# neel-dey/anatomix

Hardware: AMD Instinct MI355X
Metric: 128^3 volumes/sec feature-extraction (6M UNet) (higher is better)
Workload: dtype f16; 1 GPU; anatomix 6M UNet (ngf=16,num_downs=4) forward on sw_batch=4 windows of 1x128^3 (the predictor call of sliding_window_inference, BASELINE configs[1] / the metric); fp32 NCDHW in/out, 16-bit (f16) channels-last activations, fp32 accumulate; holds the 1e-3 tolerance against the fp32 reference in rel-L2 ONLY (max-norm 0.86e-3 .. 1.4e-3 by weight seed; the mode that holds both norms is value_strict); batch_per_gpu=4, window=128, parallelism=replicas x1 (no data-path collective)

## Files before the change

anatomix_amd/_lib.py:

```python
from __future__ import annotations

import ctypes as C
import os

_HERE = os.path.dirname(os.path.abspath(__file__))
LIB_PATH = os.environ.get("AMX_LIB_PATH") or os.path.join(_HERE, "csrc", "libanatomix_amd.so")

NORM = {"none": 0, "batch": 1, "instance": 2, "instance_affine": 3}
ACT = {"none": 0, "relu": 1, "lrelu": 2}
POOL = {"Max": 0, "Avg": 1}
INTERP = {"nearest": 0, "trilinear": 1}
WARP = {"bilinear": 0, "nearest": 1}
SEG_LABEL = {"float32": 0, "int64": 1, "uint8": 2}
SW_MAP = {"constant": 0, "gaussian": 1}
SW_OUT = {"features": 0, "logits": 1, "labels": 2}
PRECISION = {"f16": 0, "fp16": 0, "float16": 0, "bf16": 1, "bfloat16": 1, "f16x2": 2, "bf16x2": 3, "strict": 3, "fp32": 3,
             "f16x2mx": 4, "strict_mx": 4}


class UnetCfg(C.Structure):
    _fields_ = [
        ("input_nc", C.c_int32), ("output_nc", C.c_int32), ("num_downs", C.c_int32), ("ngf", C.c_int32),
        ("norm", C.c_int32), ("norm_eps", C.c_float), ("activation", C.c_int32), ("act_slope", C.c_float),
        ("final_act", C.c_int32), ("pooling", C.c_int32), ("interp", C.c_int32), ("doubleconv", C.c_int32),
        ("use_skip", C.c_int32), ("precision", C.c_int32),
    ]


class VitCfg(C.Structure):
    _fields_ = [
        ("input_channels", C.c_int32), ("num_classes", C.c_int32), ("embed_dim", C.c_int32), ("depth", C.c_int32),
        ("heads", C.c_int32), ("num_register_tokens", C.c_int32), ("grid_d", C.c_int32), ("grid_h", C.c_int32),
        ("grid_w", C.c_int32), ("hidden", C.c_int32), ("dec1", C.c_int32), ("dec2", C.c_int32), ("qk_norm", C.c_int32),
        ("scale_attn_inner", C.c_int32), ("layer_scale", C.c_int32), ("in_eps", C.c_float), ("out_norm", C.c_int32),
        ("decoder_split", C.c_int32), ("stem_split", C.c_int32),
    ]


_P = C.c_void_p
_I = C.c_int


class PackReq(C.Structure):
    _fields_ = [("d_weight", C.c_void_p), ("d_wpk", C.c_void_p), ("weight_mode", C.c_int32), ("cin_real", C.c_int32),
                ("cin_pad", C.c_int32), ("cout_real", C.c_int32), ("cout", C.c_int32), ("w", C.c_int32)]


WEIGHTS_PREPACKED = 16


class LaunchRecord(C.Structure):
    _fields_ = [("kernel", C.c_char * 64), ("module_idx", C.c_int32), ("cin", C.c_int32), ("cout", C.c_int32),
                ("n", C.c_int32), ("d", C.c_int32), ("h", C.c_int32), ("w", C.c_int32), ("ms", C.c_float),
                ("flops", C.c_double), ("bytes", C.c_double)]


SYMBOLS = {
    "amx_version": (_I, []),
    "amx_debug_fill_lds": (_I, [C.c_uint, _P]),
    "amx_last_error": (C.c_char_p, []),
    "amx_unet_create": (_I, [C.POINTER(_P), C.POINTER(UnetCfg)]),
    "amx_unet_destroy": (None, [_P]),
    "amx_unet_num_modules": (_I, [_P]),
    "amx_unet_num_convs": (_I, [_P]),
    "amx_unet_conv_info": (_I, [_P, _I, C.POINTER(_I), C.POINTER(_I), C.POINTER(_I), C.POINTER(_I)]),
    "amx_unet_load_conv": (_I, [_P, _I, _P, _P, _P, _P, _P, _P, _P]),
    "amx_unet_workspace_bytes": (C.c_size_t, [_P, _I, _I, _I, _I]),
    "amx_unet_forward": (_I, [_P, _P, _P, _I, _I, _I, _I, _P, C.c_size_t, _P]),
    "amx_unet_forward_profiled": (_I, [_P, _P, _P, _I, _I, _I, _I, _P, C.c_size_t, _P, C.POINTER(LaunchRecord), _I,
                                        C.POINTER(_I)]),
    "amx_unet_module_info": (_I, [_P, _I, C.POINTER(_I), C.POINTER(_I)]),
    "amx_unet_numerics_status": (_I, [_P, _I, _P]),
    "amx_unet_forward_taps": (_I, [_P, _P, _P, _I, _I, _I, _I, _P, C.c_size_t, C.POINTER(_I), _I, C.POINTER(_P), _I, _P]),
    "amx_unet_forward_window": (_I, [_P, _P, _I, _I, _I, _I, _I, _I, _I, _I, _I, _P, _P, _P, C.c_size_t, _P]),
    "amx_unet_forward_windows": (_I, [_P, _P, _I, _I, _I, _I, C.POINTER(C.c_int), _I, _I, _I, _P, _P, _P, C.c_size_t, _P]),
    "amx_unet_forward_windows_pipelined": (_I, [_P, _P, _I, _I, _I, _I, C.POINTER(C.c_int), _I, _I, _I, _P, _P, _P, C.c_size_t, _I, _P]),
    "amx_sw_normalize": (_I, [_P, _P, _I, C.c_longlong, _P]),
    "amx_sw_count": (_I, [_P, _I, _I, _I, _I, _I, _I, _I, _I, _I, _P, _P]),
    "amx_sw_plan": (_I, [_I, _I, _I, _I, _I, _I, C.c_double, C.POINTER(C.c_int), _I]),
    "amx_sw_importance_map": (_I, [_P, _I, _I, _I, _I, C.c_double, _P]),
    "amx_sw_count_all": (_I, [_P, _I, _I, _I, _I, _I, _I, C.c_double, _P, _P]),
    "amx_sw_finish": (_I, [_I, _P, _P, _I, C.c_longlong, _P, _P, _I, _P, _P]),
    "amx_sliding_window_workspace_bytes": (C.c_size_t, [_P, _I, _I, _I, _I]),
    "amx_sliding_window": (_I, [_P, _P, _I, _I, _I, _I, _I, _I, C.c_double, _I, C.c_double, _I, _I, _P, _P, _I, _P, _P, _P, _P,
                                C.c_size_t, _P]),
    "amx_conv3d_packed_bytes": (C.c_size_t, [_I, _I]),
    "amx_conv3d_k3_reflect": (_I, [_P, _I, _P, _I, _P, _P, _P, _I, _I, _I, _I, _I, _I, C.c_float, _I, _P, _P, _P, _P]),
    "amx_conv3d_dgrad_interior_supported": (_I, [_I, _I, _I, _I, _I, _I]),
    "amx_conv3d_dgrad_interior": (_I, [_P, _I, _P, _I, _I, _I, _I, _I, _I, _I, _I, _I, _P, _P, _P]),
    "amx_conv3d_dgrad_shell_scratch_bytes": (C.c_size_t, []),
    "amx_conv3d_dgrad_fold_shell": (_I, [_P, _I, _P, _I, _I, _P, _I, _I, _I, _I, _I, _I, _P, _P]),
    "amx_conv3d_pack_batch": (_I, [C.POINTER(PackReq), _I, _I, _P]),
    "amx_conv3d_scratch_bytes": (C.c_size_t, [_I, _I, _I, _I, _I, _I, _I, _I]),
    "amx_conv3d_k3_reflect_ws": (_I, [_P, _I, _P, _I, _P, _P, _P, _I, _I, _I, _I, _I, _I, C.c_float, _I, _P, _P, _P, _P, C.c_size_t, _P]),
    "amx_conv3d_upcat_merged_packed_bytes": (C.c_size_t, [_I, _I, _I]),
    "amx_conv3d_upcat_merged": (_I, [_P, _I, _P, _I, _P, _P, _P, _I, _I, _I, _I, _I, _I, C.c_float, _I, _P, _P, _P, _P]),
    "amx_conv3d_k3_reflect_ex": (_I, [_P, _I, _P, _I, _P, _I, _I, _I, _P, _P, _I, _I, _I, _I, _I, _I, C.c_float, _I, _P, _P, _P, _P]),
    "amx_pool2": (_I, [_P, _P, _I, _I, _I, _I, _I, _I, _I, _P]),
    "amx_instance_norm_scratch_bytes": (C.c_size_t, [_I, _I]),
    "amx_instance_norm": (_I, [_P, _P, _P, C.c_float, _I, C.c_longlong, _I, _I, C.c_float, _P, _I, _P]),
    "amx_upsample2_trilinear": (_I, [_P, _P, _I, _I, _I, _I, _I, _I, _P]),
    "amx_upsample2_trilinear_backward": (_I, [_P, _P, _I, _I, _I, _I, _I, _I, _P]),
    "amx_upcat_split_backward": (_I, [_P, _P, _P, _I, _I, _I, _I, _I, _I, _I, _I, _P]),
    "amx_upcat_split_backward_framed": (_I, [_P, _P, _P, _I, _I, _I, _I, _I, _I, _I, _I, _P]),
    "amx_export_ncdhw": (_I, [_P, _I, _I, _I, _I, _I, _P, _I, _P]),
    "amx_import_ncdhw": (_I, [_P, _P, _I, _I, _I, _I, _I, C.c_longlong, C.c_longlong, C.c_longlong, C.c_longlong, _I, _I, _P]),
    "amx_train_scratch_bytes": (C.c_size_t, [_I]),
    "amx_bn_train_forward": (_I, [_P, _P, _P, _P, C.c_float, _I, C.c_longlong, _I, _I, C.c_float, _P, _P, _P, _P, _P,
                                  C.c_float, _I, _P]),
    "amx_bn_act_backward": (_I, [_P, _P, _P, _P, _P, _P, _P, _P, _P, _I, _I, _I, _I, _I, _I, C.c_float, _P, _I, _P]),
    "amx_bn_act_backward_recompute": (_I, [_P, _P, _P, _P, _P, _P, _P, _P, _P, _I, _I, _I, _I, _I, _I, C.c_float, _P, _I, _P]),
    "amx_pad_fold": (_I, [_P, _P, _I, _I, _I, _I, _I, _I, _I, _P]),
    "amx_adamw_step": (_I, [_P, _I, C.c_double, C.c_double, C.c_double, C.c_double, C.c_double, _I, _P]),
    "amx_adamw_step_dev": (_I, [_P, _I, _P, _I, _P]),
    "amx_adamw_step_clip_dev": (_I, [_P, _I, _P, _I, _P, C.c_double, _P]),
    "amx_grad_norms_scratch_bytes": (C.c_size_t, [_P, _I, _I]),
    "amx_grad_norms": (_I, [_P, _I, _I, _P, _P, C.c_size_t, _P]),
    "amx_pool2_max_backward": (_I, [_P, _P, _P, _I, _I, _I, _I, _I, _I, _I, _P]),
    "amx_conv3d_wgrad_scratch_bytes": (C.c_size_t, [_I, _I, _I, _I, _I, _I]),
    "amx_conv3d_wgrad": (_I, [_P, C.c_longlong, C.c_longlong, C.c_longlong, C.c_longlong, _P, _I, _P, _I, _I, _I, _I, _I, _I,
                              _I, _P, _I, _P, C.c_size_t, _I, _P]),
    "amx_attention_scratch_bytes": (C.c_size_t, [_I, _I, _I, _I]),
    "amx_attention_qknorm_rope": (_I, [_P, _P, _P, _P, _P, _P, _P, C.c_float, _P, _I, _I, _I, _I, _I, _P, _P, C.c_size_t, _P]),
    "amx_attention_prepared": (_I, [_P, C.c_size_t, _I, _I, _I, _I, _P, _P]),
    "amx_vit_create": (_I, [C.POINTER(_P), C.POINTER(VitCfg)]),
    "amx_vit_destroy": (None, [_P]),
    "amx_vit_num_params": (_I, [_P]),
    "amx_vit_param_name": (C.c_char_p, [_P, _I]),
    "amx_vit_load": (_I, [_P, C.POINTER(_P), _I, _P, _P]),
    "amx_vit_workspace_bytes": (C.c_size_t, [_P, _I]),
    "amx_vit_forward": (_I, [_P, _P, _P, _I, _P, C.c_size_t, _I, _P]),
    "amx_vit_debug_read": (_I, [_P, C.c_char_p, _P, C.c_size_t, C.POINTER(C.c_size_t), _P]),
    "amx_linear": (_I, [_P, _P, _P, _I, _I, _I, _I, _P, _P]),
    "amx_supcon_scratch_bytes": (C.c_size_t, [_I, _I]),
    "amx_supcon_loss": (_I, [_P, _P, _I, _I, C.c_float, _I, _I, _I, _P, _P, _P, C.c_size_t, _P]),
    "amx_mlp_head_forward": (_I, [_P, _I, _I, _I, _I, _P, _P, _P, _P, _P, C.c_float, C.c_float, _I, C.c_float, _P, _P, _P, _P, _P]),
    "amx_mlp_head_scratch_bytes": (C.c_size_t, [_I, _I, _I]),
    "amx_mlp_head_backward": (_I, [_P, _P, _I, _I, _I, _I, _P, _P, _I, C.c_float, _P, _P, _P, _P, _P, _P, _P, _P, _P, C.c_size_t, _P]),
    "amx_mlp_heads_forward": (_I, [_I, _P, _I, _P, _I, _I, _P, _P, _P, _P, _P, C.c_float, C.c_float, _I, C.c_float, _P, _P, _P, _P, _P]),
    "amx_mlp_heads_backward": (_I, [_I, _P, _P, _I, _P, _I, _I, _P, _P, _I, C.c_float, _P, _P, _P, _P, _P, _P, _P, _P, _P, C.c_size_t, _P]),
    "amx_supcon_loss_batch": (_I, [_I, _P, _P, _I, _I, C.c_float, _I, _I, _I, _P, _P, _P, C.c_size_t, _P]),
    "amx_gather_labels_batch": (_I, [_P, _I, _I, _I, _I, _P, _I, _P, _I, _P, _P]),
    "amx_conv3d_backward_sampled_scratch_bytes": (C.c_size_t, [_I]),
    "amx_conv3d_backward_sampled": (_I, [_P, _P, _P, _I, _P, _I, _I, _I, _I, _I, _I, _I, _P, _P, _I, _P, C.c_size_t, _I, _P]),
    "amx_gather_rows": (_I, [_P, _I, C.c_longlong, C.c_longlong, C.c_longlong, C.c_longlong, C.c_longlong, _P, _I, _I, _I, _P, _P]),
    "amx_scatter_rows": (_I, [_P, _P, _P, _I, C.c_longlong, C.c_longlong, C.c_longlong, C.c_longlong, _I, _I, _I, _I, _P]),
    "amx_sample_coords": (_I, [_P, _I, _I, _I, _I, _I, _P, _P]),
    "amx_sample_perm": (_I, [_P, _I, _I, _I, _I, _P, _P]),
    "amx_import_input": (_I, [_P, _P, _I, _I, _I, _I, _I, _I, _P]),
    "amx_gather_labels": (_I, [_P, _I, _I, _I, _P, _I, _I, _I, _I, _I, _P, _P]),
    "amx_mindssc_scratch_bytes": (C.c_size_t, [_I, _I, _I]),
    "amx_mindssc": (_I, [_P, _I, _I, _I, _I, _I, _P, _P, C.c_size_t, _P]),
    "amx_avg_pool3d_cat": (_I, [_P, _I, C.c_float, _P, _I, C.c_float, _I, _I, _I, _I, _P, _P]),
    "amx_box_filter3d": (_I, [_P, _P, _I, _I, _I, _I, _I, _P]),
    "amx_correlate_scratch_bytes": (C.c_size_t, [_I, _I, _I, _I]),
    "amx_correlate_ssd": (_I, [_P, _P, _I, _I, _I, _I, _I, _P, _P, _P, C.c_size_t, _P]),
    "amx_coupled_convex_scratch_bytes": (C.c_size_t, [_I, _I, _I]),
    "amx_coupled_convex": (_I, [_P, _P, _I, _I, _I, _I, _P, _P, C.c_size_t, _P]),
    "amx_coupled_convex_step_scratch_bytes": (C.c_size_t, [_I, _I, _I]),
    "amx_coupled_convex_step": (_I, [_P, _P, _I, _I, _I, _I, _I, _P, _P, _P, C.c_size_t, _P]),
    "amx_inverse_consistency_scratch_bytes": (C.c_size_t, [_I, _I, _I]),
    "amx_inverse_consistency": (_I, [_P, _P, _I, _I, _I, _I, _P, _P, _P, C.c_size_t, _P]),
    "amx_resize_trilinear3d": (_I, [_P, _I, _I, _I, _I, _P, _I, _I, _I, C.POINTER(C.c_float), _I, _P]),
    "amx_stage1_registration_scratch_bytes": (C.c_size_t, [_I, _I, _I, _I, _I]),
    "amx_stage1_registration": (_I, [_P, _P, _I, _I, _I, _I, _I, _I, _I, _I, _I, _I, _P, _P, C.c_size_t, _P]),
    "amx_instance_opt_smooth3": (_I, [_P, _P, _I, _I, _I, _P]),
    "amx_instance_opt_scratch_bytes": (C.c_size_t, [_I, _I, _I, _I]),
    "amx_instance_opt_grad": (_I, [_P, _P, _P, _I, _I, _I, _I, C.c_float, _P, _P, _P, _P, C.c_size_t, _P]),
    "amx_instance_opt_adam_step": (_I, [_P, _P, _P, _P, C.c_longlong, C.c_double, _I, _P]),
    "amx_instance_opt": (_I, [_P, _P, _P, _I, _I, _I, _I, C.c_float, C.c_double, _I, _P, _P, C.c_size_t, _P]),
    "amx_run_instance_opt_scratch_bytes": (C.c_size_t, [_I, _I, _I, _I, _I, _I]),
    "amx_run_instance_opt": (_I, [_P, _P, _P, _I, _I, _I, _I, _I, C.c_float, _I, _I, C.c_double, _P, _P, C.c_size_t, _P]),
    "amx_warp3d": (_I, [_P, _I, _P, _I, _I, _I, _I, _P, _P]),
    "amx_seg_loss_scratch_bytes": (C.c_size_t, [_I, C.c_longlong, _I, _I]),
    "amx_seg_loss_forward": (_I, [_P, _I, _P, _P, _P, _I, _I, _I, C.c_longlong, _I, C.c_float, C.c_float, C.c_float, C.c_float, _P, _P,
                                  _P, _P, C.c_size_t, _P]),
    "amx_seg_loss_backward": (_I, [_P, _I, _P, _P, _P, _I, _I, _I, C.c_longlong, _I, C.c_float, C.c_float, C.c_float, C.c_float, _P, _P,
                                   _P, _P, _P, _P, C.c_size_t, _P]),
    "amx_seg_argmax": (_I, [_P, _I, _P, _P, _I, _I, C.c_longlong, _P, _P]),
    "amx_segaug_sample_bytes": (C.c_size_t, []),
    "amx_segaug_scratch_bytes": (C.c_size_t, [_I, C.c_longlong]),
    "amx_segaug_minmax": (_I, [_P, _I, C.c_longlong, _P, _P, C.c_size_t, _P]),
    "amx_segaug_minmax_finalize": (_I, [_P, C.c_size_t, _I, C.c_longlong, _P, _P]),
    "amx_segaug_pointwise": (_I, [_P, _P, _I, C.c_longlong, _P, _I, _P, _P, _P]),
    "amx_segaug_crop": (_I, [_I, _I, _I, _I, _P, _I, _P, _P, _P, _P, _P]),
    "amx_segaug_gaussian": (_I, [_P, _P, _P, _I, _I, _I, _I, _I, _P, _P, _P]),
    "amx_segaug_affine": (_I, [_P, _P, _I, _I, _I, _I, _P, _P, _I, _I, _I, _P, _P, _P, C.c_size_t, _P]),
    "amx_preaug_view_bytes": (C.c_size_t, []),
    "amx_preaug_spatial": (_I, [_P, _P, _I, _I, _I, _I, _P, _P, _P, _P, _P, _P]),
    "amx_preaug_blur": (_I, [_P, _P, _P, _I, _I, _I, _I, _P, _P, _P]),
    "amx_preaug_intensity": (_I, [_P, _P, _P, _I, _I, _I, _I, _P, _P, _P]),
    "amx_synth_view_bytes": (C.c_size_t, []),
    "amx_synth_scratch_bytes": (C.c_size_t, [_I, C.c_longlong]),
    "amx_synth_gmm_minmax": (_I, [_P, _P, _I, C.c_longlong, _P, _P, _P, C.c_size_t, _P]),
    "amx_synth_appearance": (_I, [_P, _P, C.POINTER(_P), C.POINTER(_I), _I, _P, _P, _I, _I, _I, _I, _P, _P, _P, C.c_size_t, _P]),
    "amx_synth_logk_mean": (_I, [_P, _I, C.c_longlong, _P, _P, C.c_size_t, _P]),
    "amx_synth_spike": (_I, [_P, _P, _I, _P, _I, _I, _I, _I, _P, _P, _P]),
    "amx_synth_lowres": (_I, [_P, _P, _I, _I, _I, _I, _P, _P, _P]),
    "amx_synth_clip_minmax": (_I, [_P, _I, C.c_longlong, _P, C.c_size_t, _P]),
    "amx_synth_finish": (_I, [_P, _P, _I, C.c_longlong, _P, _I, _P]),
    "amx_labels_template_bytes": (C.c_size_t, []),
    "amx_labels_ensemble_bytes": (C.c_size_t, []),
    "amx_labels_scratch_bytes": (C.c_size_t, [_I, C.c_longlong]),
    "amx_labels_compose": (_I, [_P, C.c_size_t, _P, _P, _I, _P, _P, _P, _I, _I, _I, _I, _P]),
    "amx_labels_median3": (_I, [_P, _P, _I, _I, _I, _I, _I, _P, _P, _P]),
    "amx_labels_sphere_mask": (_I, [C.POINTER(_P), _P, _I, _I, _P, _P, _P]),
    "amx_labels_apply_mask": (_I, [_P, _P, _P, _I, C.c_longlong, _P, _P, _P, C.c_size_t, _P]),
    "amx_labels_envelope": (_I, [_P, _P, _P, _I, _I, _I, _I, _P, _P, _P]),
    "amx_labels_merge_masks": (_I, [_P, _I, C.c_longlong, C.c_longlong, C.POINTER(_I), _P, _P, _P, _I, _P]),
    "amx_label_overlap": (_I, [_P, _I, _P, _I, C.c_longlong, _I, _P, _P, _P]),
    "amx_jacobian_det_scratch_bytes": (C.c_size_t, [_I, _I, _I]),
    "amx_jacobian_det": (_I, [_P, _I, _I, _I, _I, _P, _P, _P, C.c_size_t, _P]),
}

_lib = None


AMX_ERR_INVALID, AMX_ERR_SHAPE, AMX_ERR_NOT_LOADED, AMX_ERR_WORKSPACE, AMX_ERR_HIP, AMX_ERR_OVERFLOW = -1, -2, -3, -4, -5, -6


class AmxError(RuntimeError):

    def __init__(self, *args):
        self.code = args[0] if args and isinstance(args[0], int) else None
        super().__init__(*(args[1:] if self.code is not None else args))


class AmxEnvelopeError(AmxError):
    """The configuration lies outside what an engine entry covers (AMX_ERR_INVALID / AMX_ERR_SHAPE at create time)."""


class AmxOverflowError(AmxError, FloatingPointError):
    """AMX_ERR_OVERFLOW: f16 / f16x2 storage met a value outside the f16 range (include/anatomix_amd.h)."""


def load():
    global _lib
    if _lib is not None:
        return _lib
    if not os.path.exists(LIB_PATH):
        raise AmxError(
            f"{LIB_PATH} not found: build the HIP extension first (python -c 'import __graft_entry__ as g; "
            "g.build()' or make -C anatomix_amd/csrc).  There is no CPU fallback for the HIP path.")
    lib = C.CDLL(LIB_PATH)
    for name, (res, args) in SYMBOLS.items():
        fn = getattr(lib, name)
        fn.restype = res
        fn.argtypes = args
    _lib = lib
    return lib


def check(status: int):
    if status != 0:
        cls = AmxOverflowError if status == AMX_ERR_OVERFLOW else AmxError
        raise cls(int(status), f"anatomix_amd error {status}: {load().amx_last_error().decode()}")


def check_envelope(status: int):
    if status in (AMX_ERR_INVALID, AMX_ERR_SHAPE):
        raise AmxEnvelopeError(int(status), f"anatomix_amd error {status}: {load().amx_last_error().decode()}")
    check(status)


def ptr(t):
    return None if t is None else C.c_void_p(t.data_ptr())


def stream(dev):
    import torch
    return C.c_void_p(torch.cuda.current_stream(dev).cuda_stream)


def scratch(nbytes: int, dev):
    import torch
    return torch.empty(max(nbytes, 1), dtype=torch.uint8, device=dev)


def f32c(t):
    import torch
    return t if (t.dtype == torch.float32 and t.is_contiguous()) else t.float().contiguous()
```

anatomix_amd/csrc/amx_api.hip:

```cpp
#include <stdarg.h>
#include <stdio.h>
#include <string.h>

#include <string>
#include <vector>

#include "amx_launch.h"

static thread_local std::string g_err;

int amx::fail(int code, const char* fmt, ...) {
  char buf[512];
  va_list ap;
  va_start(ap, fmt);
  vsnprintf(buf, sizeof buf, fmt, ap);
  va_end(ap);
  g_err = buf;
  return code;
}

using namespace amx;

extern "C" {

int amx_version(void) { return AMX_VERSION; }

namespace {
__global__ __launch_bounds__(256) void fill_lds_kernel(unsigned pattern, unsigned* sink) {
  extern __shared__ unsigned lds_words[];
  for (int i = threadIdx.x; i < 160 * 1024 / 4; i += 256) lds_words[i] = pattern;
  __syncthreads();
  if (sink && lds_words[(threadIdx.x * 97) % (160 * 1024 / 4)] != pattern) *sink = 1;
}
}

int amx_debug_fill_lds(unsigned pattern, void* stream) {
  static amx::DeviceOnce attr_once;
  if (!attr_once.done()) {
    AMX_HIP(hipFuncSetAttribute((const void*)fill_lds_kernel, hipFuncAttributeMaxDynamicSharedMemorySize, 160 * 1024));
    attr_once.set();
  }
  hipLaunchKernelGGL(fill_lds_kernel, dim3(512), dim3(256), 160 * 1024, (hipStream_t)stream, pattern, (unsigned*)nullptr);
  AMX_HIP(hipGetLastError());
  return AMX_OK;
}

const char* amx_last_error(void) { return g_err.c_str(); }

int amx_sw_normalize(float* d_acc, const float* d_cnt, int channels, long long voxels, void* stream) {
  if (!d_acc || !d_cnt || channels < 1 || voxels < 1) return fail(AMX_ERR_INVALID, "bad argument");
  AMX_HIP(amx::launch_sw_normalize(d_acc, d_cnt, channels, voxels, (hipStream_t)stream));
  return AMX_OK;
}

int amx_sw_count(float* d_cnt, int vd, int vh, int vw, int oz, int oy, int ox, int rd, int rh, int rw,
                 const float* d_wmap, void* stream) {
  if (!d_cnt || !d_wmap) return fail(AMX_ERR_INVALID, "null argument");
  if (oz < 0 || oy < 0 || ox < 0 || oz + rd > vd || oy + rh > vh || ox + rw > vw)
    return fail(AMX_ERR_SHAPE, "window outside volume");
  AMX_HIP(amx::launch_sw_count(d_cnt, vd, vh, vw, oz, oy, ox, rd, rh, rw, d_wmap, (hipStream_t)stream));
  return AMX_OK;
}

int amx_sw_plan(int vd, int vh, int vw, int rd, int rh, int rw, double overlap, int* offsets_zyx, int capacity) {
  if (capacity < 0 || (capacity > 0 && !offsets_zyx)) return fail(AMX_ERR_INVALID, "bad offsets buffer");
  amx::SwPlan plan;
  if (int rc = amx::sw_make_plan(vd, vh, vw, rd, rh, rw, overlap, &plan)) return rc;
  const int n = plan.windows();
  for (int i = 0; i < n && i < capacity; ++i) plan.corner(i, offsets_zyx + 3 * i);
  return n;
}

int amx_sw_importance_map(float* d_wmap, int rd, int rh, int rw, int mode, double sigma_scale, void* stream) {
  if (!d_wmap) return fail(AMX_ERR_INVALID, "null argument");
  if (rd < 1 || rh < 1 || rw < 1) return fail(AMX_ERR_SHAPE, "non-positive roi");
  if (mode != AMX_SW_MAP_CONSTANT && mode != AMX_SW_MAP_GAUSSIAN) return fail(AMX_ERR_INVALID, "mode: constant (0) or gaussian (1) (got %d)", mode);
  if (mode == AMX_SW_MAP_GAUSSIAN && !(sigma_scale > 0.0)) return fail(AMX_ERR_INVALID, "sigma_scale must be positive (got %g)", sigma_scale);
  AMX_HIP(amx::launch_sw_importance_map(d_wmap, rd, rh, rw, mode, sigma_scale, (hipStream_t)stream));
  return AMX_OK;
}

int amx_sw_count_all(float* d_cnt, int vd, int vh, int vw, int rd, int rh, int rw, double overlap, const float* d_wmap,
                     void* stream) {
  if (!d_cnt || !d_wmap) return fail(AMX_ERR_INVALID, "null argument");
  amx::SwPlan plan;
  if (int rc = amx::sw_make_plan(vd, vh, vw, rd, rh, rw, overlap, &plan)) return rc;
  AMX_HIP(amx::launch_sw_count_all(d_cnt, plan, d_wmap, (hipStream_t)stream));
  return AMX_OK;
}

int amx_sw_finish(int kind, float* d_acc, const float* d_cnt, int feat, long long voxels, const float* d_w, const float* d_b,
                  int classes, void* d_out, void* stream) {
  if (int rc = amx::sw_finish_check(kind, d_acc, d_cnt, feat, voxels, d_w, classes, d_out)) return rc;
  AMX_HIP(amx::launch_sw_finish(kind, d_acc, d_cnt, feat, voxels, d_w, d_b, classes, d_out, (hipStream_t)stream));
  return AMX_OK;
}

size_t amx_conv3d_packed_bytes(int cin, int cout) {
  const int cin_pad = (cin + 15) / 16 * 16;
  size_t bytes = (size_t)cout * cin_pad * 28 * 2;
  if (cin == 48 && cout == 16) bytes = (bytes + 255) / 256 * 256 + amx::conv_upcat16_packed_bytes();
  return 2 * bytes + 256;
}

static int conv3d_single(const void* d_x0, int c0, const void* d_x1, int c1, const float* d_weight, int weight_mode,
                         int cin_real, int cout_real, const float* d_scale, const float* d_shift, int cout, int n, int d,
                         int hh, int w, int act, float slope, int precision, void* d_wpk, void* d_out16, float* d_out32,
                         void* stream, void* d_scratch = nullptr, size_t scratch_bytes = 0) {
  if (!d_x0 || (!d_weight && !(weight_mode & AMX_WEIGHTS_PREPACKED)) || !d_wpk || (!d_out16 == !d_out32)) return fail(AMX_ERR_INVALID, "bad pointer arguments");
  if (c0 % 16 || c1 % 16 || c0 + c1 < 16 || cout % 16 || cout < 16)
    return fail(AMX_ERR_INVALID, "channel counts must be multiples of 16 (c0=%d c1=%d cout=%d)", c0, c1, cout);
  if (c1 && (!d_x1 || (d & 1) || (hh & 1) || (w & 1))) return fail(AMX_ERR_SHAPE, "upsampled segment needs even dims");
  if (d < 2 || hh < 2 || w < 2) return fail(AMX_ERR_SHAPE, "reflect padding needs >= 2 voxels per axis");
  hipStream_t st = (hipStream_t)stream;
  if (precision < AMX_PREC_F16 || precision > AMX_PREC_F16X2_MX) return fail(AMX_ERR_INVALID, "unsupported precision %d", precision);
  const bool prepacked = (weight_mode & AMX_WEIGHTS_PREPACKED) != 0;
  weight_mode &= ~AMX_WEIGHTS_PREPACKED;
  if (prepacked && (is_split(precision) || d_scale)) return fail(AMX_ERR_INVALID, "prepacked weights: plain 16-bit precisions, no scale");
  if (is_mx(precision) && weight_mode != 0) return fail(AMX_ERR_INVALID, "f16x2mx packs forward weights only");
  const int q = amx::conv_pick_q(cout, w, precision);
  if (d_out32 && (q > 2 || w < 32)) return fail(AMX_ERR_INVALID, "fp32 planar output needs cout <= 32 and w >= 32");
  if (cin_real < 1 || cin_real > c0 + c1 || cout_real < 1 || cout_real > cout || (weight_mode != 0 && weight_mode != 1))
    return fail(AMX_ERR_INVALID, "bad weight description (mode %d, cin_real %d, cout_real %d)", weight_mode, cin_real, cout_real);
  amx::ConvParams p;
  memset(&p, 0, sizeof p);
  if (is_mx(precision)) {
    int* mxs = (int*)((char*)d_wpk + align_up((size_t)cout * (c0 + c1) * 28 * 2 * 2, 256));
    AMX_HIP(amx::launch_pack_weights_mx(d_weight, d_scale, d_wpk, mxs, cin_real, c0 + c1, cout, q, st, cout_real));
    p.mxs = mxs;
  } else if (!prepacked) {
    AMX_HIP(amx::launch_pack_weights(d_weight, d_scale, d_wpk, cin_real, c0 + c1, cout, q, precision, st, weight_mode, cout_real));
  }
  p.N = n; p.D = d; p.H = hh; p.W = w; p.Cout = cout;
  amx::set_src0(p, d_x0, c0, d, hh, w, precision);
  if (c1) {
    amx::set_src1(p, d_x1, c1, d / 2, hh / 2, w / 2, precision);
    p.up_shift = 1;
  }
  p.wpk = (const char*)d_wpk;
  p.bias = d_shift;
  p.act = act; p.slope = slope;
  if (d_out16) {
    amx::set_out(p, d_out16, cout, d, hh, w, precision);
  } else {
    p.out32 = d_out32;
    p.py = w; p.pz = (long long)hh * w; p.pc = p.pz * d; p.pn = p.pc * cout;
  }
  if (!is_split(precision) && weight_mode == 0 && cin_real == 48 && c0 == 16 && c1 == 32 && cout == 16 && amx::conv_upcat16_eligible(p)) {
    if (prepacked)
      return fail(AMX_ERR_INVALID, "prepacked weights: the 16 + up32 -> 16 merged-tap layer packs its own format (call without the flag)");
    char* up = (char*)d_wpk + ((size_t)cout * (c0 + c1) * 28 * 2 + 255) / 256 * 256;
    AMX_HIP(amx::launch_pack_upcat16(d_weight, d_scale, up, precision, st));
    p.wpk = up;
    AMX_HIP(amx::launch_conv_upcat16(p, precision, st));
    return AMX_OK;
  }
  if (d_scratch && !c1 && d_out16) {
    const size_t need = amx::conv_ks_part_bytes(c0, cout, n, d, hh, w, precision, q);
    if (need && (scratch_bytes < need || ((uintptr_t)d_scratch & 15)))
      return fail(AMX_ERR_WORKSPACE, "split-K scratch needs %zu bytes, 16-byte aligned (got %zu)", need, scratch_bytes);
    if (need) p.part = (float*)d_scratch;
  }
  AMX_HIP(amx::launch_conv(p, precision, q, st));
  return AMX_OK;
}

static bool dgrad_interior_shape_ok(int c_dy, int cout, int d, int hh, int w, int precision) {
  if (precision != AMX_PREC_F16 && precision != AMX_PREC_BF16) return false;
  amx::ConvParams p;
  memset(&p, 0, sizeof p);
  p.C0 = c_dy; p.Cout = cout; p.D = d; p.H = hh; p.W = w; p.out = (char*)1;
  return amx::conv_zmarch_eligible(p) && amx::conv_pick_q(cout, w, precision) == cout / 16 && (size_t)27 * c_dy * cout * 4 <= 150 * 1024;
}

int amx_conv3d_dgrad_interior_supported(int c_dy, int cout, int d, int hh, int w, int precision) {
  return dgrad_interior_shape_ok(c_dy, cout, d, hh, w, precision) ? 1 : 0;
}

int amx_conv3d_dgrad_interior(const void* d_dy_framed, int c_dy, const float* d_weight, int weight_flags, int cin_real, int cout_real, int cout,
                              int n, int d, int hh, int w, int precision, void* d_wpk, void* d_out16, void* stream) {
  if (!d_dy_framed || !d_wpk || !d_out16 || (!d_weight && !(weight_flags & AMX_WEIGHTS_PREPACKED)))
    return fail(AMX_ERR_INVALID, "dgrad_interior: bad pointer arguments");
  if (!dgrad_interior_shape_ok(c_dy, cout, d, hh, w, precision))
    return fail(AMX_ERR_INVALID, "dgrad_interior: shape outside the z-march kernels (ask amx_conv3d_dgrad_interior_supported)");
  if (cin_real < 1 || cin_real > c_dy || cout_real < 1 || cout_real > cout) return fail(AMX_ERR_INVALID, "dgrad_interior: bad weight description");
  hipStream_t st = (hipStream_t)stream;
  const int q = cout / 16;
  if (!(weight_flags & AMX_WEIGHTS_PREPACKED))
    AMX_HIP(amx::launch_pack_weights(d_weight, nullptr, d_wpk, cin_real, c_dy, cout, q, precision, st, 1, cout_real));
  amx::ConvParams p;
  memset(&p, 0, sizeof p);
  p.N = n; p.D = d; p.H = hh; p.W = w; p.Cout = cout; p.C0 = c_dy;
  p.s0x = (long long)c_dy * 2; p.s0y = p.s0x * (w + 4); p.s0z = p.s0y * (hh + 4); p.s0n = p.s0z * (d + 4);
  p.src0 = (const char*)d_dy_framed + 2 * (p.s0z + p.s0y + p.s0x);
  p.raw_halo = 1;
  p.wpk = (const char*)d_wpk;
  p.act = AMX_ACT_NONE;
  p.out = (char*)d_out16;
  p.ox = (long long)cout * 2; p.oy = p.ox * w; p.oz = p.oy * hh; p.on = p.oz * d;
  AMX_HIP(amx::launch_conv(p, precision, q, st));
  return AMX_OK;
}

size_t amx_conv3d_dgrad_shell_scratch_bytes(void) { return amx::dgrad_shell_scratch_bytes(); }

int amx_conv3d_dgrad_fold_shell(const void* d_dy_framed, int c_dy, const float* d_weight, int co_real, int ci_real, void* d_dx, int c_dx, int n,
                                int d, int hh, int w, int precision, void* d_scratch, void* stream) {
  if (!d_dy_framed || !d_weight || !d_dx || !d_scratch || ((uintptr_t)d_scratch & 15) || co_real < 1 || co_real > c_dy || ci_real < 1 || ci_real > c_dx || d < 2 || hh < 2 || w < 2)
    return fail(AMX_ERR_INVALID, "dgrad_fold_shell: bad arguments");
  const long long fx = (long long)c_dy * 2, fy = fx * (w + 4), fz = fy * (hh + 4), fn = fz * (d + 4);
  AMX_HIP(amx::launch_dgrad_fold_shell((const char*)d_dy_framed + 2 * (fz + fy + fx), fn, fz, fy, fx, c_dy, d_weight, co_real, ci_real, d_dx, c_dx,
                                       n, d, hh, w, precision, d_scratch, (hipStream_t)stream));
  return AMX_OK;
}

int amx_conv3d_pack_batch(const amx_pack_req* reqs, int count, int precision, void* stream) {
  if (!reqs || count < 1 || count > 256 || (precision != AMX_PREC_F16 && precision != AMX_PREC_BF16))
    return fail(AMX_ERR_INVALID, "pack_batch: bad arguments");
  std::vector<const float*> w(count);
  std::vector<void*> wpk(count);
  std::vector<int> cr(count), cp(count), co(count), q(count), md(count), cor(count);
  for (int i = 0; i < count; ++i) {
    const amx_pack_req& r = reqs[i];
    if (!r.d_weight || !r.d_wpk || r.cin_pad % 16 || r.cin_pad < 16 || r.cout % 16 || r.cout < 16 || r.cin_real < 1 || r.cin_real > r.cin_pad ||
        r.cout_real < 1 || r.cout_real > r.cout || (r.weight_mode != 0 && r.weight_mode != 1))
      return fail(AMX_ERR_INVALID, "pack_batch: bad request %d", i);
    w[i] = r.d_weight; wpk[i] = r.d_wpk; cr[i] = r.cin_real; cp[i] = r.cin_pad; co[i] = r.cout; md[i] = r.weight_mode; cor[i] = r.cout_real;
    q[i] = amx::conv_pick_q(r.cout, r.w, precision);
  }
  AMX_HIP(amx::launch_pack_weights_batch(count, w.data(), wpk.data(), cr.data(), cp.data(), co.data(), q.data(), md.data(), cor.data(), precision,
                                         (hipStream_t)stream));
  return AMX_OK;
}

size_t amx_conv3d_scratch_bytes(int c0, int c1, int cout, int n, int d, int hh, int w, int precision) {
  if (c1 || c0 % 16 || cout % 16 || precision < AMX_PREC_F16 || precision > AMX_PREC_F16X2_MX) return 0;
  return amx::conv_ks_part_bytes(c0, cout, n, d, hh, w, precision, amx::conv_pick_q(cout, w, precision));
}

int amx_conv3d_k3_reflect_ws(const void* d_x0, int c0, const void* d_x1, int c1, const float* d_weight,
                             const float* d_scale, const float* d_shift, int cout, int n, int d, int hh, int w,
                             int act, float slope, int precision, void* d_wpk, void* d_out16, float* d_out32,
                             void* d_scratch, size_t scratch_bytes, void* stream) {
  return conv3d_single(d_x0, c0, d_x1, c1, d_weight, 0, c0 + c1, cout, d_scale, d_shift, cout, n, d, hh, w, act, slope,
                       precision, d_wpk, d_out16, d_out32, stream, d_scratch, scratch_bytes);
}

int amx_conv3d_k3_reflect(const void* d_x0, int c0, const void* d_x1, int c1, const float* d_weight,
                          const float* d_scale, const float* d_shift, int cout, int n, int d, int hh, int w,
                          int act, float slope, int precision, void* d_wpk, void* d_out16, float* d_out32,
                          void* stream) {
  return conv3d_single(d_x0, c0, d_x1, c1, d_weight, 0, c0 + c1, cout, d_scale, d_shift, cout, n, d, hh, w, act, slope,
                       precision, d_wpk, d_out16, d_out32, stream);
}

int amx_conv3d_k3_reflect_ex(const void* d_x0, int c0, const void* d_x1, int c1, const float* d_weight, int weight_mode,
                             int cin_real, int cout_real, const float* d_scale, const float* d_shift, int cout, int n,
                             int d, int hh, int w, int act, float slope, int precision, void* d_wpk, void* d_out16,
                             float* d_out32, void* stream) {
  return conv3d_single(d_x0, c0, d_x1, c1, d_weight, weight_mode, cin_real, cout_real, d_scale, d_shift, cout, n, d, hh, w,
                       act, slope, precision, d_wpk, d_out16, d_out32, stream);
}

size_t amx_conv3d_upcat_merged_packed_bytes(int c0, int c1, int cout) {
  return 2 * (align_up((size_t)cout * c0 * 28 * 2, 256) + amx::conv_upmerge_packed_bytes(c1, cout, 0));
}

int amx_conv3d_upcat_merged(const void* d_x0, int c0, const void* d_x1, int c1, const float* d_weight, const float* d_scale,
                            const float* d_shift, int cout, int n, int d, int hh, int w, int act, float slope, int precision,
                            void* d_wpk, void* d_partial, void* d_out16, void* stream) {
  if (!d_x0 || !d_x1 || !d_weight || !d_wpk || !d_partial || !d_out16) return fail(AMX_ERR_INVALID, "null argument");
  if (precision < AMX_PREC_F16 || precision > AMX_PREC_BF16X2) return fail(AMX_ERR_INVALID, "unsupported precision %d", precision);
  const bool split = is_split(precision);
  if (c0 != cout || !amx::conv_upmerge_eligible(c0, c1, cout, d, hh, w, 1, split))
    return fail(AMX_ERR_INVALID, "merged concat conv needs c0 == cout >= 32 (16 in the strict precisions), c1 %% 32 == 0, w >= 16, even dims "
                "(c0=%d c1=%d cout=%d dims %d,%d,%d)", c0, c1, cout, d, hh, w);
  hipStream_t st = (hipStream_t)stream;
  const int q = amx::conv_pick_q(cout, w, precision);
  char* wmerge = (char*)d_wpk + align_up((size_t)cout * c0 * 28 * 2 * (split ? 2 : 1), 256);
  AMX_HIP(amx::launch_pack_weights(d_weight, d_scale, d_wpk, c0, c0, cout, q, precision, st, 0, 0, c0 + c1));
  AMX_HIP(amx::launch_pack_upmerge(d_weight, d_scale, wmerge, c0, c0 + c1, c1, cout, precision, st));
  amx::ConvParams p;
  memset(&p, 0, sizeof p);
  p.N = n; p.D = d; p.H = hh; p.W = w; p.Cout = cout;
  amx::set_src0(p, d_x0, c0, d, hh, w, precision);
  p.wpk = (const char*)d_wpk; p.act = AMX_ACT_NONE;
  amx::set_out(p, d_partial, cout, d, hh, w, precision);
  AMX_HIP(amx::launch_conv(p, precision, q, st));
  amx::UpmergeParams u;
  memset(&u, 0, sizeof u);
  amx::set_src(u, d_x1, c1, d / 2, hh / 2, w / 2, precision);
  u.N = n; u.LD = d / 2; u.LH = hh / 2; u.LW = w / 2; u.Cout = cout;
  u.wpk = wmerge; u.part = (const char*)d_partial; u.out = (char*)d_out16;
  u.bias = d_shift; u.act = act; u.slope = slope;
  AMX_HIP(amx::launch_conv_upmerge(u, precision, st));
  return AMX_OK;
}

int amx_pool2(const void* d_in, void* d_out, int n, int dout, int hout, int wout, int c, int avg, int precision,
              void* stream) {
  if (!d_in || !d_out || c % 8) return fail(AMX_ERR_INVALID, "bad argument");
  AMX_HIP(amx::launch_pool2(d_in, d_out, n, dout, hout, wout, c, avg, precision, (hipStream_t)stream));
  return AMX_OK;
}

size_t amx_train_scratch_bytes(int c) { return amx::train_scratch_bytes(c); }

int amx_bn_train_forward(const void* d_x, void* d_y, const float* d_gamma, const float* d_beta, float eps, int n,
                         long long voxels, int c, int act, float slope, void* d_scratch, float* d_save_mean,
                         float* d_save_rstd, float* d_running_mean, float* d_running_var, float momentum, int precision,
                         void* stream) {
  if (!d_x || !d_y || !d_scratch || n < 1 || voxels < 1 || c % 8 || c > 2048) return fail(AMX_ERR_INVALID, "bad argument");
  AMX_HIP(amx::launch_bn_train_forward(d_x, d_y, d_gamma, d_beta, eps, (long long)n * voxels, c, act, slope, d_scratch, d_save_mean,
                                       d_save_rstd, d_running_mean, d_running_var, momentum, precision, (hipStream_t)stream));
  return AMX_OK;
}

int amx_bn_act_backward(const void* d_dy, const void* d_y, const void* d_x, const float* d_mean, const float* d_rstd,
                        const float* d_gamma, float* d_dgamma, float* d_dbeta, void* d_dx_framed, int n, int d, int hh, int w,
                        int c, int act, float slope, void* d_scratch, int precision, void* stream) {
  if (!d_dy || !d_y || !d_dx_framed || !d_scratch || c % 8 || c > 2048) return fail(AMX_ERR_INVALID, "bad argument");
  if (d_mean && (!d_x || !d_rstd || !d_dgamma || !d_dbeta)) return fail(AMX_ERR_INVALID, "norm backward needs x, rstd, dgamma, dbeta");
  AMX_HIP(amx::launch_bn_act_backward(d_dy, d_y, d_x ? d_x : d_y, d_mean, d_rstd, d_gamma, nullptr, d_dgamma, d_dbeta, d_dx_framed, n,
                                      d, hh, w, c, act, slope, d_scratch, precision, (hipStream_t)stream));
  return AMX_OK;
}

int amx_bn_act_backward_recompute(const void* d_dy, const void* d_x, const float* d_mean, const float* d_rstd, const float* d_gamma,
                                  const float* d_beta, float* d_dgamma, float* d_dbeta, void* d_dx_framed, int n, int d, int hh, int w,
                                  int c, int act, float slope, void* d_scratch, int precision, void* stream) {
  if (!d_dy || !d_x || !d_mean || !d_rstd || !d_dgamma || !d_dbeta || !d_dx_framed || !d_scratch || c % 8 || c > 2048)
    return fail(AMX_ERR_INVALID, "bad argument");
  AMX_HIP(amx::launch_bn_act_backward(d_dy, nullptr, d_x, d_mean, d_rstd, d_gamma, d_beta, d_dgamma, d_dbeta, d_dx_framed, n, d, hh, w,
                                      c, act, slope, d_scratch, precision, (hipStream_t)stream));
  return AMX_OK;
}

int amx_pad_fold(const void* d_g_framed, void* d_din, int n, int d, int hh, int w, int c, int accumulate, int precision,
                 void* stream) {
  if (!d_g_framed || !d_din || c % 8 || d < 2 || hh < 2 || w < 2) return fail(AMX_ERR_INVALID, "bad argument");
  AMX_HIP(amx::launch_pad_fold(d_g_framed, d_din, n, d, hh, w, c, accumulate, precision, (hipStream_t)stream));
  return AMX_OK;
}

int amx_adamw_step(const amx_adamw_tensor* tensors, int count, double lr, double beta1, double beta2, double eps, double weight_decay,
                   int maximize, void* stream) {
  static_assert(sizeof(amx_adamw_tensor) == 48, "six 64-bit fields");
  if (count < 0 || (count && !tensors)) return fail(AMX_ERR_INVALID, "bad argument");
  if (!(lr >= 0.0) || !(eps >= 0.0) || !(beta1 >= 0.0 && beta1 < 1.0) || !(beta2 >= 0.0 && beta2 < 1.0) || !(weight_decay >= 0.0))
    return fail(AMX_ERR_INVALID, "adamw: lr %g, betas (%g, %g), eps %g, weight_decay %g out of range", lr, beta1, beta2, eps, weight_decay);
  for (int t = 0; t < count; ++t) {
    const amx_adamw_tensor& r = tensors[t];
    if (!r.param || !r.grad || !r.exp_avg || !r.exp_avg_sq || !r.step || r.numel < 0)
      return fail(AMX_ERR_INVALID, "adamw: tensor %d has a null pointer or a negative size", t);
  }
  AMX_HIP(amx::launch_adamw((const long long*)tensors, count, lr, beta1, beta2, eps, weight_decay, maximize, (hipStream_t)stream));
  return AMX_OK;
}

int amx_adamw_step_dev(const amx_adamw_tensor* tensors, int count, const double* d_hyper, int maximize, void* stream) {
  if (count < 0 || (count && !tensors) || !d_hyper) return fail(AMX_ERR_INVALID, "bad argument");
  for (int t = 0; t < count; ++t) {
    const amx_adamw_tensor& r = tensors[t];
    if (!r.param || !r.grad || !r.exp_avg || !r.exp_avg_sq || !r.step || r.numel < 0)
      return fail(AMX_ERR_INVALID, "adamw: tensor %d has a null pointer or a negative size", t);
  }
  AMX_HIP(amx::launch_adamw((const long long*)tensors, count, 0.0, 0.0, 0.0, 0.0, 0.0, maximize, (hipStream_t)stream, d_hyper));
  return AMX_OK;
}

int amx_adamw_step_clip_dev(const amx_adamw_tensor* tensors, int count, const double* d_hyper, int maximize, const float* d_total_norm,
                            double max_norm, void* stream) {
  if (count < 0 || (count && !tensors) || !d_hyper || !d_total_norm || !(max_norm >= 0.0))
    return fail(AMX_ERR_INVALID, "adamw: bad argument (max_norm %g)", max_norm);
  for (int t = 0; t < count; ++t) {
    const amx_adamw_tensor& r = tensors[t];
    if (!r.param || !r.grad || !r.exp_avg || !r.exp_avg_sq || !r.step || r.numel < 0)
      return fail(AMX_ERR_INVALID, "adamw: tensor %d has a null pointer or a negative size", t);
  }
  AMX_HIP(amx::launch_adamw((const long long*)tensors, count, 0.0, 0.0, 0.0, 0.0, 0.0, maximize, (hipStream_t)stream, d_hyper, d_total_norm,
                            max_norm));
  return AMX_OK;
}

size_t amx_grad_norms_scratch_bytes(const amx_grad_tensor* tensors, int count, int groups) {
  static_assert(sizeof(amx_grad_tensor) == 24, "three 64-bit fields");
  if (count < 0 || groups < 0 || (count && !tensors)) return 0;
  return amx::grad_norms_scratch_bytes((const long long*)tensors, count, groups);
}

int amx_grad_norms(const amx_grad_tensor* tensors, int count, int groups, float* d_out, void* d_scratch, size_t scratch_bytes,
                   void* stream) {
  if (count < 0 || groups < 0 || (count && !tensors) || (groups && !d_out) || !d_scratch) return fail(AMX_ERR_INVALID, "bad argument");
  for (int t = 0; t < count; ++t)
    if (!tensors[t].grad && tensors[t].numel) return fail(AMX_ERR_INVALID, "grad_norms: tensor %d has a null pointer", t);
  if (amx_grad_norms_scratch_bytes(tensors, count, groups) == 0 || scratch_bytes < amx_grad_norms_scratch_bytes(tensors, count, groups))
    return fail(AMX_ERR_INVALID, "grad_norms: a negative size, a group outside [0, %d), too many blocks, or too little scratch", groups);
  AMX_HIP(amx::launch_grad_norms((const long long*)tensors, count, groups, d_out, d_scratch, scratch_bytes, (hipStream_t)stream));
  return AMX_OK;
}

int amx_pool2_max_backward(const void* d_dp, const void* d_in, void* d_din, int n, int dout, int hout, int wout, int c,
                           int accumulate, int precision, void* stream) {
  if (!d_dp || !d_in || !d_din || c % 8) return fail(AMX_ERR_INVALID, "bad argument");
  AMX_HIP(amx::launch_pool2_max_backward(d_dp, d_in, d_din, n, dout, hout, wout, c, accumulate, precision, (hipStream_t)stream));
  return AMX_OK;
}

size_t amx_conv3d_wgrad_scratch_bytes(int n, int d, int hh, int w, int cout, int cin_pad) {
  return amx::wgrad_scratch_bytes(n, d, hh, w, cout, cin_pad);
}

int amx_conv3d_wgrad(const void* d_dy, long long dy_sn, long long dy_sz, long long dy_sy, long long dy_sx, const void* d_x0,
                     int c0, const void* d_x1, int c1, int cin_real, int cout, int n, int d, int hh, int w, float* d_dw,
                     int accumulate, void* d_scratch, size_t scratch_bytes, int precision, void* stream) {
  if (!d_dy || !d_x0 || !d_dw || !d_scratch) return fail(AMX_ERR_INVALID, "null argument");
  if (c0 % 16 || c1 % 16 || c0 + c1 < 16 || cout % 16 || cout < 16 || cin_real < 1 || cin_real > c0 + c1)
    return fail(AMX_ERR_INVALID, "channel counts must be multiples of 16 (c0=%d c1=%d cout=%d)", c0, c1, cout);
  if (c1 && (!d_x1 || (d & 1) || (hh & 1) || (w & 1))) return fail(AMX_ERR_SHAPE, "upsampled segment needs even dims");
  if (d < 2 || hh < 2 || w < 2 || w > 128) return fail(AMX_ERR_SHAPE, "wgrad supports 2 <= w <= 128 (got %d)", w);
  if (scratch_bytes < amx::wgrad_scratch_bytes(n, d, hh, w, cout, c0 + c1))
    return fail(AMX_ERR_WORKSPACE, "scratch needs %zu bytes", amx::wgrad_scratch_bytes(n, d, hh, w, cout, c0 + c1));
  amx::WgradParams p;
  memset(&p, 0, sizeof p);
  p.dy = (const char*)d_dy; p.yn = dy_sn; p.yz = dy_sz; p.yy = dy_sy; p.yx = dy_sx;
  amx::set_src0(p, d_x0, c0, d, hh, w, AMX_PREC_F16);
  if (c1) {
    amx::set_src1(p, d_x1, c1, d / 2, hh / 2, w / 2, AMX_PREC_F16);
    p.up_shift = 1;
  }
  p.N = n; p.D = d; p.H = hh; p.W = w; p.Cout = cout;
  AMX_HIP(amx::launch_wgrad(p, cin_real, d_dw, accumulate, d_scratch, precision, (hipStream_t)stream));
  return AMX_OK;
}

size_t amx_attention_scratch_bytes(int b, int heads, int n, int head_dim) {
  if (b < 1 || heads < 1 || n < 1 || head_dim < 2 || head_dim > 80) return 0;
  return amx::attention_scratch_bytes(b, heads, n);
}

int amx_attention_qknorm_rope(const float* d_q, const float* d_k, const float* d_v, const float* d_qn_w, const float* d_qn_b,
                              const float* d_kn_w, const float* d_kn_b, float norm_eps, const float* d_rope, int n_prefix, int b,
                              int n, int heads, int head_dim, float* d_out, void* d_scratch, size_t scratch_bytes, void* stream) {
  if (!d_q || !d_k || !d_v || !d_out || !d_scratch) return fail(AMX_ERR_INVALID, "null argument");
  if (b < 1 || n < 1 || heads < 1 || head_dim < 2 || head_dim > 80 || (head_dim & 1))
    return fail(AMX_ERR_INVALID, "attention: head_dim must be even and <= 80 (got %d), b, n, heads >= 1", head_dim);
  if ((!d_qn_w) != (!d_qn_b) || (!d_kn_w) != (!d_kn_b)) return fail(AMX_ERR_INVALID, "attention: norm weight and bias go together");
  if (n_prefix < 0 || n_prefix > n) return fail(AMX_ERR_INVALID, "attention: 0 <= n_prefix <= n");
  if (scratch_bytes < amx::attention_scratch_bytes(b, heads, n) || ((uintptr_t)d_scratch & 15))
    return fail(AMX_ERR_WORKSPACE, "attention scratch needs %zu bytes, 16-byte aligned", amx::attention_scratch_bytes(b, heads, n));
  AMX_HIP(amx::launch_attention(d_q, d_k, d_v, d_qn_w, d_qn_b, d_kn_w, d_kn_b, norm_eps, d_rope, n_prefix, b, n, heads, head_dim, d_out,
                                d_scratch, (hipStream_t)stream));
  return AMX_OK;
}

int amx_attention_prepared(const void* d_scratch, size_t scratch_bytes, int b, int n, int heads, int head_dim, float* d_out, void* stream) {
  if (!d_scratch || !d_out) return fail(AMX_ERR_INVALID, "null argument");
  if (b < 1 || n < 1 || heads < 1 || head_dim < 2 || head_dim > 80 || (head_dim & 1))
    return fail(AMX_ERR_INVALID, "attention: head_dim must be even and <= 80 (got %d), b, n, heads >= 1", head_dim);
  if (scratch_bytes < amx::attention_scratch_bytes(b, heads, n) || ((uintptr_t)d_scratch & 15))
    return fail(AMX_ERR_WORKSPACE, "attention scratch needs %zu bytes, 16-byte aligned", amx::attention_scratch_bytes(b, heads, n));
  void *Qp, *Kp, *Vt;
  amx::attention_operands((void*)d_scratch, b, heads, n, &Qp, &Kp, &Vt, nullptr, nullptr);
  AMX_HIP(amx::launch_attention_fwd(Qp, Kp, Vt, b, n, heads, head_dim, d_out, (hipStream_t)stream));
  return AMX_OK;
}

size_t amx_supcon_scratch_bytes(int n, int c) { return amx::supcon_scratch_bytes(n, c); }

int amx_supcon_loss(const float* d_feat, const int* d_labels, int n, int c, float temperature, int weigh_rarity,
                    int balance_denominator, int sqrt_mode, float* d_loss, float* d_grad, void* d_scratch,
                    size_t scratch_bytes, void* stream) {
  if (!d_feat || !d_labels || !d_loss || !d_scratch) return fail(AMX_ERR_INVALID, "null argument");
  if (n < 2 || n > 16384 || c < 1 || !(temperature > 0.f)) return fail(AMX_ERR_INVALID, "bad sizes (n=%d c=%d T=%g)", n, c, temperature);
  if (int rc = amx::need_scratch(amx::supcon_scratch_bytes(n, c), scratch_bytes)) return rc;
  AMX_HIP(amx::launch_supcon(d_feat, d_labels, n, c, temperature, weigh_rarity, balance_denominator, sqrt_mode, d_loss,
                             d_grad, d_scratch, (hipStream_t)stream));
  return AMX_OK;
}

size_t amx_instance_norm_scratch_bytes(int n, int c) { return amx::instnorm_scratch_bytes(n, c, 0); }

int amx_instance_norm(void* d_x, const float* d_gamma, const float* d_beta, float eps, int n, long long voxels, int c,
                      int act, float slope, void* d_scratch, int precision, void* stream) {
  if (!d_x || !d_scratch || c % 8 || c > 2048 || n < 1 || voxels < 1) return fail(AMX_ERR_INVALID, "bad argument");
  if (!d_gamma != !d_beta) return fail(AMX_ERR_INVALID, "gamma and beta come together");
  if (precision == AMX_PREC_F16X2_MX && voxels > (1 << 24)) return fail(AMX_ERR_INVALID, "f16x2mx: at most 2^24 voxels per sample here");
  AMX_HIP(amx::launch_instnorm(d_x, d_gamma, d_beta, eps, n, voxels, c, act, slope, d_scratch, precision,
                               (hipStream_t)stream, nullptr, 0, nullptr, (int)voxels));
  return AMX_OK;
}

int amx_upsample2_trilinear(const void* d_in, void* d_out, int n, int din, int hin, int win, int c, int precision,
                            void* stream) {
  if (!d_in || !d_out || c % 8 || n < 1 || din < 1 || hin < 1 || win < 1) return fail(AMX_ERR_INVALID, "bad argument");
  AMX_HIP(amx::launch_upsample2_trilinear(d_in, d_out, n, din, hin, win, c, precision, (hipStream_t)stream));
  return AMX_OK;
}

size_t amx_mindssc_scratch_bytes(int H, int W, int D) { return amx::mindssc_scratch_bytes(H, W, D); }

int amx_mindssc(const float* d_img, int H, int W, int D, int radius, int dilation, float* d_out, void* d_scratch,
                size_t scratch_bytes, void* stream) {
  if (!d_img || !d_out || !d_scratch) return fail(AMX_ERR_INVALID, "null argument");
  if (H < 1 || W < 1 || D < 1) return fail(AMX_ERR_SHAPE, "non-positive shape");
  if (radius < 1 || radius > 2 || dilation < 1 || dilation > 4)
    return fail(AMX_ERR_INVALID, "radius in {1, 2}, dilation in [1, 4] (got %d, %d)", radius, dilation);
  if (int rc = amx::need_scratch(amx::mindssc_scratch_bytes(H, W, D), scratch_bytes)) return rc;
  AMX_HIP(amx::launch_mindssc(d_img, H, W, D, radius, dilation, d_out, d_scratch, (hipStream_t)stream));
  return AMX_OK;
}

int amx_avg_pool3d_cat(const float* d_a, int ca, float scale_a, const float* d_b, int cb, float scale_b, int H, int W, int D,
                       int g, float* d_out, void* stream) {
  if (!d_out || (ca > 0 && !d_a) || (cb > 0 && !d_b) || ca < 0 || cb < 0 || ca + cb < 1) return fail(AMX_ERR_INVALID, "bad argument");
  if (g < 1 || H < g || W < g || D < g) return fail(AMX_ERR_SHAPE, "pool size %d does not fit (%d,%d,%d)", g, H, W, D);
  AMX_HIP(amx::launch_pool_cat(d_a, ca, scale_a, d_b, cb, scale_b, H, W, D, g, d_out, (hipStream_t)stream));
  return AMX_OK;
}

int amx_box_filter3d(const float* d_in, float* d_out, int c, int H, int W, int D, int k, void* stream) {
  if (!d_in || !d_out || d_in == d_out || c < 1 || c > 65535) return fail(AMX_ERR_INVALID, "bad argument");
  if (H < 1 || W < 1 || D < 1) return fail(AMX_ERR_SHAPE, "non-positive shape");
  if (k < 3 || k > 9 || !(k & 1)) return fail(AMX_ERR_INVALID, "kernel size must be odd in [3, 9] (got %d)", k);
  AMX_HIP(amx::launch_box_filter(d_in, d_out, c, H, W, D, k, (hipStream_t)stream));
  return AMX_OK;
}

size_t amx_correlate_scratch_bytes(int h, int w, int d, int disp_hw) { return amx::correlate_scratch_bytes(h, w, d, disp_hw); }

int amx_correlate_ssd(const float* d_fix, const float* d_mov, int c, int h, int w, int d, int disp_hw, float* d_ssd,
                      long long* d_argmin, void* d_scratch, size_t scratch_bytes, void* stream) {
  if (!d_fix || !d_mov || !d_ssd || !d_scratch || c < 1) return fail(AMX_ERR_INVALID, "bad argument");
  if (h < 1 || w < 1 || d < 1) return fail(AMX_ERR_SHAPE, "non-positive shape");
  if (disp_hw < 1 || disp_hw > 3) return fail(AMX_ERR_INVALID, "disp_hw in {1, 2, 3} (got %d)", disp_hw);
  if (int rc = amx::need_scratch(amx::correlate_scratch_bytes(h, w, d, disp_hw), scratch_bytes)) return rc;
  AMX_HIP(amx::launch_correlate(d_fix, d_mov, c, h, w, d, disp_hw, d_ssd, d_argmin, d_scratch, (hipStream_t)stream));
  return AMX_OK;
}

static int mlp_check(int n, int cin, int width, int n_layers) {
  if (n < 1 || n > 2048) return fail(AMX_ERR_SHAPE, "mlp head: 1 <= n <= 2048 rows (got %d)", n);
  if (cin < 4 || cin % 4 || width < 8 || width % 8) return fail(AMX_ERR_SHAPE, "mlp head: cin %% 4 == 0 and width %% 8 == 0 (got %d, %d)", cin, width);
  if (cin > 4096 || width > 4096) return fail(AMX_ERR_SHAPE, "mlp head: at most 4096 features per layer (got %d, %d)", cin, width);
  if (n_layers < 1 || n_layers > 8) return fail(AMX_ERR_INVALID, "mlp head: 1 <= n_layers <= 8 (got %d)", n_layers);
  return AMX_OK;
}

// ... 254 lines not shown
```

anatomix_amd/csrc/amx_conv3d_upcat.hip:

```cpp
#include <stdlib.h>

#include "amx_device.h"
#include "amx_launch.h"

namespace amx {

typedef __attribute__((address_space(1))) const void* gptr_t;
typedef __attribute__((address_space(3))) void* lptr_t;

struct UpcatCfg {
  static constexpr int TY = 8, TX = 32, NC = 8, NL = 3;
  static constexpr int R = 10;
  static constexpr int RL = 6;
  static constexpr int HY = TY + 2, HX = TX + 2, HXH = HX / 2;
  static constexpr int HVP = HY * HX;
  static constexpr int PPL = ((HVP * 16 + 255) / 256) * 256;
  static constexpr int PLSZ = 2 * PPL;
  static constexpr int LY = TY / 2 + 2, LX = TX / 2 + 2, LVP = LY * LX;
  static constexpr int LPL = ((LVP * 16 + 255) / 256) * 256;
  static constexpr int LPSZ = 4 * LPL;
  static constexpr int LOFF = R * PLSZ;
  static constexpr int FLAGOFF = LOFF + RL * LPSZ;
  static constexpr int LDS_BYTES = FLAGOFF + 64;
  static constexpr int NDMA = (HVP + 63) / 64;
  static constexpr int NDMAL = 4 * ((LVP + 63) / 64);
  static constexpr int AHEAD = R - 4;
  static constexpr int AHEADL = RL - 3;
  static_assert(LDS_BYTES <= 160 * 1024, "rings must fit the LDS");
  static_assert(R * NDMA <= 60 && RL * NDMAL <= 60, "vmcnt range");
};

template <typename T, int OUTMODE>
__global__ __launch_bounds__((UpcatCfg::NC + UpcatCfg::NL) * 64) void conv3d_upcat16_kernel(const ConvParams p, int zseg,
                                                                                           int nseg) {
  typedef UpcatCfg C;
  typedef typename Ops<T>::vec8 vec8;
  constexpr int HX = C::HX, PPL = C::PPL, PLSZ = C::PLSZ, LX = C::LX, LPL = C::LPL, LPSZ = C::LPSZ, R = C::R, RL = C::RL;
  constexpr int NC = C::NC, TY = C::TY, TX = C::TX;

  extern __shared__ __attribute__((aligned(16))) char smem[];

  const int tid = threadIdx.x, lane = tid & 63;
  const int wave = __builtin_amdgcn_readfirstlane(tid >> 6);

  int b = blockIdx.x;
  const int nb = gridDim.x;
  if ((nb & 7) == 0) b = (b & 7) * (nb >> 3) + (b >> 3);
  const int bx = b % p.nbx;
  b /= p.nbx;
  const int by = b % p.nby;
  b /= p.nby;
  const int sg = b % nseg;
  const int n = b / nseg;
  const int y0 = by * TY, x0 = bx * TX;
  const int zs = sg * zseg;
  const int ze = (zs + zseg < p.D) ? zs + zseg : p.D;
  const int nsteps = (ze - zs) / 2;
  const int nplanes = ze - zs + 2;
  const int nlow = nsteps + 2;

  int* ready = (int*)(smem + C::FLAGOFF);
  int* done = (int*)(smem + C::FLAGOFF + 32);
  if (tid < 16) ((int*)(smem + C::FLAGOFF))[tid] = 0;
  __syncthreads();

  if (wave >= NC + 2) {
    constexpr int NJ = (C::LVP + 63) / 64;
    int off[NJ];
    bool valid[NJ];
    const int LD = p.D >> 1, LH = p.H >> 1, LW = p.W >> 1;
#pragma unroll
    for (int j = 0; j < NJ; ++j) {
      const int hv = j * 64 + lane;
      const int hy = hv / LX, hx = hv - hy * LX;
      valid[j] = hv < C::LVP;
      int gy = (y0 >> 1) - 1 + hy, gxx = (x0 >> 1) - 1 + hx;
      gy = gy < 0 ? 0 : (gy >= LH ? LH - 1 : gy);
      gxx = gxx < 0 ? 0 : (gxx >= LW ? LW - 1 : gxx);
      off[j] = gy * (int)p.s1y + gxx * (int)p.s1x;
    }
    const char* src_n = p.src1 + (long long)n * p.s1n;
    auto issue_plane = [&](int ql) {
      int lz = (zs >> 1) - 1 + ql;
      lz = lz < 0 ? 0 : (lz >= LD ? LD - 1 : lz);
      const char* plane = src_n + (long long)lz * p.s1z;
      char* dstp = smem + C::LOFF + (ql % RL) * LPSZ;
#pragma unroll
      for (int cg = 0; cg < 4; ++cg)
#pragma unroll
        for (int j = 0; j < NJ; ++j)
          if (valid[j])
            __builtin_amdgcn_global_load_lds((gptr_t)(plane + off[j] + cg * 16), (lptr_t)(dstp + cg * LPL + j * 1024), 16, 0, 0);
    };
    int next_issue = 0, next_pub = 0;
    const unsigned a_ready = lds_addr(ready + 2), a_done = lds_addr(done);
    while (next_pub < nlow) {
      if (next_issue < nlow) {
        const int md = __builtin_amdgcn_readfirstlane(flag_min8_asm(a_done));
        int lim = RL + md;
        lim = lim < nlow ? lim : nlow;
        while (next_issue < lim) issue_plane(next_issue++);
      }
      if (next_issue == next_pub) {
        __builtin_amdgcn_s_sleep(2);
        continue;
      }
      WaitVm<C::NDMAL, RL - 1>::run(next_issue - next_pub - 1);
      flag_store_asm(a_ready, ++next_pub);
    }
    return;
  }
  if (wave >= NC) {
    const int cp = wave - NC;
    int off[C::NDMA];
    bool valid[C::NDMA];
#pragma unroll
    for (int j = 0; j < C::NDMA; ++j) {
      const int sl = j * 64 + lane;
      const int hy = sl / HX, pos = sl - hy * HX;
      const int hx = pos < C::HXH ? 2 * pos : 2 * (pos - C::HXH) + 1;
      valid[j] = sl < C::HVP;
      off[j] = reflect_clamp(y0 + hy - 1, p.H) * (int)p.s0y + reflect_clamp(x0 + hx - 1, p.W) * (int)p.s0x + cp * 16;
    }
    const char* src_n = p.src0 + (long long)n * p.s0n;
    auto issue_plane = [&](int q) {
      const char* plane = src_n + (long long)reflect_clamp(zs - 1 + q, p.D) * p.s0z;
      char* dstp = smem + (q % R) * PLSZ + cp * PPL;
#pragma unroll
      for (int j = 0; j < C::NDMA; ++j)
        if (valid[j]) __builtin_amdgcn_global_load_lds((gptr_t)(plane + off[j]), (lptr_t)(dstp + j * 1024), 16, 0, 0);
    };
    int next_issue = 0, next_pub = 0;
    const unsigned a_ready = lds_addr(ready + cp), a_done = lds_addr(done);
    while (next_pub < nplanes) {
      if (next_issue < nplanes) {
        const int md = __builtin_amdgcn_readfirstlane(flag_min8_asm(a_done));
        int lim = R + 2 * md;
        lim = lim < nplanes ? lim : nplanes;
        while (next_issue < lim) issue_plane(next_issue++);
      }
      if (next_issue == next_pub) {
        __builtin_amdgcn_s_sleep(2);
        continue;
      }
      WaitVm<C::NDMA, R - 1>::run(next_issue - next_pub - 1);
      flag_store_asm(a_ready, ++next_pub);
    }
    return;
  }

  const int pz = wave >> 2, py = (wave >> 1) & 1, px = wave & 1;
  const int li = lane & 15, g = lane >> 4, hi = g >> 1;
  vec8 wsk[kSteps], wup[8];
#pragma unroll
  for (int s = 0; s < kSteps; ++s) wsk[s] = *(const vec8*)(p.wpk + s * 1024 + lane * 16);
#pragma unroll
  for (int e = 0; e < 8; ++e) wup[e] = *(const vec8*)(p.wpk + (kSteps + wave * 8 + e) * 1024 + lane * 16);
  f32x4 bias = f32x4{0.f, 0.f, 0.f, 0.f};
  if (p.bias) bias = *(const f32x4*)(p.bias + g * 4);
  asm volatile("s_waitcnt vmcnt(0)" ::: "memory");

  const int slot0 = px * C::HXH + li;
  const int d1 = px ? -(C::HXH - 1) : C::HXH;
  const int lanebase = (g & 1) * PPL + (py * HX + slot0) * 16;
  const int base_d1 = lanebase + hi * d1 * 16;
  const int base_dx = lanebase + hi * HX * 16;
  const int lbase = C::LOFF + g * LPL + ((py * LX) + li + px) * 16;

  const bool full_xy = (y0 + TY <= p.H) & (x0 + TX <= p.W);
  const int yl = y0 + py, xl = x0 + 2 * li + px;
  char* out_l = OUTMODE == 0 ? p.out + (long long)n * p.on + (long long)yl * p.oy + (long long)xl * p.ox + g * 8 : nullptr;
  char* out_w = OUTMODE == 0 ? p.out + (long long)n * p.on + (long long)yl * p.oy + (long long)xl * p.ox + (g >> 1) * 16 : nullptr;
  float* out32_l = OUTMODE == 1 ? p.out32 + (long long)n * p.pn + (long long)(g * 4) * p.pc + (long long)yl * p.py + xl
                                : nullptr;

  bool bad = false;
  for (int s = 0; s < nsteps; ++s) {
    {
      int need = 2 * s + 4, needl = s + 3;
      need = need < nplanes ? need : nplanes;
      needl = needl < nlow ? needl : nlow;
      while (true) {
        static_assert(C::FLAGOFF % 16 == 0, "the ready flags are polled with one 16-byte read");
        const flag4_t r = flag_read4(ready);
        if ((r[0] < r[1] ? r[0] : r[1]) >= need && r[2] >= needl) break;
        __builtin_amdgcn_s_sleep(1);
      }
      asm volatile("" ::: "memory");
    }
    const int zo = zs + 2 * s + pz;
    int slo[3], llo[2];
#pragma unroll
    for (int kz = 0; kz < 3; ++kz) slo[kz] = __builtin_amdgcn_readfirstlane(((2 * s + pz + kz) % R) * PLSZ);
#pragma unroll
    for (int ez = 0; ez < 2; ++ez) llo[ez] = __builtin_amdgcn_readfirstlane(((s + pz + ez) % RL) * LPSZ);
    const int bzv = lanebase + (hi ? slo[1] : slo[0]);

    f32x4 acc[4];
#pragma unroll
    for (int c = 0; c < 4; ++c) acc[c] = bias;

    if (!(p.dbg & 2)) {
      constexpr int NSK = 4 * kSteps, NU = NSK + 4 * 8, NSLOT = 8;
      auto src = [&](int i) -> const vec8* {
        if (i < NSK) {
          const int st = i >> 2, c = i & 3;
          const int kz = st < 9 ? st / 3 : (st < 12 ? st - 9 : (st == 12 ? 0 : 2));
          const int ky = st < 9 ? st % 3 : (st < 12 ? 0 : 2);
          const int kx2 = st < 9 ? 0 : 1;
          const int off = (ky * HX + kx2) * 16 + (2 * c * HX) * 16;
          if (st < 9) return (const vec8*)(smem + base_d1 + (slo[kz] + off));
          if (st < 12) return (const vec8*)(smem + base_dx + (slo[kz] + off));
          if (st == 12) return (const vec8*)(smem + bzv + off);
          return (const vec8*)(smem + lanebase + (slo[2] + off));
        }
        const int e = (i - NSK) >> 2, c = (i - NSK) & 3;
        const int ez = e >> 2, ey = (e >> 1) & 1, ex = e & 1;
        return (const vec8*)(smem + lbase + (llo[ez] + ((c + ey) * LX + ex) * 16));
      };
      vec8 S[NSLOT];
#pragma unroll
      for (int i = 0; i < NSLOT; ++i) S[i] = *src(i);
#pragma unroll
      for (int i = 0; i < NU; ++i) {
        const int c = i < NSK ? (i & 3) : ((i - NSK) & 3);
        acc[c] = Ops<T>::mfma(i < NSK ? wsk[i >> 2] : wup[(i - NSK) >> 2], S[i % NSLOT], acc[c]);
        if (i + NSLOT < NU) S[i % NSLOT] = *src(i + NSLOT);
        __builtin_amdgcn_sched_barrier(0);
      }
    }
    asm volatile("s_waitcnt lgkmcnt(0)" ::: "memory");
    flag_store(done + wave, s + 1);

    act_inplace<4>(&acc[0], p.act, p.slope);
    if (OUTMODE == 0 && zo < ze && !(p.dbg & 4) && !(p.dbg & 32)) {
#pragma unroll
      for (int cp = 0; cp < 2; ++cp) {
        unsigned pk[2][2];
#pragma unroll
        for (int h = 0; h < 2; ++h) {
          float v[4];
#pragma unroll
          for (int j = 0; j < 4; ++j) {
            float f = acc[2 * cp + h][j];
              if (RangeCheck<T>::on) bad |= RangeCheck<T>::bad(f);
            v[j] = f;
          }
          pk[h][0] = (unsigned)to_bits<T>(v[0]) | ((unsigned)to_bits<T>(v[1]) << 16);
          pk[h][1] = (unsigned)to_bits<T>(v[2]) | ((unsigned)to_bits<T>(v[3]) << 16);
        }
        const auto s0 = __builtin_amdgcn_permlane16_swap(pk[0][0], pk[1][0], false, false);
        const auto s1 = __builtin_amdgcn_permlane16_swap(pk[0][1], pk[1][1], false, false);
        const int row = 2 * (2 * cp + (g & 1));
        if (!full_xy && !((yl + row < p.H) & (xl < p.W))) continue;
        *(uint4*)(out_w + (long long)zo * p.oz + row * p.oy) = make_uint4(s0[0], s1[0], s0[1], s1[1]);
      }
    } else if (zo < ze && !(p.dbg & 4)) {
#pragma unroll
      for (int c = 0; c < 4; ++c) {
        if (!full_xy && !((yl + 2 * c < p.H) & (xl < p.W))) continue;
        float v[4];
#pragma unroll
        for (int j = 0; j < 4; ++j) {
          float f = acc[c][j];
          if (OUTMODE == 0 && RangeCheck<T>::on) bad |= RangeCheck<T>::bad(f);
          v[j] = f;
        }
        if (OUTMODE == 0) {
          char* dst = out_l + (long long)zo * p.oz + (2 * c) * p.oy;
          *(uint2*)dst = make_uint2((unsigned)to_bits<T>(v[0]) | ((unsigned)to_bits<T>(v[1]) << 16),
                                    (unsigned)to_bits<T>(v[2]) | ((unsigned)to_bits<T>(v[3]) << 16));
        } else {
          float* dst = out32_l + (long long)zo * p.pz + (2 * c) * p.py;
          if (p.wmap) {
            const float wgt = p.wmap[((long long)zo * p.H + yl + 2 * c) * p.W + xl];
#pragma unroll
            for (int j = 0; j < 4; ++j) dst[(long long)j * p.pc] += wgt * v[j];
          } else {
#pragma unroll
            for (int j = 0; j < 4; ++j) dst[(long long)j * p.pc] = v[j];
          }
        }
      }
    }
  }
  if (OUTMODE == 0 && RangeCheck<T>::on) raise_flag(p.oflow, bad);
}

template <typename T>
__global__ void pack_upcat16_kernel(const float* __restrict__ w, const float* __restrict__ scale, T* __restrict__ wpk) {
  const int idx = blockIdx.x * blockDim.x + threadIdx.x;
  const int total = (kSteps + 64) * 512;
  if (idx >= total) return;
  const int e8 = idx & 7, lane = (idx >> 3) & 63, frag = idx >> 9;
  const int m = lane & 15, g = lane >> 4;
  const float sc = scale ? scale[m] : 1.f;
  float v = 0.f;
  if (frag < kSteps) {
    const int tap = (g >> 1) ? tapB_index(frag) : tapA_index(frag);
    const int cin = (g & 1) * 8 + e8;
    if (tap >= 0) v = w[(m * 48 + cin) * 27 + tap] * sc;
  } else {
    const int f = frag - kSteps;
    const int cls = f >> 3, e = f & 7;
    const int par[3] = {cls >> 2, (cls >> 1) & 1, cls & 1};
    const int ee[3] = {e >> 2, (e >> 1) & 1, e & 1};
    const int cin = 16 + g * 8 + e8;
    int lo[3], hi[3];
    for (int a = 0; a < 3; ++a) {
      if (par[a] == 0) { lo[a] = ee[a] ? 1 : 0; hi[a] = ee[a] ? 2 : 0; }
      else { lo[a] = ee[a] ? 2 : 0; hi[a] = ee[a] ? 2 : 1; }
    }
    float sum = 0.f;
    for (int kz = lo[0]; kz <= hi[0]; ++kz)
      for (int ky = lo[1]; ky <= hi[1]; ++ky)
        for (int kx = lo[2]; kx <= hi[2]; ++kx) sum += w[(m * 48 + cin) * 27 + (kz * 3 + ky) * 3 + kx];
    v = sum * sc;
  }
  wpk[idx] = (T)v;
}

size_t conv_upcat16_packed_bytes() { return (size_t)(kSteps + 64) * 1024; }

bool conv_upcat16_eligible(const ConvParams& p) {
  return !p.src0_f32c1 && p.up_shift == 1 && p.C0 == 16 && p.C1 == 32 && p.Cout == 16 && p.W >= 32 && p.H >= 8 && p.D >= 4 &&
         !(p.D & 1) && !(p.H & 1) && !(p.W & 1);
}

template <typename T, int OUTMODE>
static hipError_t launch_upcat_t(ConvParams p, hipStream_t st, ConvLaunchInfo* info) {
  typedef UpcatCfg C;
  if (info) info->report(0, "conv3d_upcat16<%s,2x8x32,c8+l3,r%d/%d,o%d>", __is_same(T, f16) ? "f16" : "bf16", C::R, C::RL, OUTMODE);
  auto kern = conv3d_upcat16_kernel<T, OUTMODE>;
  static amx::DeviceOnce attr_once;
  if (!attr_once.done()) {
    hipError_t e = hipFuncSetAttribute((const void*)kern, hipFuncAttributeMaxDynamicSharedMemorySize, C::LDS_BYTES);
    if (e != hipSuccess) return e;
    attr_once.set();
  }
  p.nby = (p.H + C::TY - 1) / C::TY;
  p.nbx = (p.W + C::TX - 1) / C::TX;
  const int tiles = p.nby * p.nbx * p.N;
  int nseg, zseg;
  pick_z_segments(tiles, p.D, 2, 256 * (C::LDS_BYTES <= 80 * 1024 ? 2 : 1), &zseg, &nseg);
  hipLaunchKernelGGL(kern, dim3((unsigned)(tiles * nseg)), dim3((C::NC + C::NL) * 64), C::LDS_BYTES, st, p, zseg, nseg);
  return hipGetLastError();
}

hipError_t launch_conv_upcat16(const ConvParams& p, int precision, hipStream_t st, ConvLaunchInfo* info) {
  const bool planar = p.out32 != nullptr;
  if (precision == 0) return planar ? launch_upcat_t<f16, 1>(p, st, info) : launch_upcat_t<f16, 0>(p, st, info);
  return planar ? launch_upcat_t<bf16, 1>(p, st, info) : launch_upcat_t<bf16, 0>(p, st, info);
}

hipError_t launch_pack_upcat16(const float* w, const float* scale, void* wpk, int precision, hipStream_t st) {
  const int total = (kSteps + 64) * 512;
  if (precision == 0)
    hipLaunchKernelGGL(pack_upcat16_kernel<f16>, dim3((total + 255) / 256), dim3(256), 0, st, w, scale, (f16*)wpk);
  else
    hipLaunchKernelGGL(pack_upcat16_kernel<bf16>, dim3((total + 255) / 256), dim3(256), 0, st, w, scale, (bf16*)wpk);
  return hipGetLastError();
}

}
```

anatomix_amd/csrc/amx_conv3d_zmarch.hip:

```cpp
#include <stdlib.h>
#include <string.h>

#include "amx_device.h"
#include "amx_launch.h"

namespace amx {

typedef __attribute__((address_space(1))) const void* gptr_t;
typedef __attribute__((address_space(3))) void* lptr_t;

template <int NCK, int QT, int TY, int TX, int R>
struct ZmCfg {
  static constexpr int NC = 8, TZ = 2;
  static constexpr int NL = 2 * NCK;
  static constexpr int HY = TY + 2, HX = TX + 2, HVP = HY * HX;
  static constexpr int PPL = ((HVP * 16 + 255) / 256) * 256;
  static constexpr int PLSZ = NL * PPL;
  static constexpr int FLAGOFF = R * PLSZ;
  static constexpr int LDS_BYTES = R * PLSZ + 64;
  static constexpr int XT = TX / 16;
  static constexpr int WPQ = NC / QT;
  static constexpr int NDMA = (HVP + 63) / 64;
  static_assert(WPQ == (TY / 2) * XT, "each consumer wave owns a 2 x 2 x 16 voxel block per step");
  static_assert(R - 4 > TZ, "ring must hold more than one step of prefetch");
  static constexpr bool VMCNT_OK = R * NDMA <= 60;
  static_assert(NL <= 8 && LDS_BYTES <= 160 * 1024, "ring must fit the LDS");
};

template <int QT, int TY, int TX, int OUTMODE>
struct ZmStage {
  static constexpr int CB = 32 * QT;
  static constexpr int CS = 2 * TY * TX * 4 + 64;
  static constexpr int BYTES = OUTMODE == 0 ? 2 * TY * TX * CB : 16 * QT * CS;
  static constexpr int NB = OUTMODE == 0 ? 2 : 1;
  static constexpr int TOTAL = NB * BYTES;
};

struct StemIn {
  const char* src;
  long long sn, sz, sy;
  long long offs[16];
  int use_offs;
  const char* wpk;
  const float* bias;
  int act;
  float slope;
};

template <int TY, int TX>
struct ZmStemCfg {
  static constexpr int HY = TY + 2, HX = TX + 2, HVP = HY * HX;
  static constexpr int IY = HY + 2, IX = HX + 2, IVP = IY * IX;
  static constexpr int RS = (TX + 8) * 2;
  static constexpr int CPSZ = IY * RS;
  static constexpr int IPLSZ = ((2 * CPSZ + 8 + 63) / 64) * 64;
  static constexpr int DUMMY = IPLSZ - 8;
  static constexpr int RC = 16;
  static constexpr int SW = 40;
  static constexpr int STGSZ = ((IY * SW * 4 + 255) / 256) * 256;
  static constexpr int RSTG = 8;
  static constexpr int NLD = (IVP + 63) / 64;
  static constexpr int BYTES = RC * IPLSZ + RSTG * STGSZ;
  static constexpr int NSW = 7;
  static constexpr int LEAD = 3;
  static constexpr int NT = 2 * HY + (2 * HY + 15) / 16;
  static constexpr bool OK = TX == 32 && IY == 12 && RSTG * 2 <= 60 && NLD == 7;
};

template <typename T, int NCK, int QT, int TY, int TX, int R, int OUTMODE, int NS, bool POOL, bool SPLIT = false, bool STEM = false>
__global__ __launch_bounds__((8 + (STEM ? ZmStemCfg<8, 32>::NSW + 1 : 2 * (SPLIT ? 2 : NCK)) + NS) * 64) void conv3d_k3_zmarch_kernel(const ConvParams p, int zseg, int nseg, const StemIn si) {
  static_assert(!SPLIT || (NCK == 1 && QT == 1 && NS == 0), "strict z-march: 16 -> 16, direct stores");
  static_assert(!STEM || (NCK == 1 && !SPLIT && NS == 0 && OUTMODE == 0), "stem-fed z-march: 16 input channels, direct 16-bit stores");
  constexpr int NCKP = SPLIT ? 2 : NCK;
  typedef ZmCfg<NCKP, QT, TY, TX, R> C;
  typedef ZmStage<QT, TY, TX, OUTMODE> SG;
  typedef typename Ops<T>::vec8 vec8;
  constexpr int HX = C::HX, PPL = C::PPL, PLSZ = C::PLSZ, XT = C::XT, NDMA = C::NDMA, NL = C::NL, NC = C::NC, TZ = C::TZ;
  constexpr int STAGEOFF = C::FLAGOFF + 128;
  static_assert(NS == 0 || NS == 2, "one storer wave per output plane of a step");
  static_assert(NS == 0 || STAGEOFF + SG::TOTAL <= 160 * 1024, "ring + staging tile must fit the LDS");

  extern __shared__ __attribute__((aligned(16))) char smem[];

  const int tid = threadIdx.x, lane = tid & 63;
  const int wave = __builtin_amdgcn_readfirstlane(tid >> 6);

  int b = blockIdx.x;
  const int nb = gridDim.x;
  if ((nb & 7) == 0) b = (b & 7) * (nb >> 3) + (b >> 3);
  const int bx = b % p.nbx;
  b /= p.nbx;
  const int by = b % p.nby;
  b /= p.nby;
  const int sg = b % nseg;
  const int n = b / nseg;
  const int y0 = by * TY, x0 = bx * TX;
  const int zs = sg * zseg;
  const int ze = (zs + zseg < p.D) ? zs + zseg : p.D;
  const int nplanes = ze - zs + 2;
  const int nsteps = (ze - zs + TZ - 1) / TZ;

  int* ready = (int*)(smem + C::FLAGOFF);
  int* done = (int*)(smem + C::FLAGOFF + 32);
  int* staged = (int*)(smem + C::FLAGOFF + 64);
  int* stored = (int*)(smem + C::FLAGOFF + 96);
  if (tid < ((NS || STEM) ? 32 : 16))
    ((int*)(smem + C::FLAGOFF))[tid] = (STEM && (tid < 8 || tid >= 24)) ? ((tid & 7) == 7 ? 0x7fffffff : (tid & 7)) : 0;
  if constexpr (STEM) {
    typedef ZmStemCfg<TY, TX> SC;
    static_assert(SC::OK && STAGEOFF + SC::BYTES <= 160 * 1024, "stem-fed geometry; ring + input rings must fit the LDS");
    for (int i = tid; i < SC::RC * SC::IPLSZ / 4; i += (NC + SC::NSW + 1) * 64) ((int*)(smem + STAGEOFF))[i] = 0;
  }
  __syncthreads();

  if (NS && wave >= NC + NL) {
    const int w = wave - NC - NL;
    const unsigned a_staged = lds_addr(staged), a_stored = lds_addr(stored + w);
    if constexpr (OUTMODE == 0) {
      constexpr int NR = TY * QT;
      const char* sbase = smem + STAGEOFF + w * TY * TX * SG::CB + lane * 16;
      char* gbase = p.out + (long long)n * p.on + (long long)y0 * p.oy + (long long)x0 * p.ox + lane * 16;
      for (int s = 0; s < nsteps; ++s) {
        while (__builtin_amdgcn_readfirstlane(flag_min8_asm(a_staged)) < s + 1) __builtin_amdgcn_s_sleep(1);
        uint4 v[NR];
#pragma unroll
        for (int r = 0; r < NR; ++r) v[r] = *(const uint4*)(sbase + (s % SG::NB) * SG::BYTES + r * 1024);
        asm volatile("s_waitcnt lgkmcnt(0)" ::: "memory");
        flag_store_asm(a_stored, s + 1);
        const int zo = zs + s * TZ + w;
        if (zo >= ze || (p.dbg & 4)) continue;
        char* dst = gbase + (long long)zo * p.oz;
#pragma unroll
        for (int r = 0; r < NR; ++r) *(uint4*)(dst + (long long)(r / QT) * p.oy + (r % QT) * 1024) = v[r];
      }
    } else {
      constexpr int NCH = 16 * QT;
      const int y = lane >> 3, xq = lane & 7;
      const char* sbase = smem + STAGEOFF + (w * TY + y) * (TX * 4) + xq * 16;
      float* gbase = p.out32 + (long long)n * p.pn + (long long)(y0 + y) * p.py + x0 + xq * 4;
      for (int s = 0; s < nsteps; ++s) {
        while (__builtin_amdgcn_readfirstlane(flag_min8_asm(a_staged)) < s + 1) __builtin_amdgcn_s_sleep(1);
        float4 v[NCH];
#pragma unroll
        for (int c = 0; c < NCH; ++c) v[c] = *(const float4*)(sbase + c * SG::CS);
        asm volatile("s_waitcnt lgkmcnt(0)" ::: "memory");
        flag_store_asm(a_stored, s + 1);
        const int zo = zs + s * TZ + w;
        if (zo >= ze || (p.dbg & 4)) continue;
        float* dst = gbase + (long long)zo * p.pz;
        if (p.wmap) {
          const float4 wg = *(const float4*)(p.wmap + ((long long)zo * p.H + y0 + y) * p.W + x0 + xq * 4);
#pragma unroll
          for (int c = 0; c < NCH; ++c) {
            const float4 old = *(const float4*)(dst + (long long)c * p.pc);
            v[c] = make_float4(old.x + wg.x * v[c].x, old.y + wg.y * v[c].y, old.z + wg.z * v[c].z, old.w + wg.w * v[c].w);
          }
        }
#pragma unroll
        for (int c = 0; c < NCH; ++c) *(float4*)(dst + (long long)c * p.pc) = v[c];
      }
    }
    return;
  }

  if constexpr (STEM) {
    if (wave >= NC) {
      typedef ZmStemCfg<TY, TX> SC;
      constexpr int RS = SC::RS, CPSZ = SC::CPSZ, IPLSZ = SC::IPLSZ, RC = SC::RC, RSTG = SC::RSTG, NLD = SC::NLD, IX = SC::IX, SW = SC::SW;
      constexpr int INOFF = STAGEOFF, STGOFF = STAGEOFF + RC * IPLSZ;
      int* landed = staged;
      int* inconv = stored;
      const int zlo = zs >= 2 ? zs - 2 : 0;
      const int zhi = ze + 1 <= p.D - 1 ? ze + 1 : p.D - 1;
      const int nin = zhi - zlo + 1;
      const char* src_n = si.src + (si.use_offs ? si.offs[n & 15] : (long long)n * si.sn);
      if (wave == NC + SC::NSW) {
        const int pr = lane / 10, pc = lane - pr * 10;
        const bool pvalid = lane < 60;
        int goff[2];
#pragma unroll
        for (int j = 0; j < 2; ++j) {
          int yy = y0 - 2 + pr + 6 * j, xx = x0 - 4 + 4 * pc;
          yy = yy < 0 ? 0 : (yy > p.H - 1 ? p.H - 1 : yy);
          xx = xx < 0 ? 0 : (xx > p.W - 4 ? p.W - 4 : xx);
          goff[j] = pvalid ? yy * (int)si.sy + xx * 4 : 0;
        }
        auto issue_plane = [&](int k) {
          const char* plane = src_n + (long long)(zlo + k) * si.sz;
          char* dstp = smem + STGOFF + (k % RSTG) * SC::STGSZ;
          if (pvalid) {
            __builtin_amdgcn_global_load_lds((gptr_t)(plane + goff[0]), (lptr_t)dstp, 16, 0, 0);
            __builtin_amdgcn_global_load_lds((gptr_t)(plane + goff[1]), (lptr_t)(dstp + 960), 16, 0, 0);
          }
        };
        int next_issue = 0, next_pub = 0, seen_conv = 0;
        const unsigned a_landed = lds_addr(landed);
        while (next_pub < nin) {
          while (next_issue < nin) {
            const int need = next_issue - RSTG + 1;
            if (seen_conv < need) seen_conv = __builtin_amdgcn_readfirstlane(flag_min8_asm(lds_addr(inconv)));
            if (seen_conv < need) break;
            issue_plane(next_issue++);
          }
          if (next_issue == next_pub) {
            __builtin_amdgcn_s_sleep(2);
            continue;
          }
          WaitVm<2, RSTG - 1>::run(next_issue - next_pub - 1);
          flag_store_asm(a_landed, ++next_pub);
        }
        return;
      }
      constexpr int NSW = SC::NSW;
      const int w = wave - NC;
      const int li = lane & 15, g = lane >> 4;
      const vec8 w0 = *(const vec8*)(si.wpk + 4096 + lane * 16);
      typedef __attribute__((ext_vector_type(2))) unsigned u32x2;
      typedef __attribute__((ext_vector_type(4))) unsigned u32x4;
      u32x2 w1 = *(const u32x2*)(si.wpk + 4096 + 1024 + lane * 16);
      if (g) w1 = u32x2{0u, 0u};
      const f32x4 sbias = si.bias ? *(const f32x4*)(si.bias + g * 4) : f32x4{0.f, 0.f, 0.f, 0.f};
      asm volatile("s_waitcnt vmcnt(0)" ::: "memory");
      const float lo_clip = si.act == ACT_RELU ? 0.f : -__builtin_inff();
      const int r0 = 2 * g, r1 = 2 * g + 1;
      const int kz0 = r0 / 3, kz1 = r1 / 3;
      auto xpart = [&](int hx) -> int {
        const int v0 = reflect_clamp(x0 + hx - 1, p.W) - (x0 - 2) - 1;
        return (v0 & 1) * CPSZ + (v0 & ~1) * 2;
      };
      auto ytop = [&](int hy) -> int { return reflect_clamp(y0 + hy - 1, p.H) - (y0 - 2) - 1; };
      const int xA = xpart(li), xB = xpart(16 + li);
      const int d0 = __builtin_amdgcn_readfirstlane((ytop(0) - 0) * RS), d9 = __builtin_amdgcn_readfirstlane((ytop(9) - 9) * RS);
      const int wlane = (g >> 1) * PPL + (g & 1) * 8 + li * 16;
      int croff[2], cwoff[2];
#pragma unroll
      for (int c = 0; c < 2; ++c) {
        const int crow = 8 * c + (li >> 1);
        const bool cvalid = crow < C::HY;
        const int crc = cvalid ? crow : 0;
        croff[c] = ytop(crc) * RS + xpart(32 + (li & 1));
        cwoff[c] = cvalid ? (g >> 1) * PPL + (g & 1) * 8 + (crow * HX + 32 + (li & 1)) * 16 : (g >> 1) * PPL + C::HVP * 16 + (g & 1) * 8;
      }
      constexpr int NB = 4;
      float vmax = 0.f;
      int seen_in = 0, seen_done = 0;
      int myk = w, seen_landed = 0, seen_ready = 0;
      bool ibad = false;
      auto convert_plane = [&](int k) {
        while (seen_landed < k + 1) {
          seen_landed = flag_load(landed);
          if (seen_landed < k + 1) __builtin_amdgcn_s_sleep(1);
        }
        const int need_done = zlo + k - RC + 3 - zs;
        while (seen_ready < need_done) {
          seen_ready = __builtin_amdgcn_readfirstlane(flag_min8_asm(lds_addr(ready)));
          if (seen_ready < need_done) __builtin_amdgcn_s_sleep(1);
        }
        asm volatile("" ::: "memory");
        const int so = (k % RSTG) * SC::STGSZ, dof = ((zlo + k) % RC) * IPLSZ;
        int lane_o = lane;
        asm volatile("" : "+v"(lane_o));
#pragma unroll
        for (int j = 0; j < NLD; ++j) {
          const int hv = j * 64 + lane_o;
          const bool valid = hv < SC::IVP;
          const int hvc = valid ? hv : SC::IVP - 1;
          const int iy = hvc / IX, ix = hvc - iy * IX;
          const int ry = reflect_clamp(y0 + iy - 2, p.H) - (y0 - 2), rx = reflect_clamp(x0 + ix - 2, p.W) - (x0 - 4);
          const float f = *(const float*)(smem + STGOFF + so + (ry * SW + rx) * 4);
          if (RangeCheck<T>::on) ibad |= RangeCheck<T>::bad(f);
          const unsigned short hb = to_bits<T>(f);
          const int la = valid ? iy * RS + ix * 2 : SC::DUMMY;
          const int lb = (valid && ix > 0) ? CPSZ + iy * RS + (ix - 1) * 2 : SC::DUMMY;
          *(unsigned short*)(smem + INOFF + dof + la) = hb;
          *(unsigned short*)(smem + INOFF + dof + lb) = hb;
        }
        asm volatile("" ::: "memory");
        flag_store(inconv + w, k + NSW);
      };
      for (int q = w; q < nplanes; q += NSW) {
        const int z1 = reflect_clamp(zs - 1 + q, p.D);
        int zi[3];
#pragma unroll
        for (int kz = 0; kz < 3; ++kz) zi[kz] = reflect_clamp(z1 - 1 + kz, p.D);
        int zmax = zi[0] > zi[1] ? zi[0] : zi[1];
        zmax = zmax > zi[2] ? zmax : zi[2];
        {
          int kmax = zs + q - zlo + SC::LEAD;
          kmax = kmax < nin - 1 ? kmax : nin - 1;
          for (; myk <= kmax; myk += NSW) convert_plane(myk);
        }
        while (seen_in < zmax - zlo + 1) {
          seen_in = __builtin_amdgcn_readfirstlane(flag_min8_asm(lds_addr(inconv)));
          if (seen_in < zmax - zlo + 1) __builtin_amdgcn_s_sleep(1);
        }
        while (q >= R + TZ * seen_done) {
          seen_done = __builtin_amdgcn_readfirstlane(flag_min8_asm(lds_addr(done)));
          if (q >= R + TZ * seen_done) __builtin_amdgcn_s_sleep(1);
        }
        asm volatile("" ::: "memory");
        int ib[3];
#pragma unroll
        for (int kz = 0; kz < 3; ++kz) ib[kz] = INOFF + (zi[kz] % RC) * IPLSZ;
        const int b0 = (kz0 == 0 ? ib[0] : (kz0 == 1 ? ib[1] : ib[2])) + (r0 % 3) * RS;
        const int b1 = (kz1 == 0 ? ib[0] : (kz1 == 1 ? ib[1] : ib[2])) + (r1 % 3) * RS;
        const int b8 = ib[2] + 2 * RS;
        int a0 = b0 + xA, a1 = b1 + xA, a8 = b8 + xA, c0 = b0 + xB, c1 = b1 + xB, c8 = b8 + xB;
        int wr = (q % R) * PLSZ + wlane;
        asm volatile("" : "+v"(a0), "+v"(a1), "+v"(a8), "+v"(c0), "+v"(c1), "+v"(c8), "+v"(wr));
        auto rd = [&](int addr) -> u32x2 {
          const unsigned* qq = (const unsigned*)(smem + addr);
          return u32x2{qq[0], qq[1]};
        };
        auto raddr = [&](int TI, int& r_0, int& r_1, int& r_8) {
          if (TI < 2 * C::HY) {
            const int row = TI >> 1, xt = TI & 1;
            const int d = (row == 0 ? d0 : (row == C::HY - 1 ? d9 : 0)) + row * RS;
            r_0 = (xt ? c0 : a0) + d; r_1 = (xt ? c1 : a1) + d; r_8 = (xt ? c8 : a8) + d;
          } else {
            const int c = TI - 2 * C::HY;
            r_0 = b0 + croff[c]; r_1 = b1 + croff[c]; r_8 = b8 + croff[c];
          }
        };
        auto waddr = [&](int TI) -> int {
          if (TI < 2 * C::HY) return wr + ((TI >> 1) * HX + 16 * (TI & 1)) * 16;
          return (q % R) * PLSZ + cwoff[TI - 2 * C::HY];
        };
        constexpr int NBT = (SC::NT + NB - 1) / NB;
        u32x4 fa[2][NB];
        u32x2 fe[2][NB];
        f32x4 sacc[2][NB];
        auto stage_a = [&](int bt) {
#pragma unroll
          for (int t = 0; t < NB; ++t) {
            if (bt * NB + t >= SC::NT) continue;
            int r_0, r_1, r_8;
            raddr(bt * NB + t, r_0, r_1, r_8);
            const u32x2 a = rd(r_0), bq = rd(r_1);
            fa[bt & 1][t] = u32x4{a[0], a[1], bq[0], bq[1]};
            fe[bt & 1][t] = rd(r_8);
          }
        };
        auto stage_b = [&](int bt) {
#pragma unroll
          for (int t = 0; t < NB; ++t)
            if (bt * NB + t < SC::NT) sacc[bt & 1][t] = Ops<T>::mfma(w0, __builtin_bit_cast(vec8, fa[bt & 1][t]), sbias);
#pragma unroll
          for (int t = 0; t < NB; ++t)
            if (bt * NB + t < SC::NT) sacc[bt & 1][t] = Ops<T>::mfma16(w1, fe[bt & 1][t], sacc[bt & 1][t]);
        };
        auto stage_c = [&](int bt) {
#pragma unroll
          for (int t = 0; t < NB; ++t) {
            if (bt * NB + t >= SC::NT) continue;
            float v[4];
#pragma unroll
            for (int j = 0; j < 4; ++j) v[j] = __builtin_amdgcn_fmed3f(sacc[bt & 1][t][j], lo_clip, __builtin_inff());
            if (RangeCheck<T>::on) {
              asm("v_max3_f32 %0, %1, |%2|, |%3|" : "=v"(vmax) : "v"(vmax), "v"(v[0]), "v"(v[1]));
              asm("v_max3_f32 %0, %1, |%2|, |%3|" : "=v"(vmax) : "v"(vmax), "v"(v[2]), "v"(v[3]));
            }
            *(uint2*)(smem + waddr(bt * NB + t)) = make_uint2(Ops<T>::pack2(v[0], v[1]), Ops<T>::pack2(v[2], v[3]));
          }
        };
        stage_a(0);
        if (NBT > 1) stage_a(1);
        __builtin_amdgcn_sched_barrier(0);
        stage_b(0);
        __builtin_amdgcn_sched_barrier(0);
#pragma unroll
        for (int bt = 0; bt < NBT; ++bt) {
          if (bt + 2 < NBT) stage_a(bt + 2);
          __builtin_amdgcn_sched_barrier(0);
          if (bt + 1 < NBT) stage_b(bt + 1);
          __builtin_amdgcn_sched_barrier(0);
          stage_c(bt);
          __builtin_amdgcn_sched_barrier(0);
        }
        asm volatile("" ::: "memory");
        flag_store(ready + w, q + NSW);
      }
      for (; myk < nin; myk += NSW) convert_plane(myk);
      if (RangeCheck<T>::on) raise_flag(p.oflow, ibad | !(vmax <= 65504.f));
      return;
    }
  }

  if (!STEM && wave >= NC) {
    static_assert(STEM || C::VMCNT_OK, "loader wave must not exceed the 6-bit vmcnt range");
    const int cp = wave - NC;
    int off[NDMA];
    bool valid[NDMA];
#pragma unroll
    for (int j = 0; j < NDMA; ++j) {
      const int hv = j * 64 + lane;
      const int hy = hv / HX, hx = hv - hy * HX;
      valid[j] = hv < C::HVP;
      off[j] = halo_coord(y0 + hy - 1, p.H, p.raw_halo) * (int)p.s0y + halo_coord(x0 + hx - 1, p.W, p.raw_halo) * (int)p.s0x + cp * 16;
    }
    const char* src_n = p.src0 + (long long)n * p.s0n;
    auto issue_plane = [&](int q) {
      const char* plane = src_n + (long long)halo_coord(zs - 1 + q, p.D, p.raw_halo) * p.s0z;
      char* dstp = smem + (q % R) * PLSZ + cp * PPL;
#pragma unroll
      for (int j = 0; j < NDMA; ++j)
        if (valid[j]) __builtin_amdgcn_global_load_lds((gptr_t)(plane + off[j]), (lptr_t)(dstp + j * 1024), 16, 0, 0);
    };
    int next_issue = 0, next_pub = 0;
    const unsigned a_ready = lds_addr(ready + cp), a_done = lds_addr(done);
    while (next_pub < nplanes) {
      if (next_issue < nplanes) {
        const int md = __builtin_amdgcn_readfirstlane(flag_min8_asm(a_done));
        int lim = R + TZ * md;
        lim = lim < nplanes ? lim : nplanes;
        while (next_issue < lim) issue_plane(next_issue++);
      }
      if (next_issue == next_pub) {
        __builtin_amdgcn_s_sleep(2);
        continue;
      }
      WaitVm<NDMA, R - 1>::run(next_issue - next_pub - 1);
      flag_store_asm(a_ready, ++next_pub);
    }
    return;
  }

  const int li = lane & 15, g = lane >> 4, hi = g >> 1;
  const int wq = wave / C::WPQ;
  const int wr = wave % C::WPQ;
  const int wrow = (wr / XT) * 2;
  const int wcx = wr % XT;
  vec8 wreg[NCKP][kSteps];
#pragma unroll
  for (int k = 0; k < NCKP; ++k)
#pragma unroll
    for (int s = 0; s < kSteps; ++s) wreg[k][s] = *(const vec8*)(p.wpk + ((k * kSteps + s) * QT + wq) * 1024 + lane * 16);
  const int cb = g * 4 * QT + wq * 4;
  f32x4 bias = f32x4{0.f, 0.f, 0.f, 0.f};
  if (p.bias) bias = *(const f32x4*)(p.bias + cb);
  asm volatile("s_waitcnt vmcnt(0)" ::: "memory");

  const int lanebase = (g & 1) * PPL + ((wrow * HX) + wcx * 16 + li) * 16;
  const int base_d1 = lanebase + hi * 16;
  const int base_dx = lanebase + hi * 16 * HX;
  const bool full_xy = (y0 + TY <= p.H) & (x0 + TX <= p.W);

  const int yl = y0 + wrow, xl = x0 + wcx * 16 + li;
  char* out_l = OUTMODE == 0 ? p.out + (long long)n * p.on + (long long)yl * p.oy + (long long)xl * p.ox + cb * 2 : nullptr;
  float* out32_l = OUTMODE == 1 ? p.out32 + (long long)n * p.pn + (long long)cb * p.pc + (long long)yl * p.py + xl : nullptr;
  constexpr bool WIDE = OUTMODE == 0 && NS == 0 && QT == 1;
  char* out_w = WIDE ? p.out + (long long)n * p.on + (long long)(yl + (g & 1)) * p.oy + (long long)xl * p.ox + (g >> 1) * 16 : nullptr;
  const bool vec_planar = OUTMODE == 1 && !(p.W & 3) && !(p.py & 3) && !(p.pz & 3) && !(p.pc & 3) && !(p.pn & 3) &&
                          !((size_t)p.out32 & 15) && !((size_t)p.wmap & 15);
  float* out32_q = OUTMODE == 1 ? p.out32 + (long long)n * p.pn + (long long)(cb + (li & 3)) * p.pc + (long long)yl * p.py +
                                      x0 + wcx * 16 + (li & ~3)
                                : nullptr;
  char* out2_l = (OUTMODE == 0 && POOL) ? p.out2 + (long long)n * p.qn + (long long)(yl >> 1) * p.qy +
                                               (long long)(xl >> 1) * p.qx + cb * 2
                                          : nullptr;

  bool bad = false;
  unsigned long long* trace = (p.dbg & 8) && (wave == 0 || wave == 4) && lane == 0 && blockIdx.x < 500
                                  ? (unsigned long long*)p.stats + ((long long)blockIdx.x * 2 + (wave >> 2)) * 128 : nullptr;
  int tcount = 0;
#define AMX_ZSTAMP()                                                             \
  do {                                                                           \
    if (trace && tcount < 128) trace[tcount] = __builtin_readcyclecounter();     \
    ++tcount;                                                                    \
  } while (0)
  AMX_ZSTAMP();
  for (int s = 0; s < nsteps; ++s) {
    {
      int need = TZ * s + TZ + 2;
      need = need < nplanes ? need : nplanes;
      static_assert(NL <= 4 && C::FLAGOFF % 16 == 0, "the ready flags are polled with one 16-byte read");
      if constexpr (STEM) {
        while (__builtin_amdgcn_readfirstlane(flag_min8_asm(lds_addr(ready))) < need) __builtin_amdgcn_s_sleep(1);
      } else {
        while (flag_min4<NL>(ready) < need) __builtin_amdgcn_s_sleep(1);
      }
      asm volatile("" ::: "memory");
    }

    AMX_ZSTAMP();
    int b1[4], bx3[4];
#pragma unroll
    for (int pl = 0; pl < 4; ++pl) {
      const int sl = ((s * TZ + pl) % R) * PLSZ;
      b1[pl] = base_d1 + sl;
      bx3[pl] = base_dx + sl;
    }
    f32x4 acc[2][2];
#pragma unroll
    for (int tz = 0; tz < 2; ++tz)
#pragma unroll
      for (int cy = 0; cy < 2; ++cy) acc[tz][cy] = bias;

    for (int rep = (p.dbg >> 10) & 7; rep >= 0; --rep)
    if (!(p.dbg & 2)) {
      if constexpr ((NCKP > 1 && !SPLIT) || STEM) {
        constexpr int PER = 4 * 6 + 8, NU = NCKP * PER, NSLOT = 4;
        int slo[4];
#pragma unroll
        for (int pl = 0; pl < 4; ++pl) slo[pl] = __builtin_amdgcn_readfirstlane(((s * TZ + pl) % R) * PLSZ);
        const int tail_lo = lanebase + (2 * HX + 2) * 16;
        auto src = [&](int i) -> const vec8* {
          const int ps = i / PER, j = i % PER, koff = ps * 2 * PPL;
          if (j < 24) {
            const int pl = j / 6, f = j % 6;
            return f < 4 ? (const vec8*)(smem + base_d1 + (slo[pl] + koff + (f * HX) * 16))
                         : (const vec8*)(smem + base_dx + (slo[pl] + koff + ((f - 4) * HX + 2) * 16));
          }
          const int t = j - 24, tz = t >> 2, cy = (t >> 1) & 1, which = t & 1;
          if (which) return (const vec8*)(smem + tail_lo + (slo[tz + 2] + koff + (cy * HX) * 16));
          return (const vec8*)(smem + tail_lo + ((hi ? slo[tz + 1] : slo[tz]) + koff + (cy * HX) * 16));
        };
        auto use = [&](int i, const vec8& frag) {
          const int ps = i / PER, j = i % PER;
          const int k = SPLIT ? 0 : ps;
          const bool both = SPLIT && ps == 0;
          auto mm = [&](const int widx, f32x4 a) {
            a = Ops<T>::mfma(wreg[k][widx], frag, a);
            if (both) a = Ops<T>::mfma(wreg[NCKP - 1][widx], frag, a);
            return a;
          };
          if (j < 24) {
            const int pl = j / 6, f = j % 6;
#pragma unroll
            for (int tz = 0; tz < 2; ++tz) {
              const int kz = pl - tz;
              if (kz < 0 || kz > 2) continue;
              if (f < 4) {
#pragma unroll
                for (int cy = 0; cy < 2; ++cy) {
                  const int ky = f - cy;
                  if (ky >= 0 && ky < 3) acc[tz][cy] = mm(kz * 3 + ky, acc[tz][cy]);
                }
              } else {
                acc[tz][f - 4] = mm(9 + kz, acc[tz][f - 4]);
              }
            }
          } else {
            const int t = j - 24, tz = t >> 2, cy = (t >> 1) & 1, which = t & 1;
            acc[tz][cy] = mm(12 + which, acc[tz][cy]);
          }
        };
        vec8 S[NSLOT];
#pragma unroll
        for (int i = 0; i < NSLOT; ++i) S[i] = *src(i);
#pragma clang loop unroll(full)
        for (int i = 0; i < NU; ++i) {
          use(i, S[i % NSLOT]);
          if (i + NSLOT < NU) S[i % NSLOT] = *src(i + NSLOT);
          __builtin_amdgcn_sched_barrier(0);
        }
      } else {
#pragma unroll
        for (int ps = 0; ps < NCKP; ++ps) {
          const int k = SPLIT ? 0 : ps;
          const bool both = SPLIT && ps == 0;
          const int koff = ps * 2 * PPL;
          auto mm = [&](const int widx, const vec8& frag, f32x4 a) {
            a = Ops<T>::mfma(wreg[k][widx], frag, a);
            if (both) a = Ops<T>::mfma(wreg[NCKP - 1][widx], frag, a);
            return a;
          };
          constexpr bool DB = NCKP == 1;
          vec8 F[DB ? 2 : 1][4], H[DB ? 2 : 1][2];
          auto load_plane = [&](int buf, int pl) {
  #pragma unroll
            for (int r = 0; r < 4; ++r) F[buf][r] = *(const vec8*)(smem + b1[pl] + koff + (r * HX) * 16);
  #pragma unroll
            for (int cy = 0; cy < 2; ++cy) H[buf][cy] = *(const vec8*)(smem + bx3[pl] + koff + (cy * HX + 2) * 16);
          };
          auto mma_plane = [&](int buf, int pl) {
  #pragma unroll
            for (int tz = 0; tz < 2; ++tz) {
              const int kz = pl - tz;
              if (kz < 0 || kz > 2) continue;
  #pragma unroll
              for (int ky = 0; ky < 3; ++ky)
  #pragma unroll
                for (int cy = 0; cy < 2; ++cy) acc[tz][cy] = mm(kz * 3 + ky, F[buf][cy + ky], acc[tz][cy]);
  #pragma unroll
              for (int cy = 0; cy < 2; ++cy) acc[tz][cy] = mm(9 + kz, H[buf][cy], acc[tz][cy]);
            }
          };
          if (DB) {
            load_plane(0, 0);
  #pragma unroll
            for (int pl = 0; pl < 4; ++pl) {
              if (pl + 1 < 4) load_plane((pl + 1) & 1, pl + 1);
              __builtin_amdgcn_sched_barrier(0);
              mma_plane(pl & 1, pl);
            }
          } else {
  #pragma unroll
            for (int pl = 0; pl < 4; ++pl) {
              load_plane(0, pl);
              mma_plane(0, pl);
            }
          }
  #pragma unroll
          for (int tz = 0; tz < 2; ++tz) {
            const int sl0 = ((s * TZ + tz) % R) * PLSZ, sl1 = ((s * TZ + tz + 1) % R) * PLSZ, sl2 = ((s * TZ + tz + 2) % R) * PLSZ;
            const int bz = lanebase + (hi ? sl1 : sl0) + koff + (2 * HX + 2) * 16;
            const int b0 = lanebase + sl2 + koff + (2 * HX + 2) * 16;
  #pragma unroll
            for (int cy = 0; cy < 2; ++cy) {
              const vec8 s0 = *(const vec8*)(smem + bz + (cy * HX) * 16);
              const vec8 s1 = *(const vec8*)(smem + b0 + (cy * HX) * 16);
              acc[tz][cy] = mm(12, s0, acc[tz][cy]);
              acc[tz][cy] = mm(13, s1, acc[tz][cy]);
            }
          }
        }
      }
      }
    asm volatile("s_waitcnt lgkmcnt(0)" ::: "memory");
    flag_store(done + wave, s + 1);
    AMX_ZSTAMP();

    if (p.dbg & 4) {
      if (NS) flag_store(staged + wave, s + 1);
      continue;
    }
    if constexpr (NS > 0) {
      if (s >= SG::NB)
        while (flag_min2(stored) < s + 1 - SG::NB) __builtin_amdgcn_s_sleep(1);
      asm volatile("" ::: "memory");
    }
    act_inplace<4>(&acc[0][0], p.act, p.slope);
    float pooled[4] = {-3.0e38f, -3.0e38f, -3.0e38f, -3.0e38f};
#pragma unroll
    for (int tz = 0; tz < 2; ++tz) {
      const int zo = zs + s * TZ + tz;
      if (WIDE && (SPLIT || !(p.dbg & 32))) {
        unsigned pk[2][2], pl[SPLIT ? 2 : 1][2];
#pragma unroll
        for (int cy = 0; cy < 2; ++cy) {
          float v[4];
#pragma unroll
          for (int j = 0; j < 4; ++j) {
            float f = acc[tz][cy][j];
              if (RangeCheck<T>::on) bad |= RangeCheck<T>::bad(f);
            v[j] = f;
            pooled[j] = f > pooled[j] ? f : pooled[j];
          }
          pk[cy][0] = (unsigned)to_bits<T>(v[0]) | ((unsigned)to_bits<T>(v[1]) << 16);
          pk[cy][1] = (unsigned)to_bits<T>(v[2]) | ((unsigned)to_bits<T>(v[3]) << 16);
          if constexpr (SPLIT) {
            float r[4];
#pragma unroll
            for (int j = 0; j < 4; ++j) r[j] = v[j] - (float)(T)v[j];
            pl[cy][0] = (unsigned)to_bits<T>(r[0]) | ((unsigned)to_bits<T>(r[1]) << 16);
            pl[cy][1] = (unsigned)to_bits<T>(r[2]) | ((unsigned)to_bits<T>(r[3]) << 16);
          }
        }
        const auto s0 = __builtin_amdgcn_permlane16_swap(pk[0][0], pk[1][0], false, false);
        const auto s1 = __builtin_amdgcn_permlane16_swap(pk[0][1], pk[1][1], false, false);
        unsigned l0a = 0, l0b = 0, l1a = 0, l1b = 0;
        if constexpr (SPLIT) {
          const auto t0 = __builtin_amdgcn_permlane16_swap(pl[0][0], pl[1][0], false, false);
          const auto t1 = __builtin_amdgcn_permlane16_swap(pl[0][1], pl[1][1], false, false);
          l0a = t0[0]; l0b = t0[1]; l1a = t1[0]; l1b = t1[1];
        }
        if (zo >= ze) continue;
        if (!full_xy && !((yl + (g & 1) < p.H) & (xl < p.W))) continue;
        *(uint4*)(out_w + (long long)zo * p.oz) = make_uint4(s0[0], s1[0], s0[1], s1[1]);
        if constexpr (SPLIT) *(uint4*)(out_w + (long long)zo * p.oz + p.Cout * 2) = make_uint4(l0a, l1a, l0b, l1b);
        continue;
      }
#pragma unroll
      for (int cy = 0; cy < 2; ++cy) {
        float v[4];
#pragma unroll
        for (int j = 0; j < 4; ++j) {
          float f = acc[tz][cy][j];
          if (OUTMODE == 0 && RangeCheck<T>::on) bad |= RangeCheck<T>::bad(f);
          v[j] = f;
          pooled[j] = f > pooled[j] ? f : pooled[j];
        }
        if constexpr (NS > 0) {
          if (OUTMODE == 0) {
            char* dst = smem + STAGEOFF + (s % SG::NB) * SG::BYTES + (((tz * TY + wrow + cy) * TX) + wcx * 16 + li) * SG::CB + cb * 2;
            *(uint2*)dst = make_uint2((unsigned)to_bits<T>(v[0]) | ((unsigned)to_bits<T>(v[1]) << 16),
                                      (unsigned)to_bits<T>(v[2]) | ((unsigned)to_bits<T>(v[3]) << 16));
          } else {
            quad_transpose4(v, li);
            char* dst = smem + STAGEOFF + (cb + (li & 3)) * SG::CS + ((tz * TY + wrow + cy) * TX + wcx * 16 + (li & ~3)) * 4;
            *(float4*)dst = make_float4(v[0], v[1], v[2], v[3]);
          }
          continue;
        }
        if (zo >= ze) continue;
        if (!full_xy && !((yl + cy < p.H) & (xl < p.W))) continue;
        if (OUTMODE == 0) {
          char* dst = out_l + (long long)zo * p.oz + cy * p.oy;
          *(uint2*)dst = make_uint2((unsigned)to_bits<T>(v[0]) | ((unsigned)to_bits<T>(v[1]) << 16),
                                    (unsigned)to_bits<T>(v[2]) | ((unsigned)to_bits<T>(v[3]) << 16));
        } else if (vec_planar) {
          quad_transpose4(v, li);
          float* dst = out32_q + (long long)zo * p.pz + cy * p.py;
          float4 o = make_float4(v[0], v[1], v[2], v[3]);
          if (p.wmap) {
            const float4 wg = *(const float4*)(p.wmap + ((long long)zo * p.H + yl + cy) * p.W + x0 + wcx * 16 + (li & ~3));
            const float4 old = *(const float4*)dst;
            o = make_float4(old.x + wg.x * o.x, old.y + wg.y * o.y, old.z + wg.z * o.z, old.w + wg.w * o.w);
          }
          *(float4*)dst = o;
        } else {
          float* dst = out32_l + (long long)zo * p.pz + cy * p.py;
          if (p.wmap) {
            const float wgt = p.wmap[((long long)zo * p.H + yl + cy) * p.W + xl];
#pragma unroll
            for (int j = 0; j < 4; ++j) dst[(long long)j * p.pc] += wgt * v[j];
          } else {
#pragma unroll
            for (int j = 0; j < 4; ++j) dst[(long long)j * p.pc] = v[j];
          }
        }
      }
    }
    if constexpr (NS > 0) {
      asm volatile("" ::: "memory");
      flag_store(staged + wave, s + 1);
    }
    if constexpr (OUTMODE == 0 && POOL) {
      float pm[4];
#pragma unroll
      for (int j = 0; j < 4; ++j) {
        const float o = dpp_quad<0xB1>(pooled[j]);
        pm[j] = pooled[j] > o ? pooled[j] : o;
      }
      const int zp = (zs + s * TZ) >> 1;
      if (!(li & 1) && zs + s * TZ + 1 < ze && (full_xy || ((yl + 1 < p.H) & (xl + 1 < p.W)))) {
        char* dst = out2_l + (long long)zp * p.qz;
        *(uint2*)dst = make_uint2((unsigned)to_bits<T>(pm[0]) | ((unsigned)to_bits<T>(pm[1]) << 16),
                                  (unsigned)to_bits<T>(pm[2]) | ((unsigned)to_bits<T>(pm[3]) << 16));
        if constexpr (SPLIT) {
          float r[4];
#pragma unroll
          for (int j = 0; j < 4; ++j) r[j] = pm[j] - (float)(T)pm[j];
          *(uint2*)(dst + p.Cout * 2) = make_uint2((unsigned)to_bits<T>(r[0]) | ((unsigned)to_bits<T>(r[1]) << 16),
                                                   (unsigned)to_bits<T>(r[2]) | ((unsigned)to_bits<T>(r[3]) << 16));
        }
      }
    }
    AMX_ZSTAMP();
  }
  if (OUTMODE == 0 && RangeCheck<T>::on) raise_flag(p.oflow, bad);
}

template <typename T, int NCK, int QT, int TY, int R, int OUTMODE, int NS, bool POOL = false, bool SPLIT = false, int TX = 32, bool STEM = false>
static hipError_t launch_zm_ns(ConvParams p, hipStream_t st, ConvLaunchInfo* info, const StemIn& si = StemIn{}) {
  if constexpr (OUTMODE == 0 && NS == 0 && !POOL && !STEM)
    if (p.out2) return launch_zm_ns<T, NCK, QT, TY, R, OUTMODE, NS, true, SPLIT, TX, STEM>(p, st, info, si);
  constexpr int TZ = 2;
  typedef ZmCfg<SPLIT ? 2 : NCK, QT, TY, TX, R> C;
  constexpr int LDS = STEM ? C::FLAGOFF + 128 + ZmStemCfg<TY, TX>::BYTES : NS ? C::FLAGOFF + 128 + ZmStage<QT, TY, TX, OUTMODE>::TOTAL : C::LDS_BYTES;
  if (info && STEM)
    info->report(0, "conv3d_k3_zmarch<%s,stem1->16->16,%dx%dx%d,c8+st%d+ld1,r%d/%d%s>", __is_same(T, f16) ? "f16" : "bf16", TZ, TY, TX,
                 ZmStemCfg<TY, TX>::NSW, R, ZmStemCfg<TY, TX>::RC, p.out2 ? ",pool" : "");
  else if (info)
    info->report(0, "conv3d_k3_zmarch<%s%s,%d->%d,%dx%dx%d,c8+l%d+s%d,r%d,o%d%s>", __is_same(T, f16) ? "f16" : "bf16", SPLIT ? "x2" : "",
                 16 * NCK, 16 * QT, TZ, TY, TX, C::NL, NS, R, OUTMODE, p.out2 ? ",pool" : "");
  auto kern = conv3d_k3_zmarch_kernel<T, NCK, QT, TY, TX, R, OUTMODE, NS, POOL, SPLIT, STEM>;
  static amx::DeviceOnce attr_once;
  if (!attr_once.done()) {
    hipError_t e = hipFuncSetAttribute((const void*)kern, hipFuncAttributeMaxDynamicSharedMemorySize, LDS);
    if (e != hipSuccess) return e;
    attr_once.set();
  }
  p.nby = (p.H + TY - 1) / TY;
  p.nbx = (p.W + TX - 1) / TX;
  const int tiles = p.nby * p.nbx * p.N;
  int nseg, zseg;
  pick_z_segments(tiles, p.D, TZ, 256 * (LDS <= 80 * 1024 ? 2 : 1), &zseg, &nseg);
  hipLaunchKernelGGL(kern, dim3((unsigned)(tiles * nseg)), dim3((8 + (STEM ? ZmStemCfg<TY, TX>::NSW + 1 : C::NL) + NS) * 64), LDS, st, p, zseg, nseg, si);
  return hipGetLastError();
}

template <int TY>
static bool zm_can_stage(const ConvParams& p) {
  if (p.H % TY || p.W % 32) return false;
  return !((size_t)p.out32 & 3) && !((size_t)p.wmap & 3);
}

template <typename T, int NCK, int QT, int TY, int R, int OUTMODE>
static hipError_t launch_zm(const ConvParams& p, hipStream_t st, ConvLaunchInfo* info) {
  if constexpr (NCK == 1 && OUTMODE == 1)
    if (zm_can_stage<TY>(p)) return launch_zm_ns<T, NCK, QT, TY, R, OUTMODE, 2>(p, st, info);
  return launch_zm_ns<T, NCK, QT, TY, R, OUTMODE, 0>(p, st, info);
}

bool conv_zmarch_eligible(const ConvParams& p) {
  if (p.src0_f32c1 || p.C1 != 0 || p.W < 32 || p.H < 8 || p.D < 8) return false;
  if (p.C0 == 16 && p.Cout == 16) return true;
  if (p.out32) return false;
  return (p.C0 == 16 || p.C0 == 32) && p.Cout == 32;
}

bool conv_zmarch_can_pool(const ConvParams& p) {
  return conv_zmarch_eligible(p) && !p.out32 && !(p.D & 1) && !(p.H & 1) && !(p.W & 1);
}

bool conv_zmarch_eligible_split(const ConvParams& p) {
  return conv_zmarch_eligible(p) && p.C0 == 16 && p.Cout == 16;
}
bool conv_zmarch_can_pool_split(const ConvParams& p) { return conv_zmarch_can_pool(p) && conv_zmarch_eligible_split(p); }

bool conv_zmarch_stem_eligible(const ConvParams& p, int precision) {
  return precision < 2 && p.C0 == 16 && p.C1 == 0 && p.Cout == 16 && !p.out32 && !p.raw_halo && p.W >= 32 && !(p.W % 32) && !(p.H % 8) &&
         !(p.D & 1) && p.D >= 8 && p.ox == 32 && (p.ocs == 0 || p.ocs == 32);
}
hipError_t launch_conv_zmarch_stem(const ConvParams& p, const float* x, long long xs_n, long long xs_z, long long xs_y, const long long* x_offs,
                                   const void* stem_wpk, const float* stem_bias, int stem_act, float stem_slope, int precision, hipStream_t st,
                                   ConvLaunchInfo* info) {
  if (stem_act != ACT_NONE && stem_act != ACT_RELU) return hipErrorInvalidValue;
  if ((precision != 0 && precision != 1) || (x_offs && p.N > 16)) return hipErrorInvalidValue;
  StemIn si;
  memset(&si, 0, sizeof si);
  si.src = (const char*)x; si.sn = xs_n; si.sz = xs_z; si.sy = xs_y;
  if (x_offs) {
    si.use_offs = 1;
    for (int i = 0; i < p.N; ++i) si.offs[i] = x_offs[i] * 4;
  }
  si.wpk = (const char*)stem_wpk; si.bias = stem_bias; si.act = stem_act; si.slope = stem_slope;
  if (precision == 0) return launch_zm_ns<f16, 1, 1, 8, 10, 0, 0, false, false, 32, true>(p, st, info, si);
  return launch_zm_ns<bf16, 1, 1, 8, 10, 0, 0, false, false, 32, true>(p, st, info, si);
}

hipError_t launch_conv_zmarch(const ConvParams& p, int precision, hipStream_t st, ConvLaunchInfo* info) {
  const bool planar = p.out32 != nullptr;
  if (precision >= 2) {
    if (p.C0 != 16 || p.Cout != 16) return hipErrorInvalidValue;
    if (precision == 2) return planar ? launch_zm_ns<f16, 1, 1, 8, 7, 1, 0, false, true>(p, st, info) : launch_zm_ns<f16, 1, 1, 8, 7, 0, 0, false, true>(p, st, info);
    return planar ? launch_zm_ns<bf16, 1, 1, 8, 7, 1, 0, false, true>(p, st, info) : launch_zm_ns<bf16, 1, 1, 8, 7, 0, 0, false, true>(p, st, info);
  }
  if (p.Cout == 16) {
    if (precision == 0) return planar ? launch_zm<f16, 1, 1, 8, 10, 1>(p, st, info) : launch_zm<f16, 1, 1, 8, 10, 0>(p, st, info);
    return planar ? launch_zm<bf16, 1, 1, 8, 10, 1>(p, st, info) : launch_zm<bf16, 1, 1, 8, 10, 0>(p, st, info);
  }
  if (p.C0 == 16) return precision == 0 ? launch_zm<f16, 1, 2, 4, 10, 0>(p, st, info) : launch_zm<bf16, 1, 2, 4, 10, 0>(p, st, info);
  return precision == 0 ? launch_zm<f16, 2, 2, 4, 10, 0>(p, st, info) : launch_zm<bf16, 2, 2, 4, 10, 0>(p, st, info);
}

}
```

anatomix_amd/csrc/amx_device.h:

```cpp
#pragma once
#include "amx_common.h"

namespace amx {

template <typename T> struct Ops;
typedef __attribute__((ext_vector_type(2))) unsigned amx_u32x2;
template <> struct Ops<f16> {
  typedef f16x8 vec8;
  static __device__ __forceinline__ f32x4 mfma(vec8 a, vec8 b, f32x4 c) {
    return __builtin_amdgcn_mfma_f32_16x16x32_f16(a, b, c, 0, 0, 0);
  }
  static __device__ __forceinline__ f32x4 mfma16(amx_u32x2 a, amx_u32x2 b, f32x4 c) {
    typedef __attribute__((ext_vector_type(4))) _Float16 h4;
    return __builtin_amdgcn_mfma_f32_16x16x16f16(__builtin_bit_cast(h4, a), __builtin_bit_cast(h4, b), c, 0, 0, 0);
  }
  static __device__ __forceinline__ unsigned pack2(float a, float b) {
    typedef __attribute__((ext_vector_type(2))) float f2;
    typedef __attribute__((ext_vector_type(2))) _Float16 h2;
    return __builtin_bit_cast(unsigned, __builtin_convertvector(f2{a, b}, h2));
  }
};
template <> struct Ops<bf16> {
  typedef bf16x8 vec8;
  static __device__ __forceinline__ f32x4 mfma(vec8 a, vec8 b, f32x4 c) {
    return __builtin_amdgcn_mfma_f32_16x16x32_bf16(a, b, c, 0, 0, 0);
  }
  static __device__ __forceinline__ f32x4 mfma16(amx_u32x2 a, amx_u32x2 b, f32x4 c) {
    typedef __attribute__((ext_vector_type(4))) short s4;
    return __builtin_amdgcn_mfma_f32_16x16x16bf16_1k(__builtin_bit_cast(s4, a), __builtin_bit_cast(s4, b), c, 0, 0, 0);
  }
  static __device__ __forceinline__ unsigned pack2(float a, float b) {
    typedef __attribute__((ext_vector_type(2))) float f2;
    typedef __attribute__((ext_vector_type(2))) __bf16 b2;
    return __builtin_bit_cast(unsigned, __builtin_convertvector(f2{a, b}, b2));
  }
};

template <typename T> struct RangeCheck {
  static constexpr bool on = false;
  static __device__ __forceinline__ bool bad(float) { return false; }
};
template <> struct RangeCheck<f16> {
  static constexpr bool on = true;
  static __device__ __forceinline__ bool bad(float v) { return !(__builtin_fabsf(v) <= 65504.f); }
};
__device__ __forceinline__ void raise_flag(int* flag, bool bad) {
  if (bad && flag) __atomic_store_n(flag, 1, __ATOMIC_RELAXED);
}

__device__ __forceinline__ int reflect_clamp(int g, int n) {
  g = g < 0 ? -g : g;
  g = g >= n ? 2 * n - 2 - g : g;
  g = g < 0 ? 0 : g;
  return g >= n ? n - 1 : g;
}

__device__ __forceinline__ int halo_coord(int g, int n, int raw) {
  if (raw) return g < -1 ? -1 : (g > n ? n : g);
  return reflect_clamp(g, n);
}

typedef __attribute__((ext_vector_type(8))) int i32x8;
constexpr float kMxLoScale = 2048.f;
__device__ __forceinline__ unsigned e4m3_pk4(float a, float b, float c, float d) {
  a = __builtin_amdgcn_fmed3f(a, -448.f, 448.f);
  b = __builtin_amdgcn_fmed3f(b, -448.f, 448.f);
  c = __builtin_amdgcn_fmed3f(c, -448.f, 448.f);
  d = __builtin_amdgcn_fmed3f(d, -448.f, 448.f);
  int v = __builtin_amdgcn_cvt_pk_fp8_f32(a, b, 0, false);
  v = __builtin_amdgcn_cvt_pk_fp8_f32(c, d, v, true);
  return (unsigned)v;
}
__device__ __forceinline__ void mx_split8(const float (&f)[8], uint2& xl8, uint2& xh8) {
  float h[8], l[8];
#pragma unroll
  for (int e = 0; e < 8; ++e) {
    h[e] = (float)(_Float16)f[e];
    l[e] = (float)(_Float16)(f[e] - h[e]) * kMxLoScale;
  }
  xl8 = make_uint2(e4m3_pk4(l[0], l[1], l[2], l[3]), e4m3_pk4(l[4], l[5], l[6], l[7]));
  xh8 = make_uint2(e4m3_pk4(h[0], h[1], h[2], h[3]), e4m3_pk4(h[4], h[5], h[6], h[7]));
}

__device__ __forceinline__ void mx_split8_direct(const float (&f)[8], uint2& xl8, uint2& xh8) {
  float h[8], l[8];
#pragma unroll
  for (int e = 0; e < 8; ++e) {
    h[e] = (float)(_Float16)f[e];
    l[e] = (f[e] - h[e]) * kMxLoScale;
  }
  xl8 = make_uint2(e4m3_pk4(l[0], l[1], l[2], l[3]), e4m3_pk4(l[4], l[5], l[6], l[7]));
  xh8 = make_uint2(e4m3_pk4(h[0], h[1], h[2], h[3]), e4m3_pk4(h[4], h[5], h[6], h[7]));
}

__device__ __forceinline__ unsigned dpp_xor1(unsigned v) {
  return (unsigned)__builtin_amdgcn_update_dpp(0, (int)v, 0xB1, 0xF, 0xF, true);
}
__device__ __forceinline__ void mx_store_copies(char* chunk, int odd, const float (&f)[8]) {
  uint2 xl8, xh8;
  mx_split8(f, xl8, xh8);
  const uint2 send = odd ? xl8 : xh8;
  const unsigned r0 = dpp_xor1(send.x), r1 = dpp_xor1(send.y);
  *(uint4*)(chunk + odd * 16) = odd ? make_uint4(r0, r1, xh8.x, xh8.y) : make_uint4(xl8.x, xl8.y, r0, r1);
}

template <typename T>
__device__ __forceinline__ unsigned short to_bits(float v) {
  T t = (T)v;
  return __builtin_bit_cast(unsigned short, t);
}

template <int CTRL>
__device__ __forceinline__ float dpp_quad(float x) {
  return __builtin_bit_cast(float, __builtin_amdgcn_update_dpp(0, __builtin_bit_cast(int, x), CTRL, 0xF, 0xF, true));
}
__device__ __forceinline__ void quad_transpose4(float (&v)[4], int lane_in_quad_bits) {
  const bool b0 = lane_in_quad_bits & 1, b1 = lane_in_quad_bits & 2;
  const float r01 = dpp_quad<0xB1>(b0 ? v[0] : v[1]);
  const float r23 = dpp_quad<0xB1>(b0 ? v[2] : v[3]);
  if (b0) { v[0] = r01; v[2] = r23; } else { v[1] = r01; v[3] = r23; }
  const float r02 = dpp_quad<0x4E>(b1 ? v[0] : v[2]);
  const float r13 = dpp_quad<0x4E>(b1 ? v[1] : v[3]);
  if (b1) { v[0] = r02; v[1] = r13; } else { v[2] = r02; v[3] = r13; }
}

__device__ __forceinline__ int flag_load(const int* p) {
  return __atomic_load_n(p, __ATOMIC_RELAXED);
}
__device__ __forceinline__ void flag_store(int* p, int v) {
  __atomic_store_n(p, v, __ATOMIC_RELAXED);
}

__device__ __forceinline__ unsigned lds_addr(const void* p) {
  return (unsigned)(size_t)(__attribute__((address_space(3))) const void*)p;
}
template <int N>
__device__ __forceinline__ void act_inplace(f32x4* a, int act, float slope) {
  if (act == ACT_RELU) {
#pragma unroll
    for (int i = 0; i < N; ++i)
#pragma unroll
      for (int j = 0; j < 4; ++j) a[i][j] = a[i][j] > 0.f ? a[i][j] : 0.f;
  } else if (act == ACT_LRELU) {
#pragma unroll
    for (int i = 0; i < N; ++i)
#pragma unroll
      for (int j = 0; j < 4; ++j) a[i][j] = a[i][j] > 0.f ? a[i][j] : a[i][j] * slope;
  }
}

__device__ __forceinline__ float act_k(int act, float slope) { return act == ACT_RELU ? 0.f : (act == ACT_LRELU ? slope : 1.f); }
__device__ __forceinline__ float act_fwd(float v, float k) { return (v > 0.f ? v : v * k) + 0.f; }
__device__ __forceinline__ float act_bwd(float dz, float y, float k) {
  const float m = y > 0.f ? 1.f : k;
  return m == 0.f ? 0.f : dz * m;
}

#pragma clang diagnostic push
#pragma clang diagnostic ignored "-Winline-asm"
__device__ __forceinline__ void dma16_asm(const void* g, unsigned lds_base) {
  asm volatile("s_mov_b32 m0, %1\n\ts_nop 0\n\tglobal_load_lds_dwordx4 %0, off" ::"v"(g), "s"(lds_base) : "memory", "m0");
}
#pragma clang diagnostic pop
__device__ __forceinline__ void flag_store_asm(unsigned addr, int v) {
  asm volatile("ds_write_b32 %0, %1" ::"v"(addr), "v"(v) : "memory");
}
__device__ __forceinline__ int flag_load_asm(unsigned addr) {
  int r;
  asm volatile("ds_read_b32 %0, %1\n\ts_waitcnt lgkmcnt(0)" : "=v"(r) : "v"(addr) : "memory");
  return r;
}

typedef __attribute__((ext_vector_type(4))) int flag4_t;
__device__ __forceinline__ flag4_t flag_read4(const int* p) {
  flag4_t a;
  asm volatile("ds_read_b128 %0, %1\n\ts_waitcnt lgkmcnt(0)" : "=v"(a) : "v"(lds_addr(p)) : "memory");
  return a;
}
__device__ __forceinline__ int flag_min2(const int* p) {
  typedef __attribute__((ext_vector_type(2))) int i32x2;
  i32x2 a;
  asm volatile("ds_read_b64 %0, %1\n\ts_waitcnt lgkmcnt(0)" : "=v"(a) : "v"(lds_addr(p)) : "memory");
  return __builtin_amdgcn_readfirstlane(a[0] < a[1] ? a[0] : a[1]);
}
template <int N>
__device__ __forceinline__ int flag_min4(const int* p) {
  typedef __attribute__((ext_vector_type(4))) int i32x4;
  i32x4 a;
  asm volatile("ds_read_b128 %0, %1\n\ts_waitcnt lgkmcnt(0)" : "=v"(a) : "v"(lds_addr(p)) : "memory");
  int m = a[0];
#pragma unroll
  for (int i = 1; i < N; ++i) m = a[i] < m ? a[i] : m;
  return __builtin_amdgcn_readfirstlane(m);
}

__device__ __forceinline__ int flag_min8_asm(unsigned addr) {
  typedef __attribute__((ext_vector_type(4))) int i32x4;
  i32x4 a, b;
  asm volatile("ds_read_b128 %0, %2\n\tds_read_b128 %1, %2 offset:16\n\ts_waitcnt lgkmcnt(0)"
               : "=&v"(a), "=&v"(b)
               : "v"(addr)
               : "memory");
  int m0 = a[0] < a[1] ? a[0] : a[1], m1 = a[2] < a[3] ? a[2] : a[3];
  int m2 = b[0] < b[1] ? b[0] : b[1], m3 = b[2] < b[3] ? b[2] : b[3];
  m0 = m0 < m1 ? m0 : m1;
  m2 = m2 < m3 ? m2 : m3;
  return m0 < m2 ? m0 : m2;
}

template <int PER, int I>
struct WaitVm {
  static __device__ __forceinline__ void run(int k) {
    if (k == I) {
      asm volatile("s_waitcnt vmcnt(%0)" ::"n"(I * PER) : "memory");
    } else {
      WaitVm<PER, I - 1>::run(k);
    }
  }
};
template <int PER>
struct WaitVm<PER, -1> {
  static __device__ __forceinline__ void run(int) {}
};

template <int I>
struct WaitVmDyn {
  static __device__ __forceinline__ void run(int n) {
    if (n >= I) {
      asm volatile("s_waitcnt vmcnt(%0)" ::"n"(I) : "memory");
    } else {
      WaitVmDyn<I - 1>::run(n);
    }
  }
};
template <>
struct WaitVmDyn<0> {
  static __device__ __forceinline__ void run(int) { asm volatile("s_waitcnt vmcnt(0)" ::: "memory"); }
};
__device__ __forceinline__ void wait_vmcnt_dyn(int n) { WaitVmDyn<63>::run(n); }


__device__ __forceinline__ float identity_coord(int i, int n) {
  if (n <= 1) return 0.f;
  const float step = 2.f / (float)(n - 1);
  const float lin = i < n / 2 ? __fmaf_rn(step, (float)i, -1.f) : __fmaf_rn(-step, (float)(n - 1 - i), 1.f);
  return __fdiv_rn(lin * (float)(n - 1), (float)n);
}

}
```

include/anatomix_amd.h:

```cpp
#ifndef ANATOMIX_AMD_H
#define ANATOMIX_AMD_H

#include <stddef.h>
#include <stdint.h>

#ifdef __cplusplus
extern "C" {
#endif

#define AMX_VERSION 100

typedef enum amx_status {
  AMX_OK = 0,
  AMX_ERR_INVALID = -1,
  AMX_ERR_SHAPE = -2,
  AMX_ERR_NOT_LOADED = -3,
  AMX_ERR_WORKSPACE = -4,
  AMX_ERR_HIP = -5,
  AMX_ERR_OVERFLOW = -6
} amx_status;

enum { AMX_NORM_NONE = 0, AMX_NORM_BATCH_EVAL = 1, AMX_NORM_INSTANCE = 2, AMX_NORM_INSTANCE_AFFINE = 3 };
enum { AMX_ACT_NONE = 0, AMX_ACT_RELU = 1, AMX_ACT_LRELU = 2 };
enum { AMX_POOL_MAX = 0, AMX_POOL_AVG = 1 };
enum { AMX_INTERP_NEAREST = 0, AMX_INTERP_TRILINEAR = 1 };
enum { AMX_PREC_F16 = 0, AMX_PREC_BF16 = 1, AMX_PREC_F16X2 = 2, AMX_PREC_BF16X2 = 3, AMX_PREC_F16X2_MX = 4 };

typedef struct amx_unet_cfg {
  int32_t input_nc;
  int32_t output_nc;
  int32_t num_downs;
  int32_t ngf;
  int32_t norm;
  float norm_eps;
  int32_t activation;
  float act_slope;
  int32_t final_act;
  int32_t pooling;
  int32_t interp;
  int32_t doubleconv;
  int32_t use_skip;
  int32_t precision;
} amx_unet_cfg;

typedef struct amx_unet amx_unet_t;

int amx_version(void);

int amx_debug_fill_lds(unsigned pattern, void* stream);
const char* amx_last_error(void);

int amx_unet_create(amx_unet_t** out, const amx_unet_cfg* cfg);
void amx_unet_destroy(amx_unet_t* h);

int amx_unet_num_modules(const amx_unet_t* h);
int amx_unet_num_convs(const amx_unet_t* h);
int amx_unet_conv_info(const amx_unet_t* h, int conv, int* module_idx, int* cin, int* cout, int* norm_module_idx);

int amx_unet_load_conv(amx_unet_t* h, int module_idx, const float* d_weight, const float* d_bias,
                       const float* d_gamma, const float* d_beta, const float* d_mean,
                       const float* d_var, void* stream);

typedef struct amx_launch_record {
  char kernel[64];
  int32_t module_idx;
  int32_t cin, cout;
  int32_t n, d, h, w;
  float ms;
  double flops;
  double bytes;
} amx_launch_record;

size_t amx_unet_workspace_bytes(const amx_unet_t* h, int n, int d, int w_h, int w_w);

int amx_unet_forward(amx_unet_t* h, const float* d_x, float* d_y, int n, int d, int hh, int w,
                     void* d_workspace, size_t workspace_bytes, void* stream);

int amx_unet_numerics_status(amx_unet_t* h, int synchronize, void* stream);

int amx_unet_module_info(const amx_unet_t* h, int module_idx, int* channels, int* level);

int amx_unet_forward_taps(amx_unet_t* h, const float* d_x, float* d_y, int n, int d, int hh, int w,
                          void* d_workspace, size_t workspace_bytes, const int* tap_modules, int n_taps,
                          float* const* d_tap_out, int stop_module, void* stream);

int amx_unet_forward_profiled(amx_unet_t* h, const float* d_x, float* d_y, int n, int d, int hh, int w,
                              void* d_workspace, size_t workspace_bytes, void* stream,
                              amx_launch_record* records, int max_records, int* n_records);

int amx_unet_forward_window(amx_unet_t* h, const float* d_vol, int vd, int vh, int vw, int oz, int oy,
                            int ox, int rd, int rh, int rw, const float* d_wmap, float* d_acc,
                            void* d_workspace, size_t workspace_bytes, void* stream);

int amx_unet_forward_windows(amx_unet_t* h, const float* d_vol, int vd, int vh, int vw, int n_windows,
                             const int* offsets_zyx, int rd, int rh, int rw, const float* d_wmap, float* d_acc,
                             void* d_workspace, size_t workspace_bytes, void* stream);

int amx_unet_forward_windows_pipelined(amx_unet_t* h, const float* d_vol, int vd, int vh, int vw, int n_windows,
                                       const int* offsets_zyx, int rd, int rh, int rw, const float* d_wmap, float* d_acc,
                                       void* d_workspace, size_t workspace_bytes, int slot, void* stream);

int amx_sw_normalize(float* d_acc, const float* d_cnt, int channels, long long voxels, void* stream);

int amx_sw_count(float* d_cnt, int vd, int vh, int vw, int oz, int oy, int ox, int rd, int rh, int rw,
                 const float* d_wmap, void* stream);

typedef enum amx_sw_map { AMX_SW_MAP_CONSTANT = 0, AMX_SW_MAP_GAUSSIAN = 1 } amx_sw_map;
typedef enum amx_sw_out {
  AMX_SW_FEATURES = 0,
  AMX_SW_LOGITS = 1,
  AMX_SW_LABELS = 2
} amx_sw_out;

int amx_sw_plan(int vd, int vh, int vw, int rd, int rh, int rw, double overlap, int* offsets_zyx, int capacity);

int amx_sw_importance_map(float* d_wmap, int rd, int rh, int rw, int mode, double sigma_scale, void* stream);

int amx_sw_count_all(float* d_cnt, int vd, int vh, int vw, int rd, int rh, int rw, double overlap, const float* d_wmap,
                     void* stream);

int amx_sw_finish(int kind, float* d_acc, const float* d_cnt, int feat, long long voxels, const float* d_w, const float* d_b,
                  int classes, void* d_out, void* stream);

size_t amx_sliding_window_workspace_bytes(const amx_unet_t* h, int n_batch, int rd, int rh, int rw);

int amx_sliding_window(amx_unet_t* h, const float* d_vol, int vd, int vh, int vw, int rd, int rh, int rw, double overlap,
                       int mode, double sigma_scale, int n_batch, int out_kind, const float* d_w, const float* d_b,
                       int classes, float* d_acc, float* d_cnt, void* d_out, void* d_workspace, size_t workspace_bytes,
                       void* stream);

size_t amx_conv3d_packed_bytes(int cin, int cout);
int amx_conv3d_k3_reflect(const void* d_x0, int c0, const void* d_x1, int c1, const float* d_weight,
                          const float* d_scale, const float* d_shift, int cout, int n, int d, int hh,
                          int w, int act, float slope, int precision, void* d_wpk, void* d_out16,
                          float* d_out32, void* stream);

size_t amx_conv3d_scratch_bytes(int c0, int c1, int cout, int n, int d, int hh, int w, int precision);
int amx_conv3d_k3_reflect_ws(const void* d_x0, int c0, const void* d_x1, int c1, const float* d_weight,
                             const float* d_scale, const float* d_shift, int cout, int n, int d, int hh,
                             int w, int act, float slope, int precision, void* d_wpk, void* d_out16,
                             float* d_out32, void* d_scratch, size_t scratch_bytes, void* stream);

int amx_conv3d_k3_reflect_ex(const void* d_x0, int c0, const void* d_x1, int c1, const float* d_weight, int weight_mode,
                             int cin_real, int cout_real, const float* d_scale, const float* d_shift, int cout, int n,
                             int d, int hh, int w, int act, float slope, int precision, void* d_wpk, void* d_out16,
                             float* d_out32, void* stream);

#define AMX_WEIGHTS_PREPACKED 16
typedef struct amx_pack_req {
  const float* d_weight;
  void* d_wpk;
  int weight_mode, cin_real, cin_pad, cout_real, cout, w;
} amx_pack_req;
int amx_conv3d_pack_batch(const amx_pack_req* reqs, int count, int precision, void* stream);

int amx_conv3d_dgrad_interior_supported(int c_dy, int cout, int d, int hh, int w, int precision);
int amx_conv3d_dgrad_interior(const void* d_dy_framed, int c_dy, const float* d_weight, int weight_flags, int cin_real, int cout_real, int cout,
                              int n, int d, int hh, int w, int precision, void* d_wpk, void* d_out16, void* stream);
size_t amx_conv3d_dgrad_shell_scratch_bytes(void);
int amx_conv3d_dgrad_fold_shell(const void* d_dy_framed, int c_dy, const float* d_weight, int co_real, int ci_real, void* d_dx, int c_dx, int n,
                                int d, int hh, int w, int precision, void* d_scratch, void* stream);

int amx_pool2(const void* d_in, void* d_out, int n, int d_out_, int h_out, int w_out, int c, int avg,
              int precision, void* stream);

size_t amx_instance_norm_scratch_bytes(int n, int c);
int amx_instance_norm(void* d_x, const float* d_gamma, const float* d_beta, float eps, int n, long long voxels,
                      int c, int act, float slope, void* d_scratch, int precision, void* stream);

int amx_upsample2_trilinear(const void* d_in, void* d_out, int n, int din, int hin, int win, int c,
                            int precision, void* stream);

int amx_upcat_split_backward(const void* d_dcat, void* d_dskip, void* d_dlow, int n, int dlow, int hlow, int wlow, int c0, int c1,
                             int accumulate_skip, int precision, void* stream);
int amx_upcat_split_backward_framed(const void* d_g_framed, void* d_dskip, void* d_dlow, int n, int dlow, int hlow, int wlow, int c0,
                                    int c1, int accumulate_skip, int precision, void* stream);

int amx_import_input(const float* d_src, void* d_dst, int n, int cin, int d, int hh, int w, int precision, void* stream);
int amx_export_ncdhw(const void* d_src, int c, int n, int d, int hh, int w, float* d_out, int precision, void* stream);
int amx_import_ncdhw(const float* d_src, void* d_dst, int n, int c, int d, int hh, int w, long long dst_sn, long long dst_sz,
                     long long dst_sy, long long dst_sx, int accumulate, int precision, void* stream);

int amx_upsample2_trilinear_backward(const void* d_gout, void* d_gin, int n, int din, int hin, int win, int c, int precision,
                                     void* stream);

size_t amx_conv3d_upcat_merged_packed_bytes(int c0, int c1, int cout);
int amx_conv3d_upcat_merged(const void* d_x0, int c0, const void* d_x1, int c1, const float* d_weight, const float* d_scale,
                            const float* d_shift, int cout, int n, int d, int hh, int w, int act, float slope, int precision,
                            void* d_wpk, void* d_partial, void* d_out16, void* stream);

size_t amx_train_scratch_bytes(int c);

int amx_bn_train_forward(const void* d_x, void* d_y, const float* d_gamma, const float* d_beta, float eps, int n,
                         long long voxels, int c, int act, float slope, void* d_scratch, float* d_save_mean,
                         float* d_save_rstd, float* d_running_mean, float* d_running_var, float momentum, int precision,
                         void* stream);

int amx_bn_act_backward(const void* d_dy, const void* d_y, const void* d_x, const float* d_mean, const float* d_rstd,
                        const float* d_gamma, float* d_dgamma, float* d_dbeta, void* d_dx_framed, int n, int d, int hh, int w,
                        int c, int act, float slope, void* d_scratch, int precision, void* stream);
int amx_bn_act_backward_recompute(const void* d_dy, const void* d_x, const float* d_mean, const float* d_rstd, const float* d_gamma,
                                  const float* d_beta, float* d_dgamma, float* d_dbeta, void* d_dx_framed, int n, int d, int hh, int w,
                                  int c, int act, float slope, void* d_scratch, int precision, void* stream);

int amx_pad_fold(const void* d_g_framed, void* d_din, int n, int d, int hh, int w, int c, int accumulate, int precision,
                 void* stream);

int amx_pool2_max_backward(const void* d_dp, const void* d_in, void* d_din, int n, int dout, int hout, int wout, int c,
                           int accumulate, int precision, void* stream);

size_t amx_conv3d_wgrad_scratch_bytes(int n, int d, int hh, int w, int cout, int cin_pad);
int amx_conv3d_wgrad(const void* d_dy, long long dy_sn, long long dy_sz, long long dy_sy, long long dy_sx, const void* d_x0,
                     int c0, const void* d_x1, int c1, int cin_real, int cout, int n, int d, int hh, int w, float* d_dw,
                     int accumulate, void* d_scratch, size_t scratch_bytes, int precision, void* stream);

size_t amx_attention_scratch_bytes(int b, int heads, int n, int head_dim);
int amx_attention_qknorm_rope(const float* d_q, const float* d_k, const float* d_v, const float* d_qn_w, const float* d_qn_b,
                              const float* d_kn_w, const float* d_kn_b, float norm_eps, const float* d_rope, int n_prefix, int b,
                              int n, int heads, int head_dim, float* d_out, void* d_scratch, size_t scratch_bytes, void* stream);

int amx_attention_prepared(const void* d_scratch, size_t scratch_bytes, int b, int n, int heads, int head_dim, float* d_out, void* stream);

typedef struct amx_vit_cfg {
  int32_t input_channels;
  int32_t num_classes;
  int32_t embed_dim;
  int32_t depth;
  int32_t heads;
  int32_t num_register_tokens;
  int32_t grid_d, grid_h, grid_w;
  int32_t hidden;
  int32_t dec1, dec2;
  int32_t qk_norm;
  int32_t scale_attn_inner;
  int32_t layer_scale;
  float in_eps;
  int32_t out_norm;
  int32_t decoder_split;
  int32_t stem_split;
} amx_vit_cfg;
typedef struct amx_vit amx_vit_t;

int amx_vit_create(amx_vit_t** out, const amx_vit_cfg* cfg);
void amx_vit_destroy(amx_vit_t* h);
int amx_vit_num_params(const amx_vit_t* h);
const char* amx_vit_param_name(const amx_vit_t* h, int idx);
int amx_vit_load(amx_vit_t* h, const float* const* d_params, int count, const float* d_rope, void* stream);
size_t amx_vit_workspace_bytes(const amx_vit_t* h, int n);
int amx_vit_forward(amx_vit_t* h, const float* d_x, float* d_y, int n, void* d_ws, size_t ws_bytes, int n_blocks, void* stream);
int amx_vit_debug_read(amx_vit_t* h, const char* name, void* d_dst, size_t max_bytes, size_t* bytes, void* stream);
int amx_linear(const float* d_x, const float* d_w, const float* d_b, int m, int k, int n, int split, float* d_y, void* stream);

size_t amx_supcon_scratch_bytes(int n, int c);
int amx_supcon_loss(const float* d_feat, const int* d_labels, int n, int c, float temperature, int weigh_rarity,
                    int balance_denominator, int sqrt_mode, float* d_loss, float* d_grad, void* d_scratch,
                    size_t scratch_bytes, void* stream);

int amx_mlp_head_forward(const float* d_x, int n, int cin, int width, int n_layers, const float* const* w,
                         const float* const* gamma, const float* const* beta, float* const* running_mean,
                         float* const* running_var, float eps, float momentum, int act, float slope, float* d_z, float* d_y,
                         float* d_mean, float* d_rstd, void* stream);

size_t amx_mlp_head_scratch_bytes(int n, int cin, int width);
int amx_mlp_head_backward(const float* d_dy, const float* d_x, int n, int cin, int width, int n_layers,
                          const float* const* w, const float* const* gamma, int act, float slope, const float* d_z,
                          const float* d_y, const float* d_mean, const float* d_rstd, float* const* dw, float* const* dgamma,
                          float* const* dbeta, float* d_dx, void* d_scratch, size_t scratch_bytes, void* stream);

size_t amx_conv3d_backward_sampled_scratch_bytes(int p);
int amx_conv3d_backward_sampled(const float* d_grows, const long long* d_coords, const void* d_x, int x_channels, const float* d_w, int n,
                                int p, int d, int hh, int w, int cout, int cin, float* d_dw, void* d_din, int din_channels, void* d_scratch,
                                size_t scratch_bytes, int precision, void* stream);

int amx_mlp_heads_forward(int n_heads, const float* const* d_x, int n, const int* cin, int width, int n_layers, const float* const* w,
                          const float* const* gamma, const float* const* beta, float* const* running_mean, float* const* running_var,
                          float eps, float momentum, int act, float slope, float* const* d_z, float* const* d_y, float* const* d_mean,
                          float* const* d_rstd, void* stream);
int amx_mlp_heads_backward(int n_heads, const float* const* d_dy, const float* const* d_x, int n, const int* cin, int width, int n_layers,
                           const float* const* w, const float* const* gamma, int act, float slope, const float* const* d_z,
                           const float* const* d_y, const float* const* d_mean, const float* const* d_rstd, float* const* dw,
                           float* const* dgamma, float* const* dbeta, float* const* d_dx, void* const* d_scratch, size_t scratch_bytes,
                           void* stream);
int amx_supcon_loss_batch(int n_losses, const float* const* d_feat, const int* const* d_labels, int n, int c, float temperature,
                          int weigh_rarity, int balance_denominator, int sqrt_mode, float* const* d_loss, float* const* d_grad,
                          void* d_scratch, size_t scratch_bytes, void* stream);
int amx_gather_labels_batch(const float* d_seg, int sd, int sh, int sw, int n_maps, const long long* const* d_coords, int p, const int* dims,
                            int views, int* const* d_labels, void* stream);

int amx_gather_rows(const void* d_src, int dtype, long long src_sn, long long src_sz, long long src_sy, long long src_sx, long long src_sc,
                    const long long* d_coords, int n, int p, int c, float* d_rows, void* stream);
int amx_scatter_rows(const float* d_rows, const long long* d_coords, void* d_dst, int precision, long long dst_sn, long long dst_sz,
                     long long dst_sy, long long dst_sx, int n, int p, int c, int accumulate, void* stream);

int amx_sample_coords(const long long* d_draws, int n_draws, int num, int d0, int d1, int d2, long long* d_coords, void* stream);
int amx_sample_perm(const long long* d_keys, int d0, int d1, int d2, int num, long long* d_coords, void* stream);
int amx_gather_labels(const float* d_seg, int sd, int sh, int sw, const long long* d_coords, int p, int d, int hh, int w, int views,
                      int* d_labels, void* stream);

typedef struct {
  void* param;
  const void* grad;
  void* exp_avg;
  void* exp_avg_sq;
  const void* step;
  long long numel;
} amx_adamw_tensor;
int amx_adamw_step(const amx_adamw_tensor* tensors, int count, double lr, double beta1, double beta2, double eps,
                   double weight_decay, int maximize, void* stream);
int amx_adamw_step_dev(const amx_adamw_tensor* tensors, int count, const double* d_hyper, int maximize, void* stream);
int amx_adamw_step_clip_dev(const amx_adamw_tensor* tensors, int count, const double* d_hyper, int maximize, const float* d_total_norm,
                            double max_norm, void* stream);
typedef struct {
  const void* grad;
  long long numel;
  long long group;
} amx_grad_tensor;
size_t amx_grad_norms_scratch_bytes(const amx_grad_tensor* tensors, int count, int groups);
int amx_grad_norms(const amx_grad_tensor* tensors, int count, int groups, float* d_out, void* d_scratch, size_t scratch_bytes,
                   void* stream);


size_t amx_mindssc_scratch_bytes(int H, int W, int D);
int amx_mindssc(const float* d_img, int H, int W, int D, int radius, int dilation, float* d_out, void* d_scratch,
                size_t scratch_bytes, void* stream);

int amx_avg_pool3d_cat(const float* d_a, int ca, float scale_a, const float* d_b, int cb, float scale_b, int H, int W, int D,
                       int g, float* d_out, void* stream);

int amx_box_filter3d(const float* d_in, float* d_out, int c, int H, int W, int D, int k, void* stream);

size_t amx_correlate_scratch_bytes(int h, int w, int d, int disp_hw);
int amx_correlate_ssd(const float* d_fix, const float* d_mov, int c, int h, int w, int d, int disp_hw, float* d_ssd,
                      long long* d_argmin, void* d_scratch, size_t scratch_bytes, void* stream);


size_t amx_coupled_convex_scratch_bytes(int h, int w, int d);
int amx_coupled_convex(const float* d_ssd, const long long* d_argmin, int h, int w, int d, int disp_hw, float* d_disp_soft,
                       void* d_scratch, size_t scratch_bytes, void* stream);

size_t amx_coupled_convex_step_scratch_bytes(int h, int w, int d);
int amx_coupled_convex_step(const float* d_ssd, const float* d_soft_hist, int j, int h, int w, int d, int disp_hw,
                            float* d_soft_out, long long* d_label, void* d_scratch, size_t scratch_bytes, void* stream);

size_t amx_inverse_consistency_scratch_bytes(int h, int w, int d);
int amx_inverse_consistency(const float* d_field1, const float* d_field2, int h, int w, int d, int iterations, float* d_out1,
                            float* d_out2, void* d_scratch, size_t scratch_bytes, void* stream);

int amx_resize_trilinear3d(const float* d_in, int c, int h, int w, int d, float* d_out, int H, int W, int D, const float* scale,
                           int flip_channels, void* stream);

size_t amx_stage1_registration_scratch_bytes(int h, int w, int d, int disp_hw, int ic);
int amx_stage1_registration(const float* d_feat_fix, const float* d_feat_mov, int n_ch, int h, int w, int d, int disp_hw,
                            int grid_sp, int ic, int H, int W, int D, float* d_disp_out, void* d_scratch, size_t scratch_bytes,
                            void* stream);


int amx_instance_opt_smooth3(const float* d_in, float* d_out, int h, int w, int d, void* stream);

size_t amx_instance_opt_scratch_bytes(int c, int h, int w, int d);
int amx_instance_opt_grad(const float* d_weight, const float* d_fix, const float* d_mov, int c, int h, int w, int d, float lambda,
                          float* d_grad_weight, float* d_disp_sample, float* d_loss2, void* d_scratch, size_t scratch_bytes,
                          void* stream);

int amx_instance_opt_adam_step(float* d_weight, const float* d_grad, float* d_exp_avg, float* d_exp_avg_sq, long long n, double lr,
                               int t, void* stream);

int amx_instance_opt(float* d_weight_io, const float* d_fix, const float* d_mov, int c, int h, int w, int d, float lambda, double lr,
                     int niter, float* d_fitted, void* d_scratch, size_t scratch_bytes, void* stream);

size_t amx_run_instance_opt_scratch_bytes(int c, int H, int W, int D, int grid_sp_adam, int selected_smooth);
int amx_run_instance_opt(const float* d_disp_hr, const float* d_feat_fix, const float* d_feat_mov, int c, int H, int W, int D,
                         int grid_sp_adam, float lambda, int niter, int selected_smooth, double lr, float* d_out, void* d_scratch,
                         size_t scratch_bytes, void* stream);

enum { AMX_WARP_BILINEAR = 0, AMX_WARP_NEAREST = 1 };
int amx_warp3d(const float* d_vol, int c, const float* d_disp, int H, int W, int D, int mode, float* d_out, void* stream);

enum { AMX_SEG_LABEL_F32 = 0, AMX_SEG_LABEL_I64 = 1, AMX_SEG_LABEL_U8 = 2 };

size_t amx_seg_loss_scratch_bytes(int n, long long voxels, int classes, int feat);

int amx_seg_loss_forward(const float* d_in, int feat, const float* d_w, const float* d_b, const void* d_labels, int label_dtype, int n,
                         int classes, long long voxels, int include_background, float smooth_nr, float smooth_dr, float lambda_dice,
                         float lambda_ce, float* d_loss, float* d_stats, long long* d_bad_labels, void* d_scratch,
                         size_t scratch_bytes, void* stream);

int amx_seg_loss_backward(const float* d_in, int feat, const float* d_w, const float* d_b, const void* d_labels, int label_dtype, int n,
                          int classes, long long voxels, int include_background, float smooth_nr, float smooth_dr, float lambda_dice,
                          float lambda_ce, const float* d_stats, const float* d_gout, float* d_dx, float* d_dw, float* d_db,
                          void* d_scratch, size_t scratch_bytes, void* stream);

int amx_seg_argmax(const float* d_in, int feat, const float* d_w, const float* d_b, int n, int classes, long long voxels,
                   unsigned char* d_out, void* stream);


int amx_label_overlap(const void* d_a, int dtype_a, const void* d_b, int dtype_b, long long voxels, int bins, long long* d_counts,
                      long long* d_bad, void* stream);

size_t amx_jacobian_det_scratch_bytes(int H, int W, int D);
int amx_jacobian_det(const float* d_disp, int H, int W, int D, int add_identity, float* d_jdet, float* d_stats, void* d_scratch,
                     size_t scratch_bytes, void* stream);

enum {
  AMX_SEGAUG_NOISE = 1,
  AMX_SEGAUG_BIAS = 2,
  AMX_SEGAUG_GIBBS = 4,
  AMX_SEGAUG_CONTRAST = 8,
  AMX_SEGAUG_SMOOTH = 16,
  AMX_SEGAUG_SHARPEN = 32,
  AMX_SEGAUG_AFFINE = 64,
  AMX_SEGAUG_RESCALE = 128
};
enum { AMX_SEGAUG_OP_SCALE = 0, AMX_SEGAUG_OP_CONTRAST = 1 };
enum { AMX_SEGAUG_GAUSS_SMOOTH = 0, AMX_SEGAUG_GAUSS_SHARPEN = 1 };

typedef struct amx_segaug_sample {
  const float* vol;
  const void* lab;
  int32_t flags;
  int32_t vol_dim[3];
  int32_t corner[3];
  float noise_std;
  float bias[20];
  float gibbs_r;
  float gamma;
  int32_t radius[3][3];
  float taps[3][3][9];
  float sharpen_alpha;
  float affine[9];
} amx_segaug_sample;

size_t amx_segaug_sample_bytes(void);
size_t amx_segaug_scratch_bytes(int n, long long voxels);

int amx_segaug_minmax(const float* d_x, int n, long long voxels, float* d_minmax, void* d_scratch, size_t scratch_bytes, void* stream);
int amx_segaug_minmax_finalize(const void* d_scratch, size_t scratch_bytes, int n, long long voxels, float* d_minmax, void* stream);

int amx_segaug_pointwise(const float* d_in, float* d_out, int n, long long voxels, const float* d_minmax, int op,
// ... 138 lines not shown
```

Baseline: 2988 volumes/s.

## Specialize conv epilogues on activation, add fast full-tile store path

Turns the activation into a template parameter for the z-march and upcat conv kernels, so activation runs as compile-time code (fmed3 for ReLU) instead of a runtime branch. The epilogue is split into a fast path for full tiles without bounds checks and a checked path. Stores use 32-bit offsets from a marching z base pointer, and the per-element f16 overflow check becomes a bitwise running max. Debug flag branches are removed. It also adds a probe API entry and int32 offset guards, at the cost of more template instantiations and code size.

```diff
diff --git a/anatomix_amd/_lib.py b/anatomix_amd/_lib.py
--- a/anatomix_amd/_lib.py
+++ b/anatomix_amd/_lib.py
@@ -86,6 +86,7 @@
                                 C.c_size_t, _P]),
     "amx_conv3d_packed_bytes": (C.c_size_t, [_I, _I]),
     "amx_conv3d_k3_reflect": (_I, [_P, _I, _P, _I, _P, _P, _P, _I, _I, _I, _I, _I, _I, C.c_float, _I, _P, _P, _P, _P]),
+    "amx_conv3d_k3_reflect_probe": (_I, [_P, _I, _P, _I, _P, _P, _P, _I, _I, _I, _I, _I, _I, C.c_float, _I, _P, _P, _P, _P, _P, _P, _P, _P]),
     "amx_conv3d_dgrad_interior_supported": (_I, [_I, _I, _I, _I, _I, _I]),
     "amx_conv3d_dgrad_interior": (_I, [_P, _I, _P, _I, _I, _I, _I, _I, _I, _I, _I, _I, _P, _P, _P]),
     "amx_conv3d_dgrad_shell_scratch_bytes": (C.c_size_t, []),
diff --git a/anatomix_amd/csrc/amx_api.hip b/anatomix_amd/csrc/amx_api.hip
--- a/anatomix_amd/csrc/amx_api.hip
+++ b/anatomix_amd/csrc/amx_api.hip
@@ -103,10 +103,17 @@
   return 2 * bytes + 256;
 }
 
+struct ConvProbe {
+  void* pool16;
+  const float* wmap;
+  int* oflow;
+  char* kernel;
+};
+
 static int conv3d_single(const void* d_x0, int c0, const void* d_x1, int c1, const float* d_weight, int weight_mode,
                          int cin_real, int cout_real, const float* d_scale, const float* d_shift, int cout, int n, int d,
                          int hh, int w, int act, float slope, int precision, void* d_wpk, void* d_out16, float* d_out32,
-                         void* stream, void* d_scratch = nullptr, size_t scratch_bytes = 0) {
+                         void* stream, void* d_scratch = nullptr, size_t scratch_bytes = 0, const ConvProbe* probe = nullptr) {
   if (!d_x0 || (!d_weight && !(weight_mode & AMX_WEIGHTS_PREPACKED)) || !d_wpk || (!d_out16 == !d_out32)) return fail(AMX_ERR_INVALID, "bad pointer arguments");
   if (c0 % 16 || c1 % 16 || c0 + c1 < 16 || cout % 16 || cout < 16)
     return fail(AMX_ERR_INVALID, "channel counts must be multiples of 16 (c0=%d c1=%d cout=%d)", c0, c1, cout);
@@ -146,13 +153,25 @@
     p.out32 = d_out32;
     p.py = w; p.pz = (long long)hh * w; p.pc = p.pz * d; p.pn = p.pc * cout;
   }
+  amx::ConvLaunchInfo info{};
+  amx::ConvLaunchInfo* const want = probe ? &info : nullptr;
+  if (probe) {
+    p.wmap = probe->wmap;
+    p.oflow = probe->oflow;
+    if (probe->wmap && !d_out32) return fail(AMX_ERR_INVALID, "the importance map belongs to the fp32 planar output");
+    if (probe->pool16) {
+      if (!d_out16 || !amx::conv_zmarch_can_pool(p)) return fail(AMX_ERR_SHAPE, "the fused max-pool needs a z-march layer with even extents");
+      amx::set_out2(p, probe->pool16, cout, d / 2, hh / 2, w / 2, precision);
+    }
+  }
   if (!is_split(precision) && weight_mode == 0 && cin_real == 48 && c0 == 16 && c1 == 32 && cout == 16 && amx::conv_upcat16_eligible(p)) {
     if (prepacked)
       return fail(AMX_ERR_INVALID, "prepacked weights: the 16 + up32 -> 16 merged-tap layer packs its own format (call without the flag)");
     char* up = (char*)d_wpk + ((size_t)cout * (c0 + c1) * 28 * 2 + 255) / 256 * 256;
     AMX_HIP(amx::launch_pack_upcat16(d_weight, d_scale, up, precision, st));
     p.wpk = up;
-    AMX_HIP(amx::launch_conv_upcat16(p, precision, st));
+    AMX_HIP(amx::launch_conv_upcat16(p, precision, st, want));
+    if (probe && probe->kernel) memcpy(probe->kernel, info.name, sizeof info.name);
     return AMX_OK;
   }
   if (d_scratch && !c1 && d_out16) {
@@ -161,7 +180,8 @@
       return fail(AMX_ERR_WORKSPACE, "split-K scratch needs %zu bytes, 16-byte aligned (got %zu)", need, scratch_bytes);
     if (need) p.part = (float*)d_scratch;
   }
-  AMX_HIP(amx::launch_conv(p, precision, q, st));
+  AMX_HIP(amx::launch_conv(p, precision, q, st, want));
+  if (probe && probe->kernel) memcpy(probe->kernel, info.name, sizeof info.name);
   return AMX_OK;
 }
 
@@ -244,6 +264,15 @@
                              void* d_scratch, size_t scratch_bytes, void* stream) {
   return conv3d_single(d_x0, c0, d_x1, c1, d_weight, 0, c0 + c1, cout, d_scale, d_shift, cout, n, d, hh, w, act, slope,
                        precision, d_wpk, d_out16, d_out32, stream, d_scratch, scratch_bytes);
+}
+
+int amx_conv3d_k3_reflect_probe(const void* d_x0, int c0, const void* d_x1, int c1, const float* d_weight, const float* d_scale,
+                                const float* d_shift, int cout, int n, int d, int hh, int w, int act, float slope, int precision,
+                                void* d_wpk, void* d_out16, float* d_out32, void* d_pool16, const float* d_wmap, int* d_oflow,
+                                char* kernel_name, void* stream) {
+  const ConvProbe probe{d_pool16, d_wmap, d_oflow, kernel_name};
+  return conv3d_single(d_x0, c0, d_x1, c1, d_weight, 0, c0 + c1, cout, d_scale, d_shift, cout, n, d, hh, w, act, slope,
+                       precision, d_wpk, d_out16, d_out32, stream, nullptr, 0, &probe);
 }
 
 int amx_conv3d_k3_reflect(const void* d_x0, int c0, const void* d_x1, int c1, const float* d_weight,
diff --git a/anatomix_amd/csrc/amx_conv3d_upcat.hip b/anatomix_amd/csrc/amx_conv3d_upcat.hip
--- a/anatomix_amd/csrc/amx_conv3d_upcat.hip
+++ b/anatomix_amd/csrc/amx_conv3d_upcat.hip
@@ -30,7 +30,7 @@
   static_assert(R * NDMA <= 60 && RL * NDMAL <= 60, "vmcnt range");
 };
 
-template <typename T, int OUTMODE>
+template <typename T, int OUTMODE, int ACT>
 __global__ __launch_bounds__((UpcatCfg::NC + UpcatCfg::NL) * 64) void conv3d_upcat16_kernel(const ConvParams p, int zseg,
                                                                                            int nseg) {
   typedef UpcatCfg C;
@@ -169,12 +169,55 @@
 
   const bool full_xy = (y0 + TY <= p.H) & (x0 + TX <= p.W);
   const int yl = y0 + py, xl = x0 + 2 * li + px;
-  char* out_l = OUTMODE == 0 ? p.out + (long long)n * p.on + (long long)yl * p.oy + (long long)xl * p.ox + g * 8 : nullptr;
-  char* out_w = OUTMODE == 0 ? p.out + (long long)n * p.on + (long long)yl * p.oy + (long long)xl * p.ox + (g >> 1) * 16 : nullptr;
+  const unsigned lo_w = OUTMODE == 0 ? (unsigned)((yl + 2 * (g & 1)) * (int)p.oy + xl * (int)p.ox + (g >> 1) * 16) : 0u;
+  char* zb = OUTMODE == 0 ? p.out + (long long)n * p.on + (long long)(zs + pz) * p.oz : nullptr;
+  const bool ok_w0 = full_xy || ((yl + 2 * (g & 1) < p.H) & (xl < p.W)), ok_w1 = full_xy || ((yl + 2 * (2 + (g & 1)) < p.H) & (xl < p.W));
   float* out32_l = OUTMODE == 1 ? p.out32 + (long long)n * p.pn + (long long)(g * 4) * p.pc + (long long)yl * p.py + xl
                                 : nullptr;
-
-  bool bad = false;
+  const bool fast = OUTMODE == 0 && full_xy;
+  unsigned amax = 0;
+
+  auto epilogue = [&](auto fast_c, const int s, f32x4 (&acc)[4]) {
+    constexpr bool FAST = decltype(fast_c)::value != 0;
+    const int zo = zs + 2 * s + pz;
+    act_values<ACT, 4>(&acc[0], p.slope);
+    if constexpr (OUTMODE == 0) {
+      unsigned ow = lo_w;
+      asm volatile("" : "+v"(ow));
+#pragma unroll
+      for (int cp = 0; cp < 2; ++cp) {
+        unsigned pk[2][2];
+#pragma unroll
+        for (int h = 0; h < 2; ++h) {
+          const f32x4 v = acc[2 * cp + h];
+          if (RangeCheck<T>::on) {
+            amax = RangeCheck<T>::template track<ACT == ACT_RELU>(amax, v[0], v[1]);
+            amax = RangeCheck<T>::template track<ACT == ACT_RELU>(amax, v[2], v[3]);
+          }
+          pk[h][0] = Ops<T>::pack2(v[0], v[1]);
+          pk[h][1] = Ops<T>::pack2(v[2], v[3]);
+        }
+        const auto s0 = __builtin_amdgcn_permlane16_swap(pk[0][0], pk[1][0], false, false);
+        const auto s1 = __builtin_amdgcn_permlane16_swap(pk[0][1], pk[1][1], false, false);
+        if (FAST || (zo < ze && (cp ? ok_w1 : ok_w0))) *(uint4*)(zb + (cp ? 4 * p.oy : 0) + ow) = make_uint4(s0[0], s1[0], s0[1], s1[1]);
+      }
+    } else if (zo < ze) {
+#pragma unroll
+      for (int c = 0; c < 4; ++c) {
+        if (!full_xy && !((yl + 2 * c < p.H) & (xl < p.W))) continue;
+        float* dst = out32_l + (long long)zo * p.pz + (2 * c) * p.py;
+        if (p.wmap) {
+          const float wgt = p.wmap[((long long)zo * p.H + yl + 2 * c) * p.W + xl];
+#pragma unroll
+          for (int j = 0; j < 4; ++j) dst[(long long)j * p.pc] += wgt * acc[c][j];
+        } else {
+#pragma unroll
+          for (int j = 0; j < 4; ++j) dst[(long long)j * p.pc] = acc[c][j];
+        }
+      }
+    }
+  };
+
   for (int s = 0; s < nsteps; ++s) {
     {
       int need = 2 * s + 4, needl = s + 3;
@@ -188,7 +231,6 @@
       }
       asm volatile("" ::: "memory");
     }
-    const int zo = zs + 2 * s + pz;
     int slo[3], llo[2];
 #pragma unroll
     for (int kz = 0; kz < 3; ++kz) slo[kz] = __builtin_amdgcn_readfirstlane(((2 * s + pz + kz) % R) * PLSZ);
@@ -200,7 +242,7 @@
 #pragma unroll
     for (int c = 0; c < 4; ++c) acc[c] = bias;
 
-    if (!(p.dbg & 2)) {
+    {
       constexpr int NSK = 4 * kSteps, NU = NSK + 4 * 8, NSLOT = 8;
       auto src = [&](int i) -> const vec8* {
         if (i < NSK) {
@@ -232,59 +274,11 @@
     asm volatile("s_waitcnt lgkmcnt(0)" ::: "memory");
     flag_store(done + wave, s + 1);
 
-    act_inplace<4>(&acc[0], p.act, p.slope);
-    if (OUTMODE == 0 && zo < ze && !(p.dbg & 4) && !(p.dbg & 32)) {
-#pragma unroll
-      for (int cp = 0; cp < 2; ++cp) {
-        unsigned pk[2][2];
-#pragma unroll
-        for (int h = 0; h < 2; ++h) {
-          float v[4];
-#pragma unroll
-          for (int j = 0; j < 4; ++j) {
-            float f = acc[2 * cp + h][j];
-              if (RangeCheck<T>::on) bad |= RangeCheck<T>::bad(f);
-            v[j] = f;
-          }
-          pk[h][0] = (unsigned)to_bits<T>(v[0]) | ((unsigned)to_bits<T>(v[1]) << 16);
-          pk[h][1] = (unsigned)to_bits<T>(v[2]) | ((unsigned)to_bits<T>(v[3]) << 16);
-        }
-        const auto s0 = __builtin_amdgcn_permlane16_swap(pk[0][0], pk[1][0], false, false);
-        const auto s1 = __builtin_amdgcn_permlane16_swap(pk[0][1], pk[1][1], false, false);
-        const int row = 2 * (2 * cp + (g & 1));
-        if (!full_xy && !((yl + row < p.H) & (xl < p.W))) continue;
-        *(uint4*)(out_w + (long long)zo * p.oz + row * p.oy) = make_uint4(s0[0], s1[0], s0[1], s1[1]);
-      }
-    } else if (zo < ze && !(p.dbg & 4)) {
-#pragma unroll
-      for (int c = 0; c < 4; ++c) {
-        if (!full_xy && !((yl + 2 * c < p.H) & (xl < p.W))) continue;
-        float v[4];
-#pragma unroll
-        for (int j = 0; j < 4; ++j) {
-          float f = acc[c][j];
-          if (OUTMODE == 0 && RangeCheck<T>::on) bad |= RangeCheck<T>::bad(f);
-          v[j] = f;
-        }
-        if (OUTMODE == 0) {
-          char* dst = out_l + (long long)zo * p.oz + (2 * c) * p.oy;
-          *(uint2*)dst = make_uint2((unsigned)to_bits<T>(v[0]) | ((unsigned)to_bits<T>(v[1]) << 16),
-                                    (unsigned)to_bits<T>(v[2]) | ((unsigned)to_bits<T>(v[3]) << 16));
-        } else {
-          float* dst = out32_l + (long long)zo * p.pz + (2 * c) * p.py;
-          if (p.wmap) {
-            const float wgt = p.wmap[((long long)zo * p.H + yl + 2 * c) * p.W + xl];
-#pragma unroll
-            for (int j = 0; j < 4; ++j) dst[(long long)j * p.pc] += wgt * v[j];
-          } else {
-#pragma unroll
-            for (int j = 0; j < 4; ++j) dst[(long long)j * p.pc] = v[j];
-          }
-        }
-      }
-    }
-  }
-  if (OUTMODE == 0 && RangeCheck<T>::on) raise_flag(p.oflow, bad);
+    if (OUTMODE == 0 && fast) epilogue(Const<1>{}, s, acc);
+    else epilogue(Const<0>{}, s, acc);
+    if constexpr (OUTMODE == 0) zb += 2 * p.oz;
+  }
+  if (OUTMODE == 0 && RangeCheck<T>::on) raise_flag(p.oflow, RangeCheck<T>::bad_bits(amax));
 }
 
 template <typename T>
@@ -327,17 +321,23 @@
          !(p.D & 1) && !(p.H & 1) && !(p.W & 1);
 }
 
-template <typename T, int OUTMODE>
+template <typename T, int OUTMODE, int ACT = -1>
 static hipError_t launch_upcat_t(ConvParams p, hipStream_t st, ConvLaunchInfo* info) {
   typedef UpcatCfg C;
+  if constexpr (ACT < 0) {
+    if (p.act == ACT_RELU) return launch_upcat_t<T, OUTMODE, ACT_RELU>(p, st, info);
+    if (p.act == ACT_LRELU) return launch_upcat_t<T, OUTMODE, ACT_LRELU>(p, st, info);
+    return launch_upcat_t<T, OUTMODE, ACT_NONE>(p, st, info);
+  } else {
   if (info) info->report(0, "conv3d_upcat16<%s,2x8x32,c8+l3,r%d/%d,o%d>", __is_same(T, f16) ? "f16" : "bf16", C::R, C::RL, OUTMODE);
-  auto kern = conv3d_upcat16_kernel<T, OUTMODE>;
+  auto kern = conv3d_upcat16_kernel<T, OUTMODE, ACT>;
   static amx::DeviceOnce attr_once;
   if (!attr_once.done()) {
     hipError_t e = hipFuncSetAttribute((const void*)kern, hipFuncAttributeMaxDynamicSharedMemorySize, C::LDS_BYTES);
     if (e != hipSuccess) return e;
     attr_once.set();
   }
+  if (p.out && (p.H + C::TY) * p.oy + (p.W + C::TX) * p.ox >= (1LL << 31)) return hipErrorInvalidValue;
   p.nby = (p.H + C::TY - 1) / C::TY;
   p.nbx = (p.W + C::TX - 1) / C::TX;
   const int tiles = p.nby * p.nbx * p.N;
@@ -345,6 +345,7 @@
   pick_z_segments(tiles, p.D, 2, 256 * (C::LDS_BYTES <= 80 * 1024 ? 2 : 1), &zseg, &nseg);
   hipLaunchKernelGGL(kern, dim3((unsigned)(tiles * nseg)), dim3((C::NC + C::NL) * 64), C::LDS_BYTES, st, p, zseg, nseg);
   return hipGetLastError();
+  }
 }
 
 hipError_t launch_conv_upcat16(const ConvParams& p, int precision, hipStream_t st, ConvLaunchInfo* info) {
diff --git a/anatomix_amd/csrc/amx_conv3d_zmarch.hip b/anatomix_amd/csrc/amx_conv3d_zmarch.hip
--- a/anatomix_amd/csrc/amx_conv3d_zmarch.hip
+++ b/anatomix_amd/csrc/amx_conv3d_zmarch.hip
@@ -67,7 +67,7 @@
   static constexpr bool OK = TX == 32 && IY == 12 && RSTG * 2 <= 60 && NLD == 7;
 };
 
-template <typename T, int NCK, int QT, int TY, int TX, int R, int OUTMODE, int NS, bool POOL, bool SPLIT = false, bool STEM = false>
+template <typename T, int NCK, int QT, int TY, int TX, int R, int OUTMODE, int NS, bool POOL, bool SPLIT = false, bool STEM = false, int ACT = ACT_NONE>
 __global__ __launch_bounds__((8 + (STEM ? ZmStemCfg<8, 32>::NSW + 1 : 2 * (SPLIT ? 2 : NCK)) + NS) * 64) void conv3d_k3_zmarch_kernel(const ConvParams p, int zseg, int nseg, const StemIn si) {
   static_assert(!SPLIT || (NCK == 1 && QT == 1 && NS == 0), "strict z-march: 16 -> 16, direct stores");
   static_assert(!STEM || (NCK == 1 && !SPLIT && NS == 0 && OUTMODE == 0), "stem-fed z-march: 16 input channels, direct 16-bit stores");
@@ -128,7 +128,7 @@
         asm volatile("s_waitcnt lgkmcnt(0)" ::: "memory");
         flag_store_asm(a_stored, s + 1);
         const int zo = zs + s * TZ + w;
-        if (zo >= ze || (p.dbg & 4)) continue;
+        if (zo >= ze) continue;
         char* dst = gbase + (long long)zo * p.oz;
 #pragma unroll
         for (int r = 0; r < NR; ++r) *(uint4*)(dst + (long long)(r / QT) * p.oy + (r % QT) * 1024) = v[r];
@@ -146,7 +146,7 @@
         asm volatile("s_waitcnt lgkmcnt(0)" ::: "memory");
         flag_store_asm(a_stored, s + 1);
         const int zo = zs + s * TZ + w;
-        if (zo >= ze || (p.dbg & 4)) continue;
+        if (zo >= ze) continue;
         float* dst = gbase + (long long)zo * p.pz;
         if (p.wmap) {
           const float4 wg = *(const float4*)(p.wmap + ((long long)zo * p.H + y0 + y) * p.W + x0 + xq * 4);
@@ -389,6 +389,7 @@
   if (!STEM && wave >= NC) {
     static_assert(STEM || C::VMCNT_OK, "loader wave must not exceed the 6-bit vmcnt range");
     const int cp = wave - NC;
+    const int lane = lane_id();
     int off[NDMA];
     bool valid[NDMA];
 #pragma unroll
@@ -436,8 +437,14 @@
 #pragma unroll
     for (int s = 0; s < kSteps; ++s) wreg[k][s] = *(const vec8*)(p.wpk + ((k * kSteps + s) * QT + wq) * 1024 + lane * 16);
   const int cb = g * 4 * QT + wq * 4;
+  constexpr bool TIGHT = NCKP > 1 && !SPLIT;
   f32x4 bias = f32x4{0.f, 0.f, 0.f, 0.f};
-  if (p.bias) bias = *(const f32x4*)(p.bias + cb);
+  float bias_q = 0.f;
+  if constexpr (TIGHT) {
+    if (p.bias) bias_q = p.bias[cb + (lane & 3)];
+  } else {
+    if (p.bias) bias = *(const f32x4*)(p.bias + cb);
+  }
   asm volatile("s_waitcnt vmcnt(0)" ::: "memory");
 
   const int lanebase = (g & 1) * PPL + ((wrow * HX) + wcx * 16 + li) * 16;
@@ -446,29 +453,173 @@
   const bool full_xy = (y0 + TY <= p.H) & (x0 + TX <= p.W);
 
   const int yl = y0 + wrow, xl = x0 + wcx * 16 + li;
-  char* out_l = OUTMODE == 0 ? p.out + (long long)n * p.on + (long long)yl * p.oy + (long long)xl * p.ox + cb * 2 : nullptr;
+  constexpr bool WIDE = OUTMODE == 0 && NS == 0 && QT == 1;
+  constexpr bool DIRECT16 = OUTMODE == 0 && NS == 0;
+  const unsigned lo_w = WIDE ? (unsigned)((yl + (g & 1)) * (int)p.oy + xl * (int)p.ox + (g >> 1) * 16) : 0u;
+  const unsigned lo_l = (DIRECT16 && !TIGHT) ? (unsigned)(yl * (int)p.oy + xl * (int)p.ox + cb * 2) : 0u;
+  char* zb = DIRECT16 ? p.out + (long long)n * p.on + (long long)zs * p.oz : nullptr;
+  if constexpr (TIGHT) zb += (long long)yl * p.oy + (long long)(x0 + wcx * 16) * p.ox + wq * 8;
+  const bool ok_w = full_xy || ((yl + (g & 1) < p.H) & (xl < p.W));
+  const bool ok_l0 = full_xy || ((yl < p.H) & (xl < p.W)), ok_l1 = full_xy || ((yl + 1 < p.H) & (xl < p.W));
   float* out32_l = OUTMODE == 1 ? p.out32 + (long long)n * p.pn + (long long)cb * p.pc + (long long)yl * p.py + xl : nullptr;
-  constexpr bool WIDE = OUTMODE == 0 && NS == 0 && QT == 1;
-  char* out_w = WIDE ? p.out + (long long)n * p.on + (long long)(yl + (g & 1)) * p.oy + (long long)xl * p.ox + (g >> 1) * 16 : nullptr;
   const bool vec_planar = OUTMODE == 1 && !(p.W & 3) && !(p.py & 3) && !(p.pz & 3) && !(p.pc & 3) && !(p.pn & 3) &&
                           !((size_t)p.out32 & 15) && !((size_t)p.wmap & 15);
   float* out32_q = OUTMODE == 1 ? p.out32 + (long long)n * p.pn + (long long)(cb + (li & 3)) * p.pc + (long long)yl * p.py +
                                       x0 + wcx * 16 + (li & ~3)
                                 : nullptr;
-  char* out2_l = (OUTMODE == 0 && POOL) ? p.out2 + (long long)n * p.qn + (long long)(yl >> 1) * p.qy +
-                                               (long long)(xl >> 1) * p.qx + cb * 2
-                                          : nullptr;
-
-  bool bad = false;
-  unsigned long long* trace = (p.dbg & 8) && (wave == 0 || wave == 4) && lane == 0 && blockIdx.x < 500
-                                  ? (unsigned long long*)p.stats + ((long long)blockIdx.x * 2 + (wave >> 2)) * 128 : nullptr;
-  int tcount = 0;
-#define AMX_ZSTAMP()                                                             \
-  do {                                                                           \
-    if (trace && tcount < 128) trace[tcount] = __builtin_readcyclecounter();     \
-    ++tcount;                                                                    \
-  } while (0)
-  AMX_ZSTAMP();
+  constexpr bool DOPOOL = OUTMODE == 0 && POOL;
+  const unsigned lo_p = (DOPOOL && !TIGHT) ? (unsigned)((yl >> 1) * (int)p.qy + (xl >> 1) * (int)p.qx + cb * 2) : 0u;
+  char* zb2 = DOPOOL ? p.out2 + (long long)n * p.qn + (long long)(zs >> 1) * p.qz : nullptr;
+  if constexpr (TIGHT && DOPOOL) zb2 += (long long)(yl >> 1) * p.qy + (long long)((x0 + wcx * 16) >> 1) * p.qx + wq * 8;
+  const bool ok_p = !(li & 1) && (full_xy || ((yl + 1 < p.H) & (xl + 1 < p.W)));
+
+  const int nfast = (DIRECT16 && full_xy) ? (ze - zs) / TZ : 0;
+  const unsigned a_done_w = lds_addr(done + wave);
+  unsigned amax_march = 0;
+  unsigned long long bad = 0;
+
+  auto epilogue = [&](auto fast_c, const int s, f32x4 (&acc)[2][2]) {
+    constexpr bool FAST = decltype(fast_c)::value != 0;
+    constexpr bool CHECK = OUTMODE == 0 && RangeCheck<T>::on;
+    constexpr bool PKPOOL = DOPOOL && ACT == ACT_RELU && !SPLIT;
+    act_values<ACT, 4>(&acc[0][0], p.slope);
+    unsigned ow = WIDE ? lo_w : lo_l, op = lo_p, amax = amax_march;
+    int li_e = li;
+    if constexpr (TIGHT) {
+      const int l = lane_id();
+      li_e = l & 15;
+      ow = (unsigned)(li_e * (int)p.ox + (l >> 4) * (8 * QT));
+      op = (unsigned)((li_e >> 1) * (int)p.qx + (l >> 4) * (8 * QT));
+      amax = 0;
+    } else {
+      if constexpr (DIRECT16) asm volatile("" : "+v"(ow));
+      if constexpr (DOPOOL) asm volatile("" : "+v"(op));
+    }
+    [[maybe_unused]] float pooled[4] = {-3.0e38f, -3.0e38f, -3.0e38f, -3.0e38f};
+    [[maybe_unused]] unsigned ppk[2] = {0u, 0u};
+#pragma unroll
+    for (int tz = 0; tz < 2; ++tz) {
+      const int zo = zs + s * TZ + tz;
+      const bool zok = FAST || zo < ze;
+      unsigned pk[2][2];
+      if constexpr (OUTMODE == 0) {
+#pragma unroll
+        for (int cy = 0; cy < 2; ++cy) {
+          const f32x4 v = acc[tz][cy];
+          if (CHECK && zok) {
+            amax = RangeCheck<T>::template track<ACT == ACT_RELU>(amax, v[0], v[1]);
+            amax = RangeCheck<T>::template track<ACT == ACT_RELU>(amax, v[2], v[3]);
+          }
+          pk[cy][0] = Ops<T>::pack2(v[0], v[1]);
+          pk[cy][1] = Ops<T>::pack2(v[2], v[3]);
+          if constexpr (PKPOOL) {
+            ppk[0] = pk_umax16(ppk[0], pk[cy][0]);
+            ppk[1] = pk_umax16(ppk[1], pk[cy][1]);
+          } else if constexpr (DOPOOL) {
+#pragma unroll
+            for (int j = 0; j < 4; ++j) pooled[j] = v[j] > pooled[j] ? v[j] : pooled[j];
+          }
+        }
+      }
+      if constexpr (WIDE) {
+        const auto s0 = __builtin_amdgcn_permlane16_swap(pk[0][0], pk[1][0], false, false);
+        const auto s1 = __builtin_amdgcn_permlane16_swap(pk[0][1], pk[1][1], false, false);
+        unsigned l0a = 0, l0b = 0, l1a = 0, l1b = 0;
+        if constexpr (SPLIT) {
+          unsigned pl[2][2];
+#pragma unroll
+          for (int cy = 0; cy < 2; ++cy) {
+            float r[4];
+#pragma unroll
+            for (int j = 0; j < 4; ++j) r[j] = acc[tz][cy][j] - (float)(T)acc[tz][cy][j];
+            pl[cy][0] = Ops<T>::pack2(r[0], r[1]);
+            pl[cy][1] = Ops<T>::pack2(r[2], r[3]);
+          }
+          const auto t0 = __builtin_amdgcn_permlane16_swap(pl[0][0], pl[1][0], false, false);
+          const auto t1 = __builtin_amdgcn_permlane16_swap(pl[0][1], pl[1][1], false, false);
+          l0a = t0[0]; l0b = t0[1]; l1a = t1[0]; l1b = t1[1];
+        }
+        if (FAST || (zok && ok_w)) {
+          char* dst = zb + (tz ? p.oz : 0) + ow;
+          *(uint4*)dst = make_uint4(s0[0], s1[0], s0[1], s1[1]);
+          if constexpr (SPLIT) *(uint4*)(dst + p.Cout * 2) = make_uint4(l0a, l1a, l0b, l1b);
+        }
+      } else {
+#pragma unroll
+        for (int cy = 0; cy < 2; ++cy) {
+          if constexpr (NS > 0) {
+            if (OUTMODE == 0) {
+              char* dst = smem + STAGEOFF + (s % SG::NB) * SG::BYTES + (((tz * TY + wrow + cy) * TX) + wcx * 16 + li) * SG::CB + cb * 2;
+              *(uint2*)dst = make_uint2(pk[cy][0], pk[cy][1]);
+            } else {
+              float v[4] = {acc[tz][cy][0], acc[tz][cy][1], acc[tz][cy][2], acc[tz][cy][3]};
+              quad_transpose4(v, li);
+              char* dst = smem + STAGEOFF + (cb + (li & 3)) * SG::CS + ((tz * TY + wrow + cy) * TX + wcx * 16 + (li & ~3)) * 4;
+              *(float4*)dst = make_float4(v[0], v[1], v[2], v[3]);
+            }
+          } else if constexpr (OUTMODE == 0) {
+            if (FAST || (zok && (cy ? ok_l1 : ok_l0)))
+              *(uint2*)(zb + (tz ? p.oz : 0) + (cy ? p.oy : 0) + ow) = make_uint2(pk[cy][0], pk[cy][1]);
+          } else {
+            if (!zok || !(cy ? ok_l1 : ok_l0)) continue;
+            float v[4] = {acc[tz][cy][0], acc[tz][cy][1], acc[tz][cy][2], acc[tz][cy][3]};
+            if (vec_planar) {
+              quad_transpose4(v, li);
+              float* dst = out32_q + (long long)zo * p.pz + cy * p.py;
+              float4 o = make_float4(v[0], v[1], v[2], v[3]);
+              if (p.wmap) {
+                const float4 wg = *(const float4*)(p.wmap + ((long long)zo * p.H + yl + cy) * p.W + x0 + wcx * 16 + (li & ~3));
+                const float4 old = *(const float4*)dst;
+                o = make_float4(old.x + wg.x * o.x, old.y + wg.y * o.y, old.z + wg.z * o.z, old.w + wg.w * o.w);
+              }
+              *(float4*)dst = o;
+            } else {
+              float* dst = out32_l + (long long)zo * p.pz + cy * p.py;
+              if (p.wmap) {
+                const float wgt = p.wmap[((long long)zo * p.H + yl + cy) * p.W + xl];
+#pragma unroll
+                for (int j = 0; j < 4; ++j) dst[(long long)j * p.pc] += wgt * v[j];
+              } else {
+#pragma unroll
+                for (int j = 0; j < 4; ++j) dst[(long long)j * p.pc] = v[j];
+              }
+            }
+          }
+        }
+      }
+    }
+    if constexpr (NS > 0) {
+      asm volatile("" ::: "memory");
+      flag_store(staged + wave, s + 1);
+    }
+    if constexpr (DOPOOL) {
+      const bool pst = FAST || (zs + s * TZ + 1 < ze && ok_p);
+      if constexpr (PKPOOL) {
+        const unsigned m0 = pk_umax16(ppk[0], dpp_xor1(ppk[0])), m1 = pk_umax16(ppk[1], dpp_xor1(ppk[1]));
+        if (FAST ? !(li_e & 1) : pst) *(uint2*)(zb2 + op) = make_uint2(m0, m1);
+      } else {
+        float pm[4];
+#pragma unroll
+        for (int j = 0; j < 4; ++j) {
+          const float o = dpp_quad<0xB1>(pooled[j]);
+          pm[j] = pooled[j] > o ? pooled[j] : o;
+        }
+        if (FAST ? !(li_e & 1) : pst) {
+          char* dst = zb2 + op;
+          *(uint2*)dst = make_uint2(Ops<T>::pack2(pm[0], pm[1]), Ops<T>::pack2(pm[2], pm[3]));
+          if constexpr (SPLIT) {
+            float r[4];
+#pragma unroll
+            for (int j = 0; j < 4; ++j) r[j] = pm[j] - (float)(T)pm[j];
+            *(uint2*)(dst + p.Cout * 2) = make_uint2(Ops<T>::pack2(r[0], r[1]), Ops<T>::pack2(r[2], r[3]));
+          }
+        }
+      }
+    }
+    if constexpr (TIGHT) bad |= __builtin_amdgcn_ballot_w64(RangeCheck<T>::bad_bits(amax));
+    else amax_march = amax;
+  };
+
   for (int s = 0; s < nsteps; ++s) {
     {
       int need = TZ * s + TZ + 2;
@@ -482,7 +633,6 @@
       asm volatile("" ::: "memory");
     }
 
-    AMX_ZSTAMP();
     int b1[4], bx3[4];
 #pragma unroll
     for (int pl = 0; pl < 4; ++pl) {
@@ -494,10 +644,12 @@
 #pragma unroll
     for (int tz = 0; tz < 2; ++tz)
 #pragma unroll
-      for (int cy = 0; cy < 2; ++cy) acc[tz][cy] = bias;
-
-    for (int rep = (p.dbg >> 10) & 7; rep >= 0; --rep)
-    if (!(p.dbg & 2)) {
+      for (int cy = 0; cy < 2; ++cy) {
+        if constexpr (TIGHT) acc[tz][cy] = f32x4{dpp_quad<0x00>(bias_q), dpp_quad<0x55>(bias_q), dpp_quad<0xAA>(bias_q), dpp_quad<0xFF>(bias_q)};
+        else acc[tz][cy] = bias;
+      }
+
+    {
       if constexpr ((NCKP > 1 && !SPLIT) || STEM) {
         constexpr int PER = 4 * 6 + 8, NU = NCKP * PER, NSLOT = 4;
         int slo[4];
@@ -618,144 +770,36 @@
       }
       }
     asm volatile("s_waitcnt lgkmcnt(0)" ::: "memory");
-    flag_store(done + wave, s + 1);
-    AMX_ZSTAMP();
-
-    if (p.dbg & 4) {
-      if (NS) flag_store(staged + wave, s + 1);
-      continue;
-    }
+    if constexpr (TIGHT) {
+      unsigned da = a_done_w;
+      asm volatile("" : "+s"(da));
+      flag_store((int*)(__attribute__((address_space(3))) int*)(size_t)da, s + 1);
+    } else {
+      flag_store(done + wave, s + 1);
+    }
+
     if constexpr (NS > 0) {
       if (s >= SG::NB)
         while (flag_min2(stored) < s + 1 - SG::NB) __builtin_amdgcn_s_sleep(1);
       asm volatile("" ::: "memory");
     }
-    act_inplace<4>(&acc[0][0], p.act, p.slope);
-    float pooled[4] = {-3.0e38f, -3.0e38f, -3.0e38f, -3.0e38f};
-#pragma unroll
-    for (int tz = 0; tz < 2; ++tz) {
-      const int zo = zs + s * TZ + tz;
-      if (WIDE && (SPLIT || !(p.dbg & 32))) {
-        unsigned pk[2][2], pl[SPLIT ? 2 : 1][2];
-#pragma unroll
-        for (int cy = 0; cy < 2; ++cy) {
-          float v[4];
-#pragma unroll
-          for (int j = 0; j < 4; ++j) {
-            float f = acc[tz][cy][j];
-              if (RangeCheck<T>::on) bad |= RangeCheck<T>::bad(f);
-            v[j] = f;
-            pooled[j] = f > pooled[j] ? f : pooled[j];
-          }
-          pk[cy][0] = (unsigned)to_bits<T>(v[0]) | ((unsigned)to_bits<T>(v[1]) << 16);
-          pk[cy][1] = (unsigned)to_bits<T>(v[2]) | ((unsigned)to_bits<T>(v[3]) << 16);
-          if constexpr (SPLIT) {
-            float r[4];
-#pragma unroll
-            for (int j = 0; j < 4; ++j) r[j] = v[j] - (float)(T)v[j];
-            pl[cy][0] = (unsigned)to_bits<T>(r[0]) | ((unsigned)to_bits<T>(r[1]) << 16);
-            pl[cy][1] = (unsigned)to_bits<T>(r[2]) | ((unsigned)to_bits<T>(r[3]) << 16);
-          }
-        }
-        const auto s0 = __builtin_amdgcn_permlane16_swap(pk[0][0], pk[1][0], false, false);
-        const auto s1 = __builtin_amdgcn_permlane16_swap(pk[0][1], pk[1][1], false, false);
-        unsigned l0a = 0, l0b = 0, l1a = 0, l1b = 0;
-        if constexpr (SPLIT) {
-          const auto t0 = __builtin_amdgcn_permlane16_swap(pl[0][0], pl[1][0], false, false);
-          const auto t1 = __builtin_amdgcn_permlane16_swap(pl[0][1], pl[1][1], false, false);
-          l0a = t0[0]; l0b = t0[1]; l1a = t1[0]; l1b = t1[1];
-        }
-        if (zo >= ze) continue;
-        if (!full_xy && !((yl + (g & 1) < p.H) & (xl < p.W))) continue;
-        *(uint4*)(out_w + (long long)zo * p.oz) = make_uint4(s0[0], s1[0], s0[1], s1[1]);
-        if constexpr (SPLIT) *(uint4*)(out_w + (long long)zo * p.oz + p.Cout * 2) = make_uint4(l0a, l1a, l0b, l1b);
-        continue;
-      }
-#pragma unroll
-      for (int cy = 0; cy < 2; ++cy) {
-        float v[4];
-#pragma unroll
-        for (int j = 0; j < 4; ++j) {
-          float f = acc[tz][cy][j];
-          if (OUTMODE == 0 && RangeCheck<T>::on) bad |= RangeCheck<T>::bad(f);
-          v[j] = f;
-          pooled[j] = f > pooled[j] ? f : pooled[j];
-        }
-        if constexpr (NS > 0) {
-          if (OUTMODE == 0) {
-            char* dst = smem + STAGEOFF + (s % SG::NB) * SG::BYTES + (((tz * TY + wrow + cy) * TX) + wcx * 16 + li) * SG::CB + cb * 2;
-            *(uint2*)dst = make_uint2((unsigned)to_bits<T>(v[0]) | ((unsigned)to_bits<T>(v[1]) << 16),
-                                      (unsigned)to_bits<T>(v[2]) | ((unsigned)to_bits<T>(v[3]) << 16));
-          } else {
-            quad_transpose4(v, li);
-            char* dst = smem + STAGEOFF + (cb + (li & 3)) * SG::CS + ((tz * TY + wrow + cy) * TX + wcx * 16 + (li & ~3)) * 4;
-            *(float4*)dst = make_float4(v[0], v[1], v[2], v[3]);
-          }
-          continue;
-        }
-        if (zo >= ze) continue;
-        if (!full_xy && !((yl + cy < p.H) & (xl < p.W))) continue;
-        if (OUTMODE == 0) {
-          char* dst = out_l + (long long)zo * p.oz + cy * p.oy;
-          *(uint2*)dst = make_uint2((unsigned)to_bits<T>(v[0]) | ((unsigned)to_bits<T>(v[1]) << 16),
-                                    (unsigned)to_bits<T>(v[2]) | ((unsigned)to_bits<T>(v[3]) << 16));
-        } else if (vec_planar) {
-          quad_transpose4(v, li);
-          float* dst = out32_q + (long long)zo * p.pz + cy * p.py;
-          float4 o = make_float4(v[0], v[1], v[2], v[3]);
-          if (p.wmap) {
-            const float4 wg = *(const float4*)(p.wmap + ((long long)zo * p.H + yl + cy) * p.W + x0 + wcx * 16 + (li & ~3));
-            const float4 old = *(const float4*)dst;
-            o = make_float4(old.x + wg.x * o.x, old.y + wg.y * o.y, old.z + wg.z * o.z, old.w + wg.w * o.w);
-          }
-          *(float4*)dst = o;
-        } else {
-          float* dst = out32_l + (long long)zo * p.pz + cy * p.py;
-          if (p.wmap) {
-            const float wgt = p.wmap[((long long)zo * p.H + yl + cy) * p.W + xl];
-#pragma unroll
-            for (int j = 0; j < 4; ++j) dst[(long long)j * p.pc] += wgt * v[j];
-          } else {
-#pragma unroll
-            for (int j = 0; j < 4; ++j) dst[(long long)j * p.pc] = v[j];
-          }
-        }
-      }
-    }
-    if constexpr (NS > 0) {
-      asm volatile("" ::: "memory");
-      flag_store(staged + wave, s + 1);
-    }
-    if constexpr (OUTMODE == 0 && POOL) {
-      float pm[4];
-#pragma unroll
-      for (int j = 0; j < 4; ++j) {
-        const float o = dpp_quad<0xB1>(pooled[j]);
-        pm[j] = pooled[j] > o ? pooled[j] : o;
-      }
-      const int zp = (zs + s * TZ) >> 1;
-      if (!(li & 1) && zs + s * TZ + 1 < ze && (full_xy || ((yl + 1 < p.H) & (xl + 1 < p.W)))) {
-        char* dst = out2_l + (long long)zp * p.qz;
-        *(uint2*)dst = make_uint2((unsigned)to_bits<T>(pm[0]) | ((unsigned)to_bits<T>(pm[1]) << 16),
-                                  (unsigned)to_bits<T>(pm[2]) | ((unsigned)to_bits<T>(pm[3]) << 16));
-        if constexpr (SPLIT) {
-          float r[4];
-#pragma unroll
-          for (int j = 0; j < 4; ++j) r[j] = pm[j] - (float)(T)pm[j];
-          *(uint2*)(dst + p.Cout * 2) = make_uint2((unsigned)to_bits<T>(r[0]) | ((unsigned)to_bits<T>(r[1]) << 16),
-                                                   (unsigned)to_bits<T>(r[2]) | ((unsigned)to_bits<T>(r[3]) << 16));
-        }
-      }
-    }
-    AMX_ZSTAMP();
-  }
-  if (OUTMODE == 0 && RangeCheck<T>::on) raise_flag(p.oflow, bad);
-}
-
-template <typename T, int NCK, int QT, int TY, int R, int OUTMODE, int NS, bool POOL = false, bool SPLIT = false, int TX = 32, bool STEM = false>
+    if (DIRECT16 && s < nfast) epilogue(Const<1>{}, s, acc);
+    else epilogue(Const<0>{}, s, acc);
+    if constexpr (DIRECT16) zb += TZ * p.oz;
+    if constexpr (DOPOOL) zb2 += p.qz;
+  }
+  if (OUTMODE == 0 && RangeCheck<T>::on) raise_flag(p.oflow, (bad != 0) | RangeCheck<T>::bad_bits(amax_march));
+}
+
+template <typename T, int NCK, int QT, int TY, int R, int OUTMODE, int NS, bool POOL = false, bool SPLIT = false, int TX = 32, bool STEM = false, int ACT = -1>
 static hipError_t launch_zm_ns(ConvParams p, hipStream_t st, ConvLaunchInfo* info, const StemIn& si = StemIn{}) {
   if constexpr (OUTMODE == 0 && NS == 0 && !POOL && !STEM)
     if (p.out2) return launch_zm_ns<T, NCK, QT, TY, R, OUTMODE, NS, true, SPLIT, TX, STEM>(p, st, info, si);
+  if constexpr (ACT < 0) {
+    if (p.act == ACT_RELU) return launch_zm_ns<T, NCK, QT, TY, R, OUTMODE, NS, POOL, SPLIT, TX, STEM, ACT_RELU>(p, st, info, si);
+    if (p.act == ACT_LRELU) return launch_zm_ns<T, NCK, QT, TY, R, OUTMODE, NS, POOL, SPLIT, TX, STEM, ACT_LRELU>(p, st, info, si);
+    return launch_zm_ns<T, NCK, QT, TY, R, OUTMODE, NS, POOL, SPLIT, TX, STEM, ACT_NONE>(p, st, info, si);
+  } else {
   constexpr int TZ = 2;
   typedef ZmCfg<SPLIT ? 2 : NCK, QT, TY, TX, R> C;
   constexpr int LDS = STEM ? C::FLAGOFF + 128 + ZmStemCfg<TY, TX>::BYTES : NS ? C::FLAGOFF + 128 + ZmStage<QT, TY, TX, OUTMODE>::TOTAL : C::LDS_BYTES;
@@ -765,13 +809,15 @@
   else if (info)
     info->report(0, "conv3d_k3_zmarch<%s%s,%d->%d,%dx%dx%d,c8+l%d+s%d,r%d,o%d%s>", __is_same(T, f16) ? "f16" : "bf16", SPLIT ? "x2" : "",
                  16 * NCK, 16 * QT, TZ, TY, TX, C::NL, NS, R, OUTMODE, p.out2 ? ",pool" : "");
-  auto kern = conv3d_k3_zmarch_kernel<T, NCK, QT, TY, TX, R, OUTMODE, NS, POOL, SPLIT, STEM>;
+  auto kern = conv3d_k3_zmarch_kernel<T, NCK, QT, TY, TX, R, OUTMODE, NS, POOL, SPLIT, STEM, ACT>;
   static amx::DeviceOnce attr_once;
   if (!attr_once.done()) {
     hipError_t e = hipFuncSetAttribute((const void*)kern, hipFuncAttributeMaxDynamicSharedMemorySize, LDS);
     if (e != hipSuccess) return e;
     attr_once.set();
   }
+  if (p.out && (p.H + TY) * p.oy + (p.W + TX) * p.ox >= (1LL << 31)) return hipErrorInvalidValue;
+  if (p.out2 && (p.H / 2 + TY) * p.qy + (p.W / 2 + TX) * p.qx >= (1LL << 31)) return hipErrorInvalidValue;
   p.nby = (p.H + TY - 1) / TY;
   p.nbx = (p.W + TX - 1) / TX;
   const int tiles = p.nby * p.nbx * p.N;
@@ -779,6 +825,7 @@
   pick_z_segments(tiles, p.D, TZ, 256 * (LDS <= 80 * 1024 ? 2 : 1), &zseg, &nseg);
   hipLaunchKernelGGL(kern, dim3((unsigned)(tiles * nseg)), dim3((8 + (STEM ? ZmStemCfg<TY, TX>::NSW + 1 : C::NL) + NS) * 64), LDS, st, p, zseg, nseg, si);
   return hipGetLastError();
+  }
 }
 
 template <int TY>
diff --git a/anatomix_amd/csrc/amx_device.h b/anatomix_amd/csrc/amx_device.h
--- a/anatomix_amd/csrc/amx_device.h
+++ b/anatomix_amd/csrc/amx_device.h
@@ -39,10 +39,19 @@
 template <typename T> struct RangeCheck {
   static constexpr bool on = false;
   static __device__ __forceinline__ bool bad(float) { return false; }
+  template <bool NONNEG> static __device__ __forceinline__ unsigned track(unsigned amax, float, float) { return amax; }
+  static __device__ __forceinline__ bool bad_bits(unsigned) { return false; }
 };
 template <> struct RangeCheck<f16> {
   static constexpr bool on = true;
   static __device__ __forceinline__ bool bad(float v) { return !(__builtin_fabsf(v) <= 65504.f); }
+  template <bool NONNEG> static __device__ __forceinline__ unsigned track(unsigned amax, float a, float b) {
+    unsigned ua = __builtin_bit_cast(unsigned, a), ub = __builtin_bit_cast(unsigned, b);
+    if (!NONNEG) { ua &= 0x7fffffffu; ub &= 0x7fffffffu; }
+    ua = ua > ub ? ua : ub;
+    return amax > ua ? amax : ua;
+  }
+  static __device__ __forceinline__ bool bad_bits(unsigned amax) { return amax > 0x477fe000u; }
 };
 __device__ __forceinline__ void raise_flag(int* flag, bool bad) {
   if (bad && flag) __atomic_store_n(flag, 1, __ATOMIC_RELAXED);
@@ -110,6 +119,13 @@
   return __builtin_bit_cast(unsigned short, t);
 }
 
+__device__ __forceinline__ int lane_id() { return (int)__builtin_amdgcn_mbcnt_hi(~0u, __builtin_amdgcn_mbcnt_lo(~0u, 0u)); }
+
+__device__ __forceinline__ unsigned pk_umax16(unsigned a, unsigned b) {
+  typedef __attribute__((ext_vector_type(2))) unsigned short u16x2;
+  return __builtin_bit_cast(unsigned, __builtin_elementwise_max(__builtin_bit_cast(u16x2, a), __builtin_bit_cast(u16x2, b)));
+}
+
 template <int CTRL>
 __device__ __forceinline__ float dpp_quad(float x) {
   return __builtin_bit_cast(float, __builtin_amdgcn_update_dpp(0, __builtin_bit_cast(int, x), CTRL, 0xF, 0xF, true));
@@ -147,6 +163,20 @@
 #pragma unroll
       for (int j = 0; j < 4; ++j) a[i][j] = a[i][j] > 0.f ? a[i][j] : a[i][j] * slope;
   }
+}
+
+template <int V> struct Const { static constexpr int value = V; };
+template <int ACT, int N>
+__device__ __forceinline__ void act_values(f32x4* a, float slope) {
+  float pinf = __builtin_inff();
+  if constexpr (ACT == ACT_RELU) asm volatile("" : "+s"(pinf));
+#pragma unroll
+  for (int i = 0; i < N; ++i)
+#pragma unroll
+    for (int j = 0; j < 4; ++j) {
+      if constexpr (ACT == ACT_RELU) a[i][j] = __builtin_amdgcn_fmed3f(a[i][j], 0.f, pinf);
+      else if constexpr (ACT == ACT_LRELU) a[i][j] = a[i][j] > 0.f ? a[i][j] : a[i][j] * slope;
+    }
 }
 
 __device__ __forceinline__ float act_k(int act, float slope) { return act == ACT_RELU ? 0.f : (act == ACT_LRELU ? slope : 1.f); }
diff --git a/include/anatomix_amd.h b/include/anatomix_amd.h
--- a/include/anatomix_amd.h
+++ b/include/anatomix_amd.h
@@ -134,6 +134,11 @@
                           const float* d_scale, const float* d_shift, int cout, int n, int d, int hh,
                           int w, int act, float slope, int precision, void* d_wpk, void* d_out16,
                           float* d_out32, void* stream);
+
+int amx_conv3d_k3_reflect_probe(const void* d_x0, int c0, const void* d_x1, int c1, const float* d_weight, const float* d_scale,
+                                const float* d_shift, int cout, int n, int d, int hh, int w, int act, float slope, int precision,
+                                void* d_wpk, void* d_out16, float* d_out32, void* d_pool16, const float* d_wmap, int* d_oflow,
+                                char* kernel_name, void* stream);
 
 size_t amx_conv3d_scratch_bytes(int c0, int c1, int cout, int n, int d, int hh, int w, int precision);
 int amx_conv3d_k3_reflect_ws(const void* d_x0, int c0, const void* d_x1, int c1, const float* d_weight,
```

Result: faster. 3077 volumes/s (median of 6 runs) (+3.0%).
